# EnricoMiccoli/nodal

Measured on AMD Instinct MI355X. Metric: circuits_per_sec, higher is better.
Workload: dtype f64; 1 GPU; cfg3: grid(1000) 1e6 nodes, sparse CSR path; n=999999, nnz=4995995, parallelism=one GPU

## Files before the change

include/nodal_hip.h:

```cpp
#ifndef NODAL_HIP_H
#define NODAL_HIP_H

#include <stddef.h>
#include <stdint.h>

#ifdef __cplusplus
extern "C" {
#endif

typedef struct nodal_ctx *nodal_handle;

typedef enum {
    NODAL_OK = 0,
    NODAL_E_INVALID = 1,
    NODAL_E_HIP = 2,
    NODAL_E_ZERO_RESISTANCE = 3,
    NODAL_E_STAMP_COLLISION = 4,
    NODAL_E_SINGULAR = 5,
    NODAL_E_NOMEM = 6,
    NODAL_E_UNSUPPORTED = 7
} nodal_status;

enum { NODAL_T_R = 0, NODAL_T_A = 1, NODAL_T_E = 2, NODAL_T_VCVS = 3,
       NODAL_T_CCVS = 4, NODAL_T_CCCS = 5,
       NODAL_T_GM = 6 };

enum { NODAL_SPARSE_AUTO = 0,
       NODAL_SPARSE_PCG = 1,
       NODAL_SPARSE_DENSIFY = 2,
       NODAL_SPARSE_LU = 3,
       NODAL_SPARSE_DIRECT = 4 };

int nodal_create(int device_id, nodal_handle *out);
int nodal_destroy(nodal_handle h);
const char *nodal_last_error(nodal_handle h);
const char *nodal_version(void);

int nodal_upload_components(nodal_handle h, int64_t ncomp,
                            const uint8_t *type, const double *value,
                            const int32_t *a, const int32_t *b,
                            const int32_t *c, const int32_t *d,
                            const int32_t *drv, const int32_t *k,
                            int32_t K, int32_t B);
int nodal_host_alloc(size_t bytes, void **out);
int nodal_host_free(void *p);

int nodal_upload_values(nodal_handle h, int32_t batch, const double *values);

int nodal_assemble_symbolic(nodal_handle h);
int nodal_assemble_numeric(nodal_handle h, int32_t member, int64_t *bad_component);

int nodal_get_sizes(nodal_handle h, int64_t *n, int64_t *nnz, int64_t *ncontrib);

int nodal_export_csr(nodal_handle h, int32_t *indptr, int32_t *indices,
                     double *data, double *rhs);
int nodal_export_dense(nodal_handle h, double *G, double *rhs);

int nodal_solve_dense(nodal_handle h, double *x, int32_t *info);
int nodal_solve_sparse(nodal_handle h, int32_t method, double *x, int32_t *info,
                       int32_t *iters, double *resid);
int nodal_download_x(nodal_handle h, double *x);

int nodal_solve_pairs(nodal_handle h, int32_t dense, int32_t npairs, const int32_t *ia,
                      const int32_t *ib, double *resistance, int32_t *info);

int nodal_solve_sources(nodal_handle h, int32_t dense, int32_t count, int32_t nsrc, const int64_t *rows,
                        const double *values, double *x_out, double *resid_out, int32_t *info_out);

int nodal_branches(nodal_handle h, double *voltage, double *current, double *power, double *totals2);

int nodal_solve_sources_branches(nodal_handle h, int32_t dense, int32_t count, int32_t nsrc, const int64_t *rows,
                                 const double *values, double *x_out, double *resid_out, int32_t *info_out,
                                 double *current_absmax, int32_t *current_member, double *potential_min,
                                 int32_t *potential_min_member, double *potential_max, int32_t *potential_max_member,
                                 double *power_out);

int nodal_sensitivities(nodal_handle h, int32_t dense, int32_t count, const int32_t *kind, const int32_t *p,
                        const int32_t *q2, double *sens_out, double *value_out, double *adjoint_out,
                        double *resid_out, int32_t *info_out);

int nodal_gradient(nodal_handle h, int32_t dense, int32_t count, const double *x, const double *cotangent, int32_t nsrc,
                   const int64_t *rows, double *grad_out, double *grad_sources_out, double *adjoint_out,
                   double *resid_out, int32_t *info_out);

int nodal_transient(nodal_handle h, int32_t dense, int32_t steps, int32_t method, int64_t ncap, const int64_t *cap_rows,
                    int32_t nsrc, const int64_t *src_rows, const double *src_values, const double *x0, int32_t nprobe,
                    const int32_t *probe_a, const int32_t *probe_b, double *wave_out, int32_t keep_every, double *x_out,
                    double *pot_min, int32_t *pot_min_step, double *pot_max, int32_t *pot_max_step, double *resid_out,
                    int32_t *info_out, int32_t *iters_out);

int nodal_transient_rlc(nodal_handle h, int32_t dense, int32_t steps, int32_t method, int64_t ncap, const int64_t *cap_rows,
                        int32_t nsrc, const int64_t *src_rows, const double *src_values, const double *x0, int32_t nprobe,
                        const int32_t *probe_a, const int32_t *probe_b, double *wave_out, int32_t keep_every, double *x_out,
                        double *pot_min, int32_t *pot_min_step, double *pot_max, int32_t *pot_max_step, double *resid_out,
                        int32_t *info_out, int32_t *iters_out, int64_t nind, const int64_t *ind_rows, const double *i0,
                        int32_t ncur, const int32_t *cur_index, double *cur_out, double *i_final_out);

int nodal_transient_gradient(nodal_handle h, int32_t dense, int32_t nprobe, const int32_t *probe_a, const int32_t *probe_b,
                             const double *wave_cot ,
                             double *grad_out ,
                             double *grad_sources_out ,
                             double *grad_x0_out ,
                             double *adjoint_out ,
                             double *resid_out , int32_t *info_out );

int nodal_ac_sweep(nodal_handle h, int32_t dense, int32_t nfreq, const double *omega ,
                   int64_t nreact, const uint8_t *kind , const double *value ,
                   const int32_t *lead_a, const int32_t *lead_b ,
                   int32_t nsrc, const int64_t *src_rows, const double *src_re, const double *src_im,
                   int32_t nprobe, const int32_t *probe_a, const int32_t *probe_b, double *wave_out ,
                   int32_t ncur, const int32_t *cur_index , double *cur_out ,
                   int32_t keep_every, double *x_out ,
                   double *peak_out , int32_t *peak_freq_out ,
                   double *resid_out , int32_t *info_out );

int nodal_ac_noise(nodal_handle h, int32_t dense, int32_t nfreq, const double *omega ,
                   int64_t nreact, const uint8_t *kind , const double *value ,
                   const int32_t *lead_a, const int32_t *lead_b ,
                   double temperature ,
                   int32_t nout, const int32_t *out_a, const int32_t *out_b ,
                   int64_t input_row , const double *weight ,
                   double *density_out , double *gain_out ,
                   double *contrib_out , double *resid_out ,
                   int32_t *info_out );

int nodal_ac_ports(nodal_handle h, int32_t dense, int32_t nfreq, const double *omega ,
                   int64_t nreact, const uint8_t *kind , const double *value ,
                   const int32_t *lead_a, const int32_t *lead_b ,
                   int32_t nports, const int32_t *ia, const int32_t *ib ,
                   double *z_out ,
                   double *node_peak_out , int32_t *node_peak_port_out ,
                   int32_t *node_peak_freq_out ,
                   double *resid_out , int32_t *info_out ,
                   int64_t *work_out );

int nodal_port_matrix(nodal_handle h, int32_t dense, int32_t nports, const int32_t *ia, const int32_t *ib,
                      double *z_out , double *voc_out ,
                      double *resid_out , int32_t *info_out );

int nodal_residual(nodal_handle h, double *scaled_residual);

int nodal_run(nodal_handle h, int32_t dense, int32_t member, int32_t reuse_symbolic,
              int32_t *info);

int nodal_run_batch(nodal_handle h, int32_t first, int32_t count, int32_t reuse_symbolic,
                    double *x_out, int32_t *info_out);
int nodal_batch_x_device(nodal_handle h, void *device_dst, int64_t capacity_bytes);
int nodal_x_device(nodal_handle h, void *device_dst, int64_t capacity_bytes);

int nodal_last_timings(nodal_handle h, double *ms3);
int nodal_last_kernel_stats(nodal_handle h, double *ms_total, int64_t *launches,
                            double *alg_bytes_or_flops);

int nodal_last_solve_info(nodal_handle h, int32_t *iterations, int32_t *amg_levels,
                          double *relative_residual);

int nodal_synchronize(nodal_handle h);

enum {
    NODAL_OPT_FORCE_PIVOTING = 1, NODAL_OPT_GEPP_PANEL = 2, NODAL_OPT_EXTRA_STREAMS = 3, NODAL_OPT_BORROW_TABLE = 4,
    NODAL_OPT_TRANSIENT_TAPE = 5
};
int nodal_set_option(nodal_handle h, int32_t option, int32_t value);

int nodal_debug_gemm(nodal_handle h, int32_t M, int32_t N, int32_t K, const double *A,
                     const double *B, double *C);
int nodal_debug_sources_rhs(nodal_handle h, int32_t count, int32_t nsrc, const int64_t *rows,
                            const double *values, double *rhs_out);
int nodal_debug_residual(nodal_handle h, int32_t transposed, int32_t cols, int32_t layout, const double *x,
                         const double *b, double *scaled_out, double *norms_out);
int nodal_debug_direct_apply(nodal_handle h, int32_t transposed, int32_t cols, const double *r, double *z,
                             int64_t *perturbed_out, int32_t *info_out);
enum {
    NODAL_HA_ACOL = 0, NODAL_HA_AVAL = 1, NODAL_HA_AVALF = 2, NODAL_HA_ALEN = 3, NODAL_HA_DINV = 4, NODAL_HA_ADCOL = 5,
    NODAL_HA_AGG = 6, NODAL_HA_PCOL = 7, NODAL_HA_PVAL = 8, NODAL_HA_PVALF = 9, NODAL_HA_RCOL = 10, NODAL_HA_RVAL = 11,
    NODAL_HA_RVALF = 12, NODAL_HA_RLEN = 13, NODAL_HA_WCOL = 14, NODAL_HA_WVAL = 15, NODAL_HA_WLEN = 16
};
int nodal_debug_hierarchy_info(nodal_handle h, int32_t *nlev, int64_t *ints , double *reals );
int nodal_debug_hierarchy_array(nodal_handle h, int32_t level, int32_t which, void *dst, int64_t capacity_bytes,
                                int64_t *bytes_out);

#ifdef __cplusplus
}
#endif
#endif
```

nodal_amd/_ffi.py:

```python

import atexit
import ctypes as C
import os
import weakref

import numpy as np

_HERE = os.path.dirname(os.path.abspath(__file__))
LIB_PATH = os.path.join(_HERE, "libnodal_hip.so")

OK, E_INVALID, E_HIP, E_ZERO_RESISTANCE, E_STAMP_COLLISION, E_SINGULAR, E_NOMEM, \
    E_UNSUPPORTED = range(8)
SPARSE_AUTO, SPARSE_PCG, SPARSE_DENSIFY, SPARSE_LU, SPARSE_DIRECT = range(5)
OPT_FORCE_PIVOTING = 1
OPT_GEPP_PANEL = 2
OPT_EXTRA_STREAMS = 3
OPT_BORROW_TABLE = 4
OPT_TRANSIENT_TAPE = 5

_p = C.POINTER
_i32p, _i64p, _f64p, _u8p = _p(C.c_int32), _p(C.c_int64), _p(C.c_double), _p(C.c_uint8)

SIGNATURES = {
    "nodal_version": (C.c_char_p, []),
    "nodal_create": (C.c_int, [C.c_int, _p(C.c_void_p)]),
    "nodal_destroy": (C.c_int, [C.c_void_p]),
    "nodal_last_error": (C.c_char_p, [C.c_void_p]),
    "nodal_upload_components": (C.c_int, [C.c_void_p, C.c_int64, _u8p, _f64p, _i32p, _i32p,
                                          _i32p, _i32p, _i32p, _i32p, C.c_int32, C.c_int32]),
    "nodal_host_alloc": (C.c_int, [C.c_size_t, _p(C.c_void_p)]),
    "nodal_host_free": (C.c_int, [C.c_void_p]),
    "nodal_upload_values": (C.c_int, [C.c_void_p, C.c_int32, _f64p]),
    "nodal_assemble_symbolic": (C.c_int, [C.c_void_p]),
    "nodal_assemble_numeric": (C.c_int, [C.c_void_p, C.c_int32, _i64p]),
    "nodal_get_sizes": (C.c_int, [C.c_void_p, _i64p, _i64p, _i64p]),
    "nodal_export_csr": (C.c_int, [C.c_void_p, _i32p, _i32p, _f64p, _f64p]),
    "nodal_export_dense": (C.c_int, [C.c_void_p, _f64p, _f64p]),
    "nodal_solve_dense": (C.c_int, [C.c_void_p, _f64p, _i32p]),
    "nodal_solve_sparse": (C.c_int, [C.c_void_p, C.c_int32, _f64p, _i32p, _i32p, _f64p]),
    "nodal_download_x": (C.c_int, [C.c_void_p, _f64p]),
    "nodal_solve_pairs": (C.c_int, [C.c_void_p, C.c_int32, C.c_int32, _i32p, _i32p, _f64p, _i32p]),
    "nodal_solve_sources": (C.c_int, [C.c_void_p, C.c_int32, C.c_int32, C.c_int32, _i64p, _f64p, _f64p, _f64p,
                                      _i32p]),
    "nodal_branches": (C.c_int, [C.c_void_p, _f64p, _f64p, _f64p, _f64p]),
    "nodal_solve_sources_branches": (C.c_int, [C.c_void_p, C.c_int32, C.c_int32, C.c_int32, _i64p, _f64p, _f64p, _f64p,
                                               _i32p, _f64p, _i32p, _f64p, _i32p, _f64p, _i32p, _f64p]),
    "nodal_sensitivities": (C.c_int, [C.c_void_p, C.c_int32, C.c_int32, _i32p, _i32p, _i32p, _f64p, _f64p, _f64p, _f64p,
                                      _i32p]),
    "nodal_gradient": (C.c_int, [C.c_void_p, C.c_int32, C.c_int32, _f64p, _f64p, C.c_int32, _i64p, _f64p, _f64p, _f64p,
                                 _f64p, _i32p]),
    "nodal_transient": (C.c_int, [C.c_void_p, C.c_int32, C.c_int32, C.c_int32, C.c_int64, _i64p, C.c_int32, _i64p, _f64p,
                                  _f64p, C.c_int32, _i32p, _i32p, _f64p, C.c_int32, _f64p, _f64p, _i32p, _f64p, _i32p,
                                  _f64p, _i32p, _i32p]),
    "nodal_transient_rlc": (C.c_int, [C.c_void_p, C.c_int32, C.c_int32, C.c_int32, C.c_int64, _i64p, C.c_int32, _i64p, _f64p,
                                      _f64p, C.c_int32, _i32p, _i32p, _f64p, C.c_int32, _f64p, _f64p, _i32p, _f64p, _i32p,
                                      _f64p, _i32p, _i32p, C.c_int64, _i64p, _f64p, C.c_int32, _i32p, _f64p, _f64p]),
    "nodal_transient_gradient": (C.c_int, [C.c_void_p, C.c_int32, C.c_int32, _i32p, _i32p, _f64p, _f64p, _f64p, _f64p, _f64p,
                                           _f64p, _i32p]),
    "nodal_ac_sweep": (C.c_int, [C.c_void_p, C.c_int32, C.c_int32, _f64p, C.c_int64, _u8p, _f64p, _i32p, _i32p, C.c_int32,
                                 _i64p, _f64p, _f64p, C.c_int32, _i32p, _i32p, _f64p, C.c_int32, _i32p, _f64p, C.c_int32,
                                 _f64p, _f64p, _i32p, _f64p, _i32p]),
    "nodal_ac_noise": (C.c_int, [C.c_void_p, C.c_int32, C.c_int32, _f64p, C.c_int64, _u8p, _f64p, _i32p, _i32p, C.c_double,
                                 C.c_int32, _i32p, _i32p, C.c_int64, _f64p, _f64p, _f64p, _f64p, _f64p, _i32p]),
    "nodal_ac_ports": (C.c_int, [C.c_void_p, C.c_int32, C.c_int32, _f64p, C.c_int64, _u8p, _f64p, _i32p, _i32p, C.c_int32,
                                 _i32p, _i32p, _f64p, _f64p, _i32p, _i32p, _f64p, _i32p, _i64p]),
    "nodal_port_matrix": (C.c_int, [C.c_void_p, C.c_int32, C.c_int32, _i32p, _i32p, _f64p, _f64p, _f64p, _i32p]),
    "nodal_residual": (C.c_int, [C.c_void_p, _f64p]),
    "nodal_run": (C.c_int, [C.c_void_p, C.c_int32, C.c_int32, C.c_int32, _i32p]),
    "nodal_run_batch": (C.c_int, [C.c_void_p, C.c_int32, C.c_int32, C.c_int32, _f64p, _i32p]),
    "nodal_batch_x_device": (C.c_int, [C.c_void_p, C.c_void_p, C.c_int64]),
    "nodal_x_device": (C.c_int, [C.c_void_p, C.c_void_p, C.c_int64]),
    "nodal_last_timings": (C.c_int, [C.c_void_p, _f64p]),
    "nodal_last_kernel_stats": (C.c_int, [C.c_void_p, _f64p, _i64p, _f64p]),
    "nodal_last_solve_info": (C.c_int, [C.c_void_p, _i32p, _i32p, _f64p]),
    "nodal_synchronize": (C.c_int, [C.c_void_p]),
    "nodal_set_option": (C.c_int, [C.c_void_p, C.c_int32, C.c_int32]),
    "nodal_debug_gemm": (C.c_int, [C.c_void_p, C.c_int32, C.c_int32, C.c_int32, _f64p, _f64p, _f64p]),
    "nodal_debug_sources_rhs": (C.c_int, [C.c_void_p, C.c_int32, C.c_int32, _i64p, _f64p, _f64p]),
    "nodal_debug_residual": (C.c_int, [C.c_void_p, C.c_int32, C.c_int32, C.c_int32, _f64p, _f64p, _f64p, _f64p]),
    "nodal_debug_direct_apply": (C.c_int, [C.c_void_p, C.c_int32, C.c_int32, _f64p, _f64p, _i64p, _i32p]),
    "nodal_debug_hierarchy_info": (C.c_int, [C.c_void_p, _i32p, _i64p, _f64p]),
    "nodal_debug_hierarchy_array": (C.c_int, [C.c_void_p, C.c_int32, C.c_int32, C.c_void_p, C.c_int64, _i64p]),
}

HIERARCHY_ARRAYS = (("acol", np.int32), ("aval", np.float64), ("avalf", np.float32), ("alen", np.int32),
                    ("dinv", np.float64), ("adcol", np.int16), ("agg", np.int32), ("pcol", np.int32),
                    ("pval", np.float64), ("pvalf", np.float32), ("rcol", np.int32), ("rval", np.float64),
                    ("rvalf", np.float32), ("rlen", np.int32), ("wcol", np.int32), ("wval", np.float32),
                    ("wlen", np.int32))
HIERARCHY_INFO = ("n", "ld", "nc", "width", "maxlen", "wfix", "nnz", "rld", "rcap", "wslots", "fold_want", "fold", "d16",
                  "in_tail", "refreshed", "dense_coarsest")

_lib = None
_live = weakref.WeakSet()


@atexit.register
def _close_all():
    _closing[0] = True
    for h in list(_live):
        h.close()


class NodalHipError(RuntimeError):
    def __init__(self, status, message):
        super().__init__(f"libnodal_hip status {status}: {message}")
        self.status = status


def load():
    global _lib
    if _lib is None:
        if not os.path.exists(LIB_PATH):
            raise OSError(
                f"{LIB_PATH} not found: build it with `make` (or "
                "`python -c 'import __graft_entry__ as g; g.build()'`) -- "
                "nodal_amd has no CPU fallback")
        lib = C.CDLL(LIB_PATH)
        for name, (res, args) in SIGNATURES.items():
            fn = getattr(lib, name)
            fn.restype, fn.argtypes = res, args
        _lib = lib
    return _lib


def _ptr(arr, ctype):
    return arr.ctypes.data_as(_p(ctype))


PINNED_MIN_BYTES = 1 << 20
_PINNED_POOL = {}
_PINNED_POOL_BYTES = [0]
_PINNED_POOL_MAX = 1 << 30
_pinned_ok = [None]
_closing = [False]


def _pinned_release(addr, nbytes):
    if _lib is None or _closing[0]:
        return
    if _PINNED_POOL_BYTES[0] + nbytes <= _PINNED_POOL_MAX:
        _PINNED_POOL.setdefault(nbytes, []).append(addr)
        _PINNED_POOL_BYTES[0] += nbytes
    else:
        _lib.nodal_host_free(C.c_void_p(addr))


def host_empty(count, dtype):
    dtype = np.dtype(dtype)
    nbytes = int(count) * dtype.itemsize
    if nbytes < PINNED_MIN_BYTES or _pinned_ok[0] is False:
        return np.empty(count, dtype=dtype)
    try:
        lib = load()
    except OSError:
        _pinned_ok[0] = False
        return np.empty(count, dtype=dtype)
    size = (nbytes + 4095) & ~4095
    free = _PINNED_POOL.get(size)
    if free:
        addr = free.pop()
        _PINNED_POOL_BYTES[0] -= size
    else:
        out = C.c_void_p()
        if lib.nodal_host_alloc(size, C.byref(out)) != OK or not out.value:
            _pinned_ok[0] = False
            return np.empty(count, dtype=dtype)
        _pinned_ok[0] = True
        addr = out.value
    buf = (C.c_char * size).from_address(addr)
    weakref.finalize(buf, _pinned_release, addr, size)
    return np.frombuffer(buf, dtype=dtype, count=count)


class Handle:

    def __init__(self, device=0):
        self.lib = load()
        self._h = C.c_void_p()
        status = self.lib.nodal_create(device, C.byref(self._h))
        if status != OK:
            raise NodalHipError(
                status, f"nodal_create(device={device}) failed: no usable MI355X "
                "(HIP device) is visible; nodal_amd has no CPU fallback")
        self.n = self.nnz = self.ncontrib = 0
        self._ncomp = self._K = 0
        self.lib.nodal_set_option(self._h, OPT_BORROW_TABLE, 1)
        _live.add(self)

    def close(self):
        if getattr(self, "_h", None):
            self.lib.nodal_destroy(self._h)
            self._h = None

    __del__ = close

    @property
    def closed(self):
        return not getattr(self, "_h", None)

    def _check(self, status, allow=()):
        if status != OK and status not in allow:
            raise NodalHipError(status, self.lib.nodal_last_error(self._h).decode())
        return status

    def upload(self, table):
        names = ("type", "value", "a", "b") if table.B == 0 else ("type", "value", "a", "b", "c", "d", "drv", "k")
        cols = [np.ascontiguousarray(getattr(table, n)) for n in names]
        self._keep = cols
        t, v, a, b = cols[:4]
        rest = [_ptr(x, C.c_int32) for x in cols[4:]] or [None] * 4
        self.n_members = table.K + table.B
        self._ncomp, self._K = int(table.ncomp), int(table.K)
        self._check(self.lib.nodal_upload_components(
            self._h, table.ncomp, _ptr(t, C.c_uint8), _ptr(v, C.c_double),
            _ptr(a, C.c_int32), _ptr(b, C.c_int32), *rest, table.K, table.B))

    def upload_values(self, values):
        values = np.ascontiguousarray(values, dtype=np.float64)
        assert values.ndim == 2
        self._check(self.lib.nodal_upload_values(self._h, values.shape[0], _ptr(values, C.c_double)))

    def assemble_symbolic(self):
        self._check(self.lib.nodal_assemble_symbolic(self._h))
        self._refresh_sizes()

    def _refresh_sizes(self):
        n, nnz, nc = C.c_int64(), C.c_int64(), C.c_int64()
        self._check(self.lib.nodal_get_sizes(self._h, C.byref(n), C.byref(nnz), C.byref(nc)))
        self.n, self.nnz, self.ncontrib = n.value, nnz.value, nc.value

    def assemble_numeric(self, member=0):
        bad = C.c_int64(-1)
        status = self._check(self.lib.nodal_assemble_numeric(self._h, member, C.byref(bad)),
                             allow=(E_ZERO_RESISTANCE, E_STAMP_COLLISION))
        return status, bad.value

    def export_csr(self, values=True):
        indptr = np.empty(self.n + 1, dtype=np.int32)
        indices = np.empty(self.nnz, dtype=np.int32)
        data = np.empty(self.nnz, dtype=np.float64) if values else None
        rhs = np.empty(self.n, dtype=np.float64) if values else None
        self._check(self.lib.nodal_export_csr(
            self._h, _ptr(indptr, C.c_int32), _ptr(indices, C.c_int32),
            _ptr(data, C.c_double) if values else None,
            _ptr(rhs, C.c_double) if values else None))
        return indptr, indices, data, rhs

    def export_dense(self):
        G = np.empty((self.n, self.n), dtype=np.float64)
        rhs = np.empty(self.n, dtype=np.float64)
        self._check(self.lib.nodal_export_dense(self._h, _ptr(G, C.c_double), _ptr(rhs, C.c_double)))
        return G, rhs

    def solve_dense(self, download=True):
        x = host_empty(self.n, np.float64) if download else None
        info = C.c_int32(0)
        self._check(self.lib.nodal_solve_dense(
            self._h, _ptr(x, C.c_double) if download else None, C.byref(info)),
            allow=(E_SINGULAR,))
        return x, info.value

    def solve_sparse(self, method=SPARSE_AUTO, download=True):
        x = host_empty(self.n, np.float64) if download else None
        info, iters, resid = C.c_int32(0), C.c_int32(0), C.c_double(0)
        self._check(self.lib.nodal_solve_sparse(
            self._h, method, _ptr(x, C.c_double) if download else None,
            C.byref(info), C.byref(iters), C.byref(resid)))
        return x, info.value, iters.value, resid.value

    def solve_pairs(self, ia, ib, dense):
        ia = np.ascontiguousarray(ia, dtype=np.int32)
        ib = np.ascontiguousarray(ib, dtype=np.int32)
        out = np.empty(len(ia), dtype=np.float64)
        info = C.c_int32(0)
        self._check(self.lib.nodal_solve_pairs(self._h, int(dense), len(ia), _ptr(ia, C.c_int32),
                                               _ptr(ib, C.c_int32), _ptr(out, C.c_double),
                                               C.byref(info)), allow=(E_SINGULAR,))
        return out, info.value

    def solve_sources(self, rows, values, dense):
        rows = np.ascontiguousarray(rows, dtype=np.int64)
        values = np.ascontiguousarray(values, dtype=np.float64)
        assert values.ndim == 2 and values.shape[1] == len(rows)
        count = values.shape[0]
        x = np.empty((count, self.n), dtype=np.float64)
        info = np.zeros(count, dtype=np.int32)
        resid = np.zeros(count, dtype=np.float64)
        self._check(self.lib.nodal_solve_sources(self._h, int(dense), count, len(rows), _ptr(rows, C.c_int64),
                                                 _ptr(values, C.c_double), _ptr(x, C.c_double),
                                                 _ptr(resid, C.c_double), _ptr(info, C.c_int32)))
        return x, info, resid

    def solve_sources_branches(self, rows, values, dense, keep_solutions=True):
        rows = np.ascontiguousarray(rows, dtype=np.int64)
        values = np.ascontiguousarray(values, dtype=np.float64)
        assert values.ndim == 2 and values.shape[1] == len(rows)
        count = values.shape[0]
        ncomp, K = self._ncomp, self._K
        x = np.empty((count, self.n), dtype=np.float64) if keep_solutions else None
        info = np.zeros(count, dtype=np.int32)
        resid = np.zeros(count, dtype=np.float64)
        env = {"current_absmax": np.empty(ncomp), "current_member": np.empty(ncomp, dtype=np.int32),
               "potential_min": np.empty(K), "potential_min_member": np.empty(K, dtype=np.int32),
               "potential_max": np.empty(K), "potential_max_member": np.empty(K, dtype=np.int32),
               "power": np.empty((count, 2))}
        self._check(self.lib.nodal_solve_sources_branches(
            self._h, int(dense), count, len(rows), _ptr(rows, C.c_int64), _ptr(values, C.c_double),
            _ptr(x, C.c_double) if keep_solutions else None, _ptr(resid, C.c_double), _ptr(info, C.c_int32),
            *(_ptr(env[key], C.c_int32 if key.endswith("member") else C.c_double) for key in env)))
        return x, info, resid, env

    def branches(self, voltage=True, current=True, power=True):
        out = [host_empty(self._ncomp, np.float64) if want else None for want in (voltage, current, power)]
        totals = np.zeros(2)
        self._check(self.lib.nodal_branches(self._h, *(_ptr(a, C.c_double) if a is not None else None for a in out),
                                            _ptr(totals, C.c_double)))
        return out[0], out[1], out[2], float(totals[0]), float(totals[1])

    def sensitivities(self, kind, p, q2, dense, adjoints=False, out=None):
        kind, p, q2 = (np.ascontiguousarray(v, dtype=np.int32) for v in (kind, p, q2))
        count = len(kind)
        assert len(p) == count and len(q2) == count
        if out is not None:
            assert out.shape == (count, self._ncomp) and out.dtype == np.float64 and out.flags.c_contiguous
            sens = out
        else:
            sens = host_empty(count * self._ncomp, np.float64).reshape(count, self._ncomp)
        lam = host_empty(count * self.n, np.float64).reshape(count, self.n) if adjoints else None
        y = np.zeros(count, dtype=np.float64)
        resid = np.zeros(count, dtype=np.float64)
        info = np.zeros(count, dtype=np.int32)
        self._check(self.lib.nodal_sensitivities(
            self._h, int(dense), count, _ptr(kind, C.c_int32), _ptr(p, C.c_int32), _ptr(q2, C.c_int32),
            _ptr(sens, C.c_double), _ptr(y, C.c_double), _ptr(lam, C.c_double) if adjoints else None,
            _ptr(resid, C.c_double), _ptr(info, C.c_int32)))
        return sens, y, lam, resid, info

    def gradient(self, cotangents, dense, rows=None, solutions=None, adjoints=False):
        cot = np.ascontiguousarray(cotangents, dtype=np.float64)
        assert cot.ndim == 2 and cot.shape[1] == self.n
        count = cot.shape[0]
        rows = np.ascontiguousarray(rows if rows is not None else [], dtype=np.int64)
        x = None
        if solutions is not None:
            x = np.ascontiguousarray(solutions, dtype=np.float64)
            assert x.shape == cot.shape
        grad = np.zeros(self._ncomp, dtype=np.float64)
        gsrc = np.zeros((count, len(rows)), dtype=np.float64)
        lam = host_empty(count * self.n, np.float64).reshape(count, self.n) if adjoints else None
        resid = np.zeros(count, dtype=np.float64)
        info = np.zeros(count, dtype=np.int32)
        self._check(self.lib.nodal_gradient(
            self._h, int(dense), count, _ptr(x, C.c_double) if x is not None else None, _ptr(cot, C.c_double),
            len(rows), _ptr(rows, C.c_int64) if len(rows) else None, _ptr(grad, C.c_double), _ptr(gsrc, C.c_double),
            _ptr(lam, C.c_double) if adjoints else None, _ptr(resid, C.c_double), _ptr(info, C.c_int32)))
        return grad, gsrc, lam, resid, info

    def port_matrix(self, ia, ib, dense, voc=True):
        ia, ib = (np.ascontiguousarray(v, dtype=np.int32) for v in (ia, ib))
        count = len(ia)
        assert ia.ndim == 1 and ib.shape == ia.shape
        z = np.zeros((count, count), dtype=np.float64)
        v_oc = np.zeros(count, dtype=np.float64) if voc else None
        resid = np.zeros(count, dtype=np.float64)
        info = np.zeros(count, dtype=np.int32)
        self._check(self.lib.nodal_port_matrix(
            self._h, int(dense), count, _ptr(ia, C.c_int32), _ptr(ib, C.c_int32), _ptr(z, C.c_double),
            _ptr(v_oc, C.c_double) if voc else None, _ptr(resid, C.c_double), _ptr(info, C.c_int32)))
        return z, v_oc, info, resid

    def transient(self, cap_rows, rows, values, x0, ia, ib, dense, method=0, keep_every=0, envelope=False):
        return self._transient(cap_rows, rows, values, x0, ia, ib, dense, method, keep_every, envelope)[:6]

    def transient_rlc(self, cap_rows, ind_rows, rows, values, x0, i0, ia, ib, cur_index, dense, method=0, keep_every=0,
                      envelope=False):
        return self._transient(cap_rows, rows, values, x0, ia, ib, dense, method, keep_every, envelope,
                               inductors=(ind_rows, i0, cur_index))

    def _transient(self, cap_rows, rows, values, x0, ia, ib, dense, method, keep_every, envelope, inductors=None):
        cap_rows = np.ascontiguousarray(cap_rows, dtype=np.int64)
        rows = np.ascontiguousarray(rows, dtype=np.int64)
        values = np.ascontiguousarray(values, dtype=np.float64)
        assert values.ndim == 2 and values.shape[1] == len(rows)
        steps = values.shape[0]
        x0 = np.ascontiguousarray(x0, dtype=np.float64)
        assert x0.shape == (self.n,)
        ia, ib = (np.ascontiguousarray(v, dtype=np.int32) for v in (ia, ib))
        assert ia.ndim == 1 and ib.shape == ia.shape
        wave = np.zeros((steps + 1, len(ia)), dtype=np.float64)
        kept = steps // keep_every if keep_every > 0 else 0
        x = host_empty(kept * self.n, np.float64).reshape(kept, self.n) if keep_every > 0 else None
# ... 260 lines not shown
```

nodal_amd/csrc/knobs.h:

```cpp
#pragma once
#include <stdint.h>
#include <stdlib.h>

#include <optional>

namespace knob {

struct Present {
    const char *name;
    bool now() const { return getenv(name) != nullptr; }
};
struct OnUnless0 {
    const char *name;
    bool now() const { const char *e = getenv(name); return !(e && atoi(e) == 0); }
};
struct OffUnlessNon0 {
    const char *name;
    bool now() const { const char *e = getenv(name); return e && atoi(e) != 0; }
};
struct OnIfSet0 {
    const char *name;
    bool now() const { const char *e = getenv(name); return e != nullptr && atoi(e) == 0; }
};
struct Level {
    const char *name;
    int now() const {
        const char *e = getenv(name);
        if (!e) return 0;
        const int v = atoi(e);
        return v > 1 ? v : 1;
    }
};
struct Int {
    const char *name;
    int dflt;
    int now() const { const char *e = getenv(name); return e ? atoi(e) : dflt; }
};
struct Int64 {
    const char *name;
    int64_t dflt;
    int64_t now() const { const char *e = getenv(name); return e ? atoll(e) : dflt; }
};
struct Double {
    const char *name;
    double dflt;
    double now() const { const char *e = getenv(name); return e ? atof(e) : dflt; }
};
struct IntIfSet {
    const char *name;
    std::optional<int> now() const { const char *e = getenv(name); return e ? std::optional<int>(atoi(e)) : std::nullopt; }
};
struct Int64IfSet {
    const char *name;
    std::optional<int64_t> now() const { const char *e = getenv(name); return e ? std::optional<int64_t>(atoll(e)) : std::nullopt; }
};
struct DoubleIfSet {
    const char *name;
    std::optional<double> now() const { const char *e = getenv(name); return e ? std::optional<double>(atof(e)) : std::nullopt; }
};
struct Text {
    const char *name;
    const char *now() const { return getenv(name); }
};

inline constexpr Present TRACE{"NODAL_TRACE"};
inline constexpr Level POISON{"NODAL_POISON"};
inline constexpr Present NOFILL{"NODAL_NOFILL"};
inline constexpr Present NANCHECK{"NODAL_NANCHECK"};
inline constexpr Double WAIT_TIMEOUT_S{"NODAL_WAIT_TIMEOUT_S", 60.0};
inline constexpr Text STREAM_PRIORITY{"NODAL_STREAM_PRIORITY"};
inline constexpr IntIfSet EXTRA_STREAMS{"NODAL_EXTRA_STREAMS"};
inline constexpr IntIfSet HOST_THREADS{"NODAL_HOST_THREADS"};
inline constexpr IntIfSet CSV_CHUNKS{"NODAL_CSV_CHUNKS"};
inline constexpr OnUnless0 FOLD_STREAM{"NODAL_FOLD_STREAM"};
inline constexpr OffUnlessNon0 COUNT_LDS{"NODAL_COUNT_LDS"};
inline constexpr IntIfSet DENSE_BLOCKINV{"NODAL_DENSE_BLOCKINV"};
inline constexpr IntIfSet GJ_SCALAR{"NODAL_GJ_SCALAR"};
inline constexpr OnUnless0 GJ_DPP{"NODAL_GJ_DPP"};
inline constexpr OnUnless0 BI_SYM{"NODAL_BI_SYM"};
inline constexpr OnIfSet0 BI_MASKED{"NODAL_BI_MASKED"};
inline constexpr Int PANEL_CUS{"NODAL_PANEL_CUS", 32};
inline constexpr Int64 BI_UNMASK_ROWS{"NODAL_BI_UNMASK_ROWS", 0};
inline constexpr OnUnless0 BI_EARLY_COPY{"NODAL_BI_EARLY_COPY"};
inline constexpr Int BI_FIRST_BLOCKS{"NODAL_BI_FIRST_BLOCKS", 2};
inline constexpr Text BI_SWITCH{"NODAL_BI_SWITCH"};
inline constexpr Text BI_SWITCH2{"NODAL_BI_SWITCH2"};
inline constexpr Text BI_WIDTH{"NODAL_BI_WIDTH"};
inline constexpr IntIfSet GEPP_PANEL{"NODAL_GEPP_PANEL"};
inline constexpr Int GEPP_MAX{"NODAL_GEPP_MAX", 1280};
inline constexpr Present GEPP_PROBE{"NODAL_GEPP_PROBE"};
inline constexpr Int64IfSet FCG_MAXIT{"NODAL_FCG_MAXIT"};
inline constexpr OnUnless0 FCG_HOST_SUM{"NODAL_FCG_HOST_SUM"};
inline constexpr Double FCG_LOOK{"NODAL_FCG_LOOK", 0.75};
inline constexpr OnUnless0 LOWDEG{"NODAL_LOWDEG"};
inline constexpr IntIfSet LOWDEG_SHARE{"NODAL_LOWDEG_SHARE"};
inline constexpr Int64 LOWDEG_MIN{"NODAL_LOWDEG_MIN", 32};
inline constexpr Present SPARSE_FORCE_DIRECT{"NODAL_SPARSE_FORCE_DIRECT"};
inline constexpr Present SPARSE_CHILD_DIRECT{"NODAL_SPARSE_CHILD_DIRECT"};
inline constexpr OnUnless0 SAGG{"NODAL_SAGG"};
inline constexpr OnUnless0 SA_REUSE{"NODAL_SA_REUSE"};
inline constexpr OnUnless0 SA_FORK{"NODAL_SA_FORK"};
inline constexpr Double SA_SPREAD{"NODAL_SA_SPREAD", 16.0};
inline constexpr Double SA_SHARE{"NODAL_SA_SHARE", 0.9};
inline constexpr IntIfSet SA_MIS{"NODAL_SA_MIS"};
inline constexpr Text SA_OMEGA_P{"NODAL_SA_OMEGA_P"};
inline constexpr Double SA_PADSLACK{"NODAL_SA_PADSLACK", 1.3};
inline constexpr OnUnless0 SA_D16{"NODAL_SA_D16"};
inline constexpr Int SA_GG{"NODAL_SA_GG", 40};
inline constexpr Int64 SA_GCAP{"NODAL_SA_GCAP", 16384};
inline constexpr Int SA_GSEG{"NODAL_SA_GSEG", 4};
inline constexpr Text SA_NU{"NODAL_SA_NU"};
inline constexpr Int SA_KCYCLE{"NODAL_SA_KCYCLE", 1};
inline constexpr Int SA_KLEVELS{"NODAL_SA_KLEVELS", 1};
inline constexpr OnUnless0 SA_KFREEZE{"NODAL_SA_KFREEZE"};
inline constexpr OnUnless0 SA_FUSE_DIR{"NODAL_SA_FUSE_DIR"};
inline constexpr OffUnlessNon0 SA_GRAPH{"NODAL_SA_GRAPH"};
inline constexpr Text SA_FOLD_POST{"NODAL_SA_FOLD_POST"};
inline constexpr OffUnlessNon0 SA_FOLD_CHECK{"NODAL_SA_FOLD_CHECK"};
inline constexpr OnUnless0 SA_TAIL_DENSE{"NODAL_SA_TAIL_DENSE"};
inline constexpr OffUnlessNon0 SA_TAIL_CHECK{"NODAL_SA_TAIL_CHECK"};
inline constexpr Int SA_TAIL_NU{"NODAL_SA_TAIL_NU", 3};
inline constexpr Present TAIL_PROBE{"NODAL_TAIL_PROBE"};
inline constexpr IntIfSet AMG_PASSES0{"NODAL_AMG_PASSES0"};
inline constexpr IntIfSet AMG_PASSES1{"NODAL_AMG_PASSES1"};
inline constexpr IntIfSet AMG_SWEEPS0{"NODAL_AMG_SWEEPS0"};
inline constexpr IntIfSet AMG_BLOCK{"NODAL_AMG_BLOCK"};
inline constexpr DoubleIfSet AMG_THETA{"NODAL_AMG_THETA"};
inline constexpr Present AMG_KEEP_DENSE{"NODAL_AMG_KEEP_DENSE"};
inline constexpr Present AMG_NOTAIL{"NODAL_AMG_NOTAIL"};
inline constexpr IntIfSet AMG_KMAX{"NODAL_AMG_KMAX"};
inline constexpr OnUnless0 PAIRS_BLOCK{"NODAL_PAIRS_BLOCK"};
inline constexpr OnUnless0 PAIRS_FUNCTIONAL{"NODAL_PAIRS_FUNCTIONAL"};
inline constexpr Int PAIRS_DIRECT{"NODAL_PAIRS_DIRECT", -1};
inline constexpr Int64 PAIRS_DIRECT_MIN{"NODAL_PAIRS_DIRECT_MIN", 256};
inline constexpr Double MULTI_BAR{"NODAL_MULTI_BAR", 1e-14};
inline constexpr IntIfSet PRESOLVE{"NODAL_PRESOLVE"};
inline constexpr OnUnless0 PRESOLVE_KEEP{"NODAL_PRESOLVE_KEEP"};
inline constexpr IntIfSet FGMRES_WINDOW{"NODAL_FGMRES_WINDOW"};
inline constexpr Text DIRECT_NB{"NODAL_DIRECT_NB"};
inline constexpr Int DIRECT_LANES{"NODAL_DIRECT_LANES", 4};
inline constexpr DoubleIfSet DIRECT_MAX_GB{"NODAL_DIRECT_MAX_GB"};
inline constexpr IntIfSet DIRECT_BIG_DIM{"NODAL_DIRECT_BIG_DIM"};
inline constexpr OnUnless0 DIRECT_FRONT_LDS{"NODAL_DIRECT_FRONT_LDS"};
inline constexpr Int DIRECT_LDS_BS{"NODAL_DIRECT_LDS_BS", 64};
inline constexpr OnUnless0 DIRECT_PANEL_REGS{"NODAL_DIRECT_PANEL_REGS"};
inline constexpr OnUnless0 DIRECT_BATCHED{"NODAL_DIRECT_BATCHED"};
inline constexpr OnUnless0 DIRECT_WAVE{"NODAL_DIRECT_WAVE"};
inline constexpr Present DIRECT_LEVELS{"NODAL_DIRECT_LEVELS"};
inline constexpr OnUnless0 DIRECT_SUPER{"NODAL_DIRECT_SUPER"};
inline constexpr OnUnless0 DIRECT_APPLY_STEPPED{"NODAL_DIRECT_APPLY_STEPPED"};
inline constexpr OnUnless0 DIRECT_PEEL{"NODAL_DIRECT_PEEL"};
inline constexpr Int ND_DEPTH{"NODAL_ND_DEPTH", 4};
inline constexpr Int64 ND_PAR{"NODAL_ND_PAR", 20000};
inline constexpr Present SLU_DEBUG{"SLU_DEBUG"};

}
```

nodal_amd/csrc/sagg.hip:

```cpp
#include <hip/hip_ext.h>

#include <atomic>
#include <type_traits>

#include "group.h"

int grounded_flags(nodal_ctx *h, uint8_t *flags_dev);

namespace {

using grp::TB;
constexpr int PW = 4;
constexpr int ACAP = 64;
constexpr int RCAP = 96;
constexpr int RCAP_SMALL = 512;
constexpr int RCAP_SMALL_ROWS = 16384;
inline int rcap_for(int64_t nc) { return nc <= RCAP_SMALL_ROWS ? RCAP_SMALL : RCAP; }
constexpr int W0_MAX = 32;
constexpr int COARSEST = 64;
constexpr int MAX_LEVELS = 12;
constexpr int MIS_ROUNDS = 6;
constexpr int TAIL_MAX_N = 1024;
constexpr int TAIL_LEVELS = 6;
constexpr int TAIL_LDS_BUDGET = 150 * 1024;
constexpr int APAD = 32;
constexpr int DOT_BLOCKS = 1024;
#ifndef NODAL_SA_OMEGA
#define NODAL_SA_OMEGA 0.85
#endif
constexpr double OMEGA = NODAL_SA_OMEGA;
constexpr double OMEGA_P = 0.70;
constexpr double OMEGA_P_COARSE = 0.85;
using cyc_t = nodal_cyc_t;

inline unsigned grid_for(int64_t n, unsigned cap = 8192) {
    int64_t g = (n + TB - 1) / TB;
    if (g < 1) g = 1;
    if (g >= 64) g = (g + 7) & ~(int64_t)7;
    return (unsigned)(g > cap ? cap : g);
}
inline int64_t pad64(int64_t n) { return (n + 63) & ~(int64_t)63; }
inline size_t align256(size_t x) { return (x + 255) & ~(size_t)255; }

__device__ __forceinline__ unsigned xcd_block() {
    const unsigned g = gridDim.x, b = blockIdx.x;
    return (g & 7u) ? b : (b & 7u) * (g >> 3) + (b >> 3);
}


struct Ell {
    int64_t n = 0, ld = 0;
    int32_t width = 0;
    const int32_t *col = nullptr;
    const int16_t *dcol = nullptr;
    const double *val = nullptr;
    const float *valf = nullptr;
    const int32_t *len = nullptr;
};

enum { ST_MAXLEN = 0, ST_GRADED = 1, ST_BADDIAG = 2, ST_OVERFLOW = 3, ST_NNZ = 4, ST_UNASSIGNED = 5,
       ST_MAXR = 6, ST_NC = 7 ,
       ST_FARCOL = 8 ,
       ST_FOLDMISS = 9 ,
       ST_COUNT = 10 };

struct SLevel {
    int64_t n = 0, ld = 0, nc = 0;
    int32_t width = 0;
    int32_t maxlen = 0;
    int32_t wfix = 0;
    int64_t nnz = 0;
    DevBuf acol, aval, alen, dinv;
    DevBuf adcol;
    bool d16 = false;
    DevBuf agg, pcol, pval;
    DevBuf rcol, rval, rlen;
    int64_t rld = 0;
    DevBuf vec, part, gflag;
    DevBuf avalf, pvalf, rvalf;
    DevBuf wcol, wval, wlen;
    int32_t wslots = 0;
    bool fold_want = false, fold = false;
    Ell A() const {
        Ell e;
        e.n = n; e.ld = ld; e.width = width;
        e.col = acol.as<int32_t>(); e.val = aval.as<double>(); e.len = alen.as<int32_t>();
        e.valf = avalf.as<float>();
        e.dcol = d16 ? adcol.as<int16_t>() : nullptr;
        return e;
    }
    template <typename T = double> T *v(int which) const { return reinterpret_cast<T *>(vec.as<double>() + (int64_t)which * ld); }
};
enum { V_X = 0, V_R = 1, V_XP = 2, V_RC = 3, V_C1 = 4, V_C2 = 5, V_V1 = 6, V_V2 = 7, V_R2 = 8, V_X1 = 9, V_T = 10,
       V_COUNT = 11 };

struct TailLevelDesc {
    int n, nc, ld, rld, width, nq, lpr;
    const int32_t *acol, *pcol, *rcol, *rlen, *alen;
    const double *aval, *dinv, *pval, *rval;
    int o_aval, o_acol, o_dinv, o_pval, o_pcol, o_rval, o_rcol, o_B, o_X, o_Y, o_R;
};
struct TailDesc {
    int nlev;
    TailLevelDesc lv[TAIL_LEVELS];
    const double *inv;
    int nu;
    int image_bytes;
    int lds_bytes;
    int skip;
    int slots;
    long long *stamps;
};

struct SHierarchy {
    std::vector<SLevel *> pool;
    int nlev = 0;
    int tail = -1;
    bool ready = false;
    bool kcycle = true;
    bool kfrozen = false;
    int kslot = -1, kcount = 0, ksamples = 0;
    int klevels = 1;
    int nu[3] = {2, 1, 2};
    bool dense_coarsest = true;
    DevBuf tail_stamps, tail_image, apcol, apval, aplen, bstat;
    DevBuf tail_op;
    bool tail_dense = false;
    DevBuf mvec;
    hipEvent_t ev_copy = nullptr;
    hipStream_t aux = nullptr;
    hipEvent_t ev_fork = nullptr, ev_join = nullptr, ev_flags = nullptr;
    bool aux_pending = false;
    bool aux_tried = false;
    bool want_flags = false;
    int flags_levels = 0;
    DevBuf stats, coarse_inv, mis_t, mis_m, mis_flag, mis_id, agg1, keys, rstart, cursor, lists;
    TailDesc td;
    uint64_t *host_stats = nullptr;
    bool sym_valid = false;
    uint64_t sym_epoch = 0;
    int64_t sym_n = 0, sym_nnz = 0;
    bool sym_general = false, sym_check = false;
    int32_t sym_floating = 0;
    hipGraph_t it_graph = nullptr;
    hipGraphExec_t it_exec = nullptr;
    uint64_t it_key = 0;
    bool refreshed = false;
    int last_iters = 0;
    int hint_iters = 0;
    int64_t hint_n = 0, hint_nnz = 0;
    int mblock_iters = 0;
    int64_t mblock_n = 0;
    unsigned long long sym_stats[MAX_LEVELS * ST_COUNT] = {0};
    SLevel *level(int l) {
        while ((int)pool.size() <= l) pool.push_back(new SLevel());
        return pool[l];
    }
    void drop_graph() {
        if (it_exec) (void)hipGraphExecDestroy(it_exec);
        if (it_graph) (void)hipGraphDestroy(it_graph);
        it_exec = nullptr;
        it_graph = nullptr;
        it_key = 0;
    }
    ~SHierarchy() {
        drop_graph();
        if (ev_copy) (void)hipEventDestroy(ev_copy);
        if (ev_fork) (void)hipEventDestroy(ev_fork);
        if (ev_join) (void)hipEventDestroy(ev_join);
        if (ev_flags) (void)hipEventDestroy(ev_flags);
        if (aux) (void)hipStreamDestroy(aux);
        for (SLevel *l : pool) {
            DevBuf *b[] = {&l->acol, &l->aval, &l->alen, &l->dinv, &l->agg, &l->pcol, &l->pval, &l->rcol,
                           &l->rval, &l->rlen, &l->vec, &l->part, &l->gflag, &l->avalf, &l->pvalf, &l->rvalf, &l->adcol,
                           &l->wcol, &l->wval, &l->wlen};
            for (DevBuf *x : b) x->release();
            delete l;
        }
        tail_image.release();
        tail_op.release();
        mvec.release();
        tail_stamps.release();
        bstat.release();
        apcol.release();
        apval.release();
        aplen.release();
        DevBuf *b[] = {&stats, &coarse_inv, &mis_t, &mis_m, &mis_flag, &mis_id, &agg1, &keys, &rstart, &cursor, &lists};
        for (DevBuf *x : b) x->release();
        if (host_stats) (void)hipHostFree(host_stats);
    }
};


constexpr int BSTAT_MAX = 65536;
__global__ __launch_bounds__(1024) void reduce_bstat(int nblocks, const uint32_t *__restrict__ bstat,
                                                     unsigned long long *__restrict__ stats, int slot_max,
                                                     int slot_sum) {
    __shared__ unsigned int s_max;
    __shared__ unsigned long long s_sum;
    if (threadIdx.x == 0) { s_max = 0; s_sum = 0; }
    __syncthreads();
    unsigned int m = 0;
    unsigned long long t = 0;
    for (int i = threadIdx.x; i < nblocks; i += 1024) {
        m = max(m, bstat[i]);
        t += bstat[BSTAT_MAX + i];
    }
    atomicMax(&s_max, m);
    atomicAdd(&s_sum, t);
    __syncthreads();
    if (threadIdx.x == 0) {
        if (slot_max >= 0) stats[slot_max] = s_max;
        if (slot_sum >= 0) stats[slot_sum] = s_sum;
    }
}

__global__ __launch_bounds__(TB) void row_stats(int64_t n, const int32_t *__restrict__ indptr,
                                                const int32_t *__restrict__ indices,
                                                const double *__restrict__ data, double share, double spread,
                                                bool general, unsigned long long *__restrict__ stats,
                                                uint32_t *__restrict__ bstat) {
    int32_t mlen = 0;
    uint32_t graded = 0, bad = 0, far = 0;
    for (int64_t i = (int64_t)xcd_block() * TB + threadIdx.x; i < n; i += (int64_t)gridDim.x * TB) {
        const int32_t e0 = indptr[i], e1 = indptr[i + 1];
        mlen = max(mlen, e1 - e0);
        double d = 0.0, mx = 0.0, mn = 1e300;
        for (int32_t e = e0; e < e1; ++e) {
            const double v = data[e];
            const int64_t dc = (int64_t)indices[e] - i;
            if (dc > 32767 || dc < -32767) far = 1;
            if (indices[e] == (int32_t)i) d = v;
            else if (v != 0.0) {
                mx = fmax(mx, fabs(v));
                mn = fmin(mn, fabs(v));
                if (v > 0.0 && !general) bad = 1;
            }
        }
        if (!(d > 0.0)) bad = 1;
        graded += (d > 0.0 && (mx > share * d || mx > spread * mn)) ? 1u : 0u;
    }
    __shared__ unsigned int s_len, s_graded, s_bad;
    if (threadIdx.x == 0) s_len = s_graded = s_bad = 0;
    __syncthreads();
    atomicMax(&s_len, (unsigned)mlen);
    if (graded) atomicAdd(&s_graded, graded);
    if (bad) atomicOr(&s_bad, 1u);
    if (far) atomicOr(&s_bad, 2u);
    __syncthreads();
    if (threadIdx.x == 0) {
        bstat[blockIdx.x] = s_len;
        bstat[BSTAT_MAX + blockIdx.x] = s_graded;
        if (s_bad & 1u) atomicOr(&stats[ST_BADDIAG], 1ull);
        if (s_bad & 2u) stats[ST_FARCOL] = 1ull;
    }
}

__global__ __launch_bounds__(TB) void csr_to_ell(int64_t n, int64_t ld, const int32_t *__restrict__ indptr,
                                                 const int32_t *__restrict__ indices,
                                                 const double *__restrict__ data, int32_t *__restrict__ col,
                                                 double *__restrict__ val, float *__restrict__ valf,
                                                 int32_t *__restrict__ len, double *__restrict__ dinv, int32_t wpad,
                                                 int16_t *__restrict__ dcol) {
    for (int64_t i = (int64_t)xcd_block() * TB + threadIdx.x; i < n; i += (int64_t)gridDim.x * TB) {
        const int32_t e0 = indptr[i], e1 = indptr[i + 1];
        double d = 1.0;
        for (int32_t e = e0; e < e1; ++e) {
            const int32_t c = indices[e];
            const double v = data[e];
            col[(int64_t)(e - e0) * ld + i] = c;
            if (dcol) dcol[(int64_t)(e - e0) * ld + i] = (int16_t)(c - (int32_t)i);
            val[(int64_t)(e - e0) * ld + i] = v;
            valf[(int64_t)(e - e0) * ld + i] = (float)v;
            if (c == (int32_t)i) d = v;
        }
        for (int32_t s = e1 - e0; s < wpad; ++s) {
            col[(int64_t)s * ld + i] = (int32_t)i;
            if (dcol) dcol[(int64_t)s * ld + i] = 0;
            val[(int64_t)s * ld + i] = 0.0;
            valf[(int64_t)s * ld + i] = 0.0f;
        }
        len[i] = e1 - e0;
        dinv[i] = 1.0 / d;
    }
}


__device__ __forceinline__ uint32_t hash30(uint32_t x) {
    x ^= x >> 16;
    x *= 0x7feb352du;
    x ^= x >> 15;
    x *= 0x846ca68bu;
    x ^= x >> 16;
    return x & 0x3fffffffu;
}

__global__ __launch_bounds__(TB) void mis_init(int64_t n, uint32_t *__restrict__ T) {
    for (int64_t i = (int64_t)xcd_block() * TB + threadIdx.x; i < n; i += (int64_t)gridDim.x * TB)
        T[i] = (1u << 30) | hash30((uint32_t)i);
}

template <int NB>
__device__ __forceinline__ uint32_t nbr_max_batch(const Ell &A, const uint32_t *__restrict__ v, int64_t i, int32_t l, int32_t s0,
                                                  uint32_t best) {
    int32_t c[NB];
#pragma unroll
    for (int u = 0; u < NB; ++u) c[u] = A.col[(int64_t)(s0 + u < l ? s0 + u : 0) * A.ld + i];
    uint32_t t[NB];
#pragma unroll
    for (int u = 0; u < NB; ++u) t[u] = v[c[u]];
#pragma unroll
    for (int u = 0; u < NB; ++u) best = t[u] > best ? t[u] : best;
    return best;
}
__device__ __forceinline__ uint32_t nbr_max(const Ell &A, const uint32_t *__restrict__ v, int64_t i, int32_t l, uint32_t best) {
    if (l <= 5) return nbr_max_batch<5>(A, v, i, l, 0, best);
    for (int32_t s0 = 0; s0 < l; s0 += 8) best = nbr_max_batch<8>(A, v, i, l, s0, best);
    return best;
}

__global__ __launch_bounds__(TB) void mis_max(Ell A, const uint32_t *__restrict__ v, uint32_t *__restrict__ m) {
    for (int64_t i = (int64_t)xcd_block() * TB + threadIdx.x; i < A.n; i += (int64_t)gridDim.x * TB)
        m[i] = nbr_max(A, v, i, A.len[i], v[i]);
}

__global__ __launch_bounds__(TB) void mis_update(Ell A, uint32_t *__restrict__ T, const uint32_t *__restrict__ m1) {
    for (int64_t i = (int64_t)xcd_block() * TB + threadIdx.x; i < A.n; i += (int64_t)gridDim.x * TB) {
        const uint32_t own = T[i];
        if ((own >> 30) != 1) continue;
        const uint32_t best = nbr_max(A, m1, i, A.len[i], m1[i]);
        if (best == own) T[i] = own | (2u << 30);
        else if ((best >> 30) == 3) T[i] = 0;
    }
}

__global__ __launch_bounds__(TB) void mis_count(int64_t n, const uint32_t *__restrict__ T,
                                                unsigned long long *__restrict__ out) {
    uint32_t left = 0;
    for (int64_t i = (int64_t)xcd_block() * TB + threadIdx.x; i < n; i += (int64_t)gridDim.x * TB)
        left += (T[i] >> 30) == 1 ? 1u : 0u;
#pragma unroll
    for (int off = 32; off > 0; off >>= 1) left += __shfl_down(left, off, 64);
    if ((threadIdx.x & 63) == 0 && left) atomicAdd(out, (unsigned long long)left);
}

__global__ __launch_bounds__(TB) void mis_flag_roots(Ell A, const uint32_t *__restrict__ T,
                                                     uint32_t *__restrict__ flag) {
    for (int64_t i = (int64_t)xcd_block() * TB + threadIdx.x; i <= A.n; i += (int64_t)gridDim.x * TB) {
        uint32_t f = 0;
        if (i < A.n) {
            const uint32_t own = T[i];
            if ((own >> 30) == 3) f = 1;
            else if ((own >> 30) == 1) {
                bool near = false;
                const int32_t l = A.len[i];
                for (int32_t s = 0; s < l; ++s) near = near || (T[A.col[(int64_t)s * A.ld + i]] >> 30) == 3;
                f = near ? 0u : 1u;
            }
        }
        flag[i] = f;
    }
}

constexpr int64_t MIS_SMALL_MAX = 1024;
__global__ __launch_bounds__(1024) void mis_small(Ell A, uint32_t *__restrict__ T, uint32_t *__restrict__ M,
                                                  uint32_t *__restrict__ flag, int rounds) {
    const int64_t n = A.n;
    for (int64_t i = threadIdx.x; i < n; i += 1024) T[i] = (1u << 30) | hash30((uint32_t)i);
    __syncthreads();
    for (int r = 0; r < rounds; ++r) {
        for (int64_t i = threadIdx.x; i < n; i += 1024) {
            uint32_t best = T[i];
            const int32_t l = A.len[i];
            for (int32_t s = 0; s < l; ++s) {
                const uint32_t t = T[A.col[(int64_t)s * A.ld + i]];
                best = t > best ? t : best;
            }
            M[i] = best;
        }
        __syncthreads();
        for (int64_t i = threadIdx.x; i < n; i += 1024) {
            const uint32_t own = T[i];
            if ((own >> 30) != 1) continue;
            uint32_t best = M[i];
            const int32_t l = A.len[i];
            for (int32_t s = 0; s < l; ++s) {
                const uint32_t t = M[A.col[(int64_t)s * A.ld + i]];
                best = t > best ? t : best;
            }
            if (best == own) T[i] = own | (2u << 30);
            else if ((best >> 30) == 3) T[i] = 0;
        }
        __syncthreads();
    }
    for (int64_t i = threadIdx.x; i <= n; i += 1024) {
        uint32_t f = 0;
        if (i < n) {
            const uint32_t own = T[i];
            if ((own >> 30) == 3) f = 1;
            else if ((own >> 30) == 1) {
                bool near = false;
                const int32_t l = A.len[i];
                for (int32_t s = 0; s < l; ++s) near = near || (T[A.col[(int64_t)s * A.ld + i]] >> 30) == 3;
                f = near ? 0u : 1u;
            }
        }
        flag[i] = f;
    }
}

__global__ __launch_bounds__(TB) void assign_near(Ell A, const uint32_t *__restrict__ T,
                                                  const uint32_t *__restrict__ flag,
                                                  const uint32_t *__restrict__ id, int32_t *__restrict__ agg1) {
    for (int64_t i = (int64_t)xcd_block() * TB + threadIdx.x; i < A.n; i += (int64_t)gridDim.x * TB) {
        int32_t a = -1;
        if (flag[i]) a = (int32_t)id[i];
        else {
            uint32_t best = 0;
            const int32_t l = A.len[i];
            auto batch = [&](auto NBc, int32_t s0) {
                constexpr int NB = decltype(NBc)::value;
                int32_t c[NB];
#pragma unroll
                for (int u = 0; u < NB; ++u) c[u] = A.col[(int64_t)(s0 + u < l ? s0 + u : 0) * A.ld + i];
                uint32_t fl[NB], tt[NB], idd[NB];
#pragma unroll
                for (int u = 0; u < NB; ++u) {
                    fl[u] = flag[c[u]];
                    tt[u] = T[c[u]];
                    idd[u] = id[c[u]];
                }
#pragma unroll
                for (int u = 0; u < NB; ++u) {
                    if (s0 + u >= l || c[u] == (int32_t)i || !fl[u]) continue;
                    const uint32_t t = tt[u] | (3u << 30);
                    if (t > best) { best = t; a = (int32_t)idd[u]; }
                }
            };
            if (l <= 5) batch(std::integral_constant<int, 5>{}, 0);
            else for (int32_t s0 = 0; s0 < l; s0 += 8) batch(std::integral_constant<int, 8>{}, s0);
        }
        agg1[i] = a;
    }
}

__global__ __launch_bounds__(TB) void assign_far(Ell A, const int32_t *__restrict__ agg1, int32_t *__restrict__ agg,
                                                 unsigned long long *__restrict__ stats) {
    for (int64_t i = (int64_t)xcd_block() * TB + threadIdx.x; i < A.n; i += (int64_t)gridDim.x * TB) {
        int32_t a = agg1[i];
        if (a < 0) {
            double bw = -1.0;
            const int32_t l = A.len[i];
            auto batch = [&](auto NBc, int32_t s0) {
                constexpr int NB = decltype(NBc)::value;
                int32_t c[NB];
                double w[NB];
#pragma unroll
                for (int u = 0; u < NB; ++u) {
                    const int64_t at = (int64_t)(s0 + u < l ? s0 + u : 0) * A.ld + i;
                    c[u] = A.col[at];
                    w[u] = fabs(A.val[at]);
                }
                int32_t aj[NB];
#pragma unroll
                for (int u = 0; u < NB; ++u) aj[u] = agg1[c[u]];
#pragma unroll
                for (int u = 0; u < NB; ++u) {
                    if (s0 + u >= l || c[u] == (int32_t)i || aj[u] < 0) continue;
                    if (w[u] > bw) { bw = w[u]; a = aj[u]; }
                }
            };
            if (l <= 5) batch(std::integral_constant<int, 5>{}, 0);
            else for (int32_t s0 = 0; s0 < l; s0 += 8) batch(std::integral_constant<int, 8>{}, s0);
            if (a < 0) stats[ST_UNASSIGNED] = 1;
        }
        agg[i] = a;
    }
}
// ... 448 lines not shown
#pragma unroll
        for (int q = 0; q < 4; ++q) {
            mine[q] = set[lane * 4 + q];
            cnt += mine[q] >= 0 ? 1 : 0;
        }
        int off = wave_excl_scan(cnt, &total);
        __syncthreads();
#pragma unroll
        for (int q = 0; q < 4; ++q)
            if (mine[q] >= 0) set[off++] = mine[q];
        __syncthreads();
        if (total > ACAP) {
            my_flags |= 1u;
            total = ACAP;
        }
        myJ = lane < total ? set[lane] : 0x7fffffff;
        __syncthreads();
#pragma unroll
        for (int k = 2; k <= 64; k <<= 1) {
#pragma unroll
            for (int j = k >> 1; j > 0; j >>= 1) {
                const int32_t other = __shfl_xor(myJ, j, 64);
                const bool up = (lane & k) == 0, lower = (lane & j) == 0;
                const int32_t lo = myJ < other ? myJ : other, hi = myJ < other ? other : myJ;
                myJ = (lower == up) ? lo : hi;
            }
        }
        }
        const int nseg = min(maxseg, total <= 16 ? 4 : (total <= 32 ? 2 : 1)), segw = 64 / nseg;
        const int seg = lane / segw;
        const int32_t segJ = __shfl(myJ, lane % segw, 64);
        double acc = 0.0;
        for (int g = 0; g < ngroups; ++g) {
            if (ngroups > 1 || NUMERIC)
                np = galerkin_products(ld, apcol, apval, aplen, rld, rcol, rval, I, g * G, min(G, rl - g * G), lJ, lV);
            int chunk = (((np + nseg - 1) / nseg) + 7) & ~7;
            if (nseg > 1 && ((chunk >> 3) & 1) == 0) chunk += 8;
            for (int p = seg * chunk; p < (seg + 1) * chunk; p += 8) {
                int32_t j8[8];
                double v8[8];
#pragma unroll
                for (int u = 0; u < 8; ++u) {
                    j8[u] = lJ[p + u];
                    v8[u] = lV[p + u];
                }
#pragma unroll
                for (int u = 0; u < 8; ++u) acc += j8[u] == segJ ? v8[u] : 0.0;
            }
            __syncthreads();
        }
        if (nseg == 4) {
            const double a1 = __shfl(acc, lane + 16, 64), a2 = __shfl(acc, lane + 32, 64), a3 = __shfl(acc, lane + 48, 64);
            acc = (acc + a1) + (a2 + a3);
        } else if (nseg == 2) {
            acc += __shfl(acc, lane + 32, 64);
        }
        if (lane >= total && lane < APAD) {
            ccol[(int64_t)lane * cld + I] = (int32_t)I;
            cval[(int64_t)lane * cld + I] = 0.0;
            cvalf[(int64_t)lane * cld + I] = 0.0f;
        }
        if (lane < total) {
            ccol[(int64_t)lane * cld + I] = myJ;
            cval[(int64_t)lane * cld + I] = acc;
            cvalf[(int64_t)lane * cld + I] = (float)acc;
            if (myJ == (int32_t)I) {
                if (!(acc > 0.0)) my_flags |= 4u;
                cdinv[I] = acc > 0.0 ? 1.0 / acc : 1.0;
            }
        }
        if (lane == 0) {
            clen[I] = total;
            my_max = (uint32_t)total > my_max ? (uint32_t)total : my_max;
            my_nnz += (uint32_t)total;
        }
        __syncthreads();
    }
    if (lane == 0) {
        bstat[blockIdx.x] = my_max;
        bstat[BSTAT_MAX + blockIdx.x] = my_nnz;
    }
    if (my_flags & 1u) atomicOr(&stats[ST_OVERFLOW], 1ull);
    if (my_flags & 4u) atomicOr(&stats[ST_BADDIAG], 1ull);
}

__global__ __launch_bounds__(256) void coarsest_inverse(Ell A, double *__restrict__ inv,
                                                        unsigned long long *__restrict__ stats) {
    __shared__ double M[COARSEST][2 * COARSEST + 1];
    const int n = (int)A.n;
    for (int t = threadIdx.x; t < n * 2 * n; t += 256) {
        const int r = t / (2 * n), c = t % (2 * n);
        M[r][c] = (c >= n && c - n == r) ? 1.0 : 0.0;
    }
    __syncthreads();
    for (int r = threadIdx.x; r < n; r += 256)
        for (int s = 0; s < A.len[r]; ++s) M[r][A.col[(int64_t)s * A.ld + r]] = A.val[(int64_t)s * A.ld + r];
    __syncthreads();
    for (int k = 0; k < n; ++k) {
        const double pv = M[k][k];
        if (!(pv > 0.0)) {
            if (threadIdx.x == 0) atomicOr(&stats[ST_BADDIAG], 2ull);
            return;
        }
        const double rp = 1.0 / pv;
        __syncthreads();
        for (int c = threadIdx.x; c < 2 * n; c += 256) M[k][c] *= rp;
        __syncthreads();
        for (int t = threadIdx.x; t < n * 2 * n; t += 256) {
            const int r = t / (2 * n), c = t % (2 * n);
            if (r != k && c != k) M[r][c] = fma(-M[r][k], M[k][c], M[r][c]);
        }
        __syncthreads();
        for (int r = threadIdx.x; r < n; r += 256)
            if (r != k) M[r][k] = 0.0;
        __syncthreads();
    }
    for (int t = threadIdx.x; t < n * n; t += 256) inv[t] = M[t / n][n + t % n];
}

__global__ __launch_bounds__(TB) void flags_up(int64_t n, const int32_t *__restrict__ agg,
                                               const uint8_t *__restrict__ fine, uint8_t *__restrict__ coarse) {
    for (int64_t i = (int64_t)xcd_block() * TB + threadIdx.x; i < n; i += (int64_t)gridDim.x * TB)
        if (fine[i]) coarse[agg[i]] = 1;
}
__global__ __launch_bounds__(64) void last_level_floating(Ell A, const uint8_t *__restrict__ grounded,
                                                          uint32_t *__restrict__ floating) {
    __shared__ int label[COARSEST];
    __shared__ int changed;
    const int n = (int)A.n, i = threadIdx.x;
    if (i < n) label[i] = i;
    __syncthreads();
    for (int it = 0; it < COARSEST; ++it) {
        if (i == 0) changed = 0;
        __syncthreads();
        int best = i < n ? label[i] : 0;
        if (i < n)
            for (int s = 0; s < A.len[i]; ++s) {
                const int l = label[A.col[(int64_t)s * A.ld + i]];
                best = l < best ? l : best;
            }
        __syncthreads();
        if (i < n && best < label[i]) {
            label[i] = best;
            changed = 1;
        }
        __syncthreads();
        if (!changed) break;
        __syncthreads();
    }
    __shared__ int ok[COARSEST];
    if (i < n) ok[i] = 0;
    __syncthreads();
    if (i < n && grounded[i]) ok[label[i]] = 1;
    __syncthreads();
    if (i < n && label[i] == i && !ok[i]) *floating = 1;
}

__global__ __launch_bounds__(TB) void any_unflagged(int64_t n, const uint8_t *__restrict__ grounded,
                                                    uint32_t *__restrict__ floating) {
    for (int64_t i = (int64_t)xcd_block() * TB + threadIdx.x; i < n; i += (int64_t)gridDim.x * TB)
        if (!grounded[i]) *floating = 1;
}

}

#include "sagg_cycle.h"

namespace {

constexpr int SAGG_DECLINED = -3;

int width_class(int maxlen) {
    static const int classes[] = {4, 5, 6, 8, 12, 16, 20, 24, 32};
    for (int c : classes)
        if (maxlen <= c) return c;
    return 0;
}
int choose_wfix(int maxlen, int64_t n, int64_t nnz, int pad_limit) {
    const int c = width_class(maxlen);
    if (c == 0 || c > pad_limit) return 0;
    static const double slack = knob::SA_PADSLACK.now();
    if ((double)c * (double)n <= slack * (double)nnz || n <= 32768) return c;
    return 0;
}

SHierarchy *hierarchy_of(nodal_ctx *h) {
    if (!h->sagg) h->sagg = new SHierarchy();
    return static_cast<SHierarchy *>(h->sagg);
}

struct SolveBufs {
    double *r, *p, *p2, *Ap, *part_rz, *part_zap, *part_rr, *part_pap, *sc;
    cyc_t *z, *x0;
    int g0;
};

template <bool NUMERIC>
int galerkin_product(nodal_ctx *h, SHierarchy *H, int l, hipEvent_t r_ready = nullptr, int phase = 0) {
    hipStream_t st = h->stream;
    SLevel *L = H->level(l), *C = H->level(l + 1);
    const int64_t n = L->n, ld = L->ld, nc = C->n;
    Ell A = L->A();
    A.width = L->maxlen;
    unsigned long long *dstats = H->stats.as<unsigned long long>();
    const int apw = A.width <= 6 ? 16 : 64;
    NODAL_HIP_TRY(h, H->apcol.reserve((size_t)apw * ld * 4 + 64));
    NODAL_HIP_TRY(h, H->apval.reserve((size_t)apw * ld * 8 + 64));
    NODAL_HIP_TRY(h, H->aplen.reserve((size_t)ld * 4 + 64));
    int32_t *apcol = H->apcol.as<int32_t>(), *aplen = H->aplen.as<int32_t>();
    double *apval = H->apval.as<double>();
    unsigned long long *lst = dstats + (size_t)l * ST_COUNT;
    const unsigned g = grid_for(n);
    if (phase != 2) {
        const bool w = L->fold_want && L->wslots == apw;
        int32_t *wcol = w ? L->wcol.as<int32_t>() : nullptr, *wlen = w ? L->wlen.as<int32_t>() : nullptr;
        float *wval = w ? L->wval.as<float>() : nullptr;
        const double *dinv = L->dinv.as<double>();
        const int32_t *pc = L->pcol.as<int32_t>();
        const double *pv = L->pval.as<double>();
        const unsigned gl = (unsigned)((n + 63) / 64 < 4096 ? (n + 63) / 64 : 4096);
        if (apw == 16 && w) ap_rows<16, true><<<g, TB, 0, st>>>(A, pc, pv, apcol, apval, aplen, lst, dinv, wcol, wval, wlen);
        else if (apw == 16) ap_rows<16, false><<<g, TB, 0, st>>>(A, pc, pv, apcol, apval, aplen, lst, dinv, wcol, wval, wlen);
        else if (w) ap_rows_lds<64, true><<<gl, 64, 0, st>>>(A, pc, pv, apcol, apval, aplen, lst, dinv, wcol, wval, wlen);
        else ap_rows_lds<64, false><<<gl, 64, 0, st>>>(A, pc, pv, apcol, apval, aplen, lst, dinv, wcol, wval, wlen);
        NODAL_HIP_TRY(h, hipGetLastError());
    }
    if (phase == 1) return NODAL_OK;
    int G = 1024 / apw;
    G = (G < 8 ? 8 : (G > 64 ? 64 : G));
    static const int g_env = knob::SA_GG.now();
    if (g_env >= 8 && g_env <= 64 && apw == 16) G = g_env & ~7;
    const int pcap = G * apw + 72;
    const size_t lds = 1024 + (size_t)pcap * 12;
    static const int64_t gcap = knob::SA_GCAP.now();
    static const int maxseg = knob::SA_GSEG.now();
    const unsigned gg = (unsigned)(nc < gcap ? nc : (gcap < BSTAT_MAX ? gcap : BSTAT_MAX));
    if (r_ready) NODAL_HIP_TRY(h, hipStreamWaitEvent(st, r_ready, 0));
    galerkin<NUMERIC><<<gg, 64, lds, st>>>(
        ld, apcol, apval, aplen, nc, L->rld, L->rcol.as<int32_t>(), L->rval.as<double>(), L->rlen.as<int32_t>(),
        C->ld, C->acol.as<int32_t>(), C->aval.as<double>(), C->avalf.as<float>(), C->alen.as<int32_t>(),
        C->dinv.as<double>(), dstats + (size_t)(l + 1) * ST_COUNT, H->bstat.as<uint32_t>(), G, pcap, maxseg);
    if (!NUMERIC)
        reduce_bstat<<<1, 1024, 0, st>>>((int)gg, H->bstat.as<uint32_t>(), dstats + (size_t)(l + 1) * ST_COUNT,
                                         ST_MAXLEN, ST_NNZ);
    NODAL_HIP_TRY(h, hipGetLastError());
    return NODAL_OK;
}

double omega_p(int level) {
    static double w[2] = {-1.0, -1.0};
    if (w[0] < 0.0) {
        double a = OMEGA_P, b = OMEGA_P_COARSE;
        if (const char *e = knob::SA_OMEGA_P.now()) {
            a = atof(e);
            const char *c = strchr(e, ',');
            b = c ? atof(c + 1) : a;
        }
        w[1] = b > 0.0 && b < 1.2 ? b : OMEGA_P_COARSE;
        w[0] = a > 0.0 && a < 1.0 ? a : OMEGA_P;
    }
    return w[level > 0 ? 1 : 0];
}

constexpr int64_t FOLD_MAX_ROWS = 1 << 19;
struct FoldSetting { int mode = 0; unsigned mask = 0; };
const FoldSetting &fold_setting() {
    static const FoldSetting s = [] {
        FoldSetting f;
        const char *e = knob::SA_FOLD_POST.now();
        if (!e || !*e) return f;
        if (strchr(e, 'l')) {
            f.mode = 3;
            for (const char *q = e; (q = strchr(q, 'l')) != nullptr; ++q) {
                const int k = atoi(q + 1);
                if (q[1] >= '0' && q[1] <= '9' && k < MAX_LEVELS) f.mask |= 1u << k;
            }
        } else {
            f.mode = atoi(e) == 0 ? 1 : 2;
        }
        return f;
    }();
    return s;
}
bool fold_wanted(int level, int64_t n) {
    if (level > 0 && n <= TAIL_MAX_N) return false;
    const FoldSetting &f = fold_setting();
    switch (f.mode) {
    case 1: return false;
    case 2: return true;
    case 3: return (f.mask >> level & 1u) != 0;
    default: return n <= FOLD_MAX_ROWS;
    }
}
void decide_folds(SHierarchy *H, const unsigned long long *hs, bool trace) {
    for (int k = 0; k < H->nlev; ++k) {
        SLevel *L = H->pool[k];
        const bool runs_cycle = k + 1 < H->nlev && (H->tail < 0 || k < H->tail);
        const bool miss = hs[(size_t)k * ST_COUNT + ST_FOLDMISS] != 0;
        L->fold = L->fold_want && runs_cycle && !miss;
        if (trace && L->fold_want && runs_cycle)
            fprintf(stderr, "[sagg] level %d (%lld rows): first post-smoothing sweep %s\n", k, (long long)L->n,
                    miss ? "NOT folded: a row of A P lacks a column of its P row (no stored diagonal)"
                         : "folded into the prolongation");
    }
}

int build_level(nodal_ctx *h, SHierarchy *H, int l, unsigned long long *hs, bool *declined, bool *stop) {
    hipStream_t st = h->stream;
    SLevel *L = H->level(l);
    const int64_t n = L->n, ld = L->ld;
    Ell A = L->A();
    A.width = L->maxlen;
    unsigned long long *dstats = H->stats.as<unsigned long long>();

    NODAL_HIP_TRY(h, H->mis_t.reserve((size_t)n * 8 + 64));
    NODAL_HIP_TRY(h, H->mis_m.reserve((size_t)n * 8 + 64));
    NODAL_HIP_TRY(h, H->mis_flag.reserve((size_t)(n + 1) * 4 + 64));
    NODAL_HIP_TRY(h, H->mis_id.reserve((size_t)(n + 1) * 4 + 64 + scan_tmp_bytes(n + 1)));
    NODAL_HIP_TRY(h, H->agg1.reserve((size_t)n * 4 + 64));
    NODAL_HIP_TRY(h, L->agg.reserve((size_t)n * 4 + 64));
    NODAL_HIP_TRY(h, H->cursor.reserve((MIS_ROUNDS + 2) * 8 + 64));
    uint32_t *T = H->mis_t.as<uint32_t>(), *M = H->mis_m.as<uint32_t>();
    uint32_t *flag = H->mis_flag.as<uint32_t>(), *id = H->mis_id.as<uint32_t>();
    unsigned long long *cnt = H->cursor.as<unsigned long long>();
    void *scan_tmp = H->mis_id.as<char>() + (((size_t)(n + 1) * 4 + 63) & ~(size_t)63);

    const unsigned g = grid_for(n);
    static const bool trace_mis = knob::TRACE.now();
    if (trace_mis) NODAL_HIP_TRY(h, hipMemsetAsync(cnt, 0, (MIS_ROUNDS + 2) * 8, st));
    static const int mis_rounds = std::min(MIS_ROUNDS, std::max(1, knob::SA_MIS.now().value_or(MIS_ROUNDS)));
    if (n <= MIS_SMALL_MAX && !trace_mis) {
        mis_small<<<1, 1024, 0, st>>>(A, T, M, flag, mis_rounds);
    } else {
        mis_init<<<g, TB, 0, st>>>(n, T);
        for (int r = 0; r < mis_rounds; ++r) {
            mis_max<<<g, TB, 0, st>>>(A, T, M);
            mis_update<<<g, TB, 0, st>>>(A, T, M);
            if (trace_mis) mis_count<<<g, TB, 0, st>>>(n, T, cnt + r + 1);
        }
        mis_flag_roots<<<grid_for(n + 1), TB, 0, st>>>(A, T, flag);
    }
    NODAL_HIP_TRY(h, hipGetLastError());
    NODAL_TRY(scan_exclusive_u32(h, flag, id, n + 1, reinterpret_cast<uint32_t *>(dstats + (size_t)l * ST_COUNT + ST_NC),
                                 scan_tmp));
    NODAL_HIP_TRY(h, hipMemcpyAsync(hs, dstats, (size_t)MAX_LEVELS * ST_COUNT * 8, hipMemcpyDeviceToHost, st));
    unsigned long long hcnt[MIS_ROUNDS + 1] = {0};
    if (trace_mis) NODAL_HIP_TRY(h, hipMemcpyAsync(hcnt, cnt, sizeof hcnt, hipMemcpyDeviceToHost, st));
    if (!H->ev_copy) NODAL_HIP_TRY(h, hipEventCreateWithFlags(&H->ev_copy, hipEventDisableTiming));
    NODAL_HIP_TRY(h, hipEventRecord(H->ev_copy, st));
    NODAL_HIP_TRY(h, L->pcol.reserve((size_t)PW * ld * 4 + 64));
    NODAL_HIP_TRY(h, L->pval.reserve((size_t)PW * ld * 8 + 64));
    NODAL_HIP_TRY(h, L->pvalf.reserve((size_t)PW * ld * 4 + 64));
    assign_near<<<g, TB, 0, st>>>(A, T, flag, id, H->agg1.as<int32_t>());
    assign_far<<<g, TB, 0, st>>>(A, H->agg1.as<int32_t>(), L->agg.as<int32_t>(), dstats + (size_t)l * ST_COUNT);
    build_P<<<g, TB, 0, st>>>(A, L->dinv.as<double>(), L->agg.as<int32_t>(), L->pcol.as<int32_t>(),
                             L->pval.as<double>(), L->pvalf.as<float>(), omega_p(l));
    NODAL_HIP_TRY(h, hipGetLastError());
    NODAL_WAIT_EVENT(h, H->ev_copy, st);
    if (trace_mis) {
        fprintf(stderr, "[sagg] level %d: undecided after each MIS round:", l);
        for (int r = 1; r <= MIS_ROUNDS; ++r) fprintf(stderr, " %llu", hcnt[r]);
        fprintf(stderr, "\n");
    }
    const int64_t nc = (int64_t)(hs[(size_t)l * ST_COUNT + ST_NC] & 0xffffffffull);
    if (l > 0) {
        const unsigned long long *s = hs + (size_t)l * ST_COUNT;
        L->maxlen = (int32_t)s[ST_MAXLEN];
        L->nnz = (int64_t)s[ST_NNZ];
        A.width = L->maxlen;
        if (s[ST_OVERFLOW] || s[ST_BADDIAG] || hs[(size_t)(l - 1) * ST_COUNT + ST_OVERFLOW] ||
            hs[(size_t)(l - 1) * ST_COUNT + ST_UNASSIGNED]) {
            *declined = true;
            return NODAL_OK;
        }
    }
    if (nc >= n || L->maxlen <= 1) {
        *stop = true;
        return NODAL_OK;
    }
    if ((nc * 2 > n && n > 4096) || nc < 1) {
        *declined = true;
        return NODAL_OK;
    }
    L->nc = nc;

    static const bool fork_allowed = knob::SA_FORK.now();
    if (H->aux && !nodal_extra_streams_ok(h) && nodal_calls_in_flight() <= 1) {
        NODAL_WAIT_STREAM(h, H->aux);
        (void)hipStreamDestroy(H->aux);
        H->aux = nullptr;
        H->aux_tried = false;
    }
    if (fork_allowed && !H->aux_tried && nodal_extra_streams_ok(h)) {
        H->aux_tried = true;
        if (hipStreamCreateWithFlags(&H->aux, hipStreamNonBlocking) != hipSuccess) H->aux = nullptr;
        if (H->aux && ((!H->ev_fork && hipEventCreateWithFlags(&H->ev_fork, hipEventDisableTiming) != hipSuccess) ||
                       (!H->ev_join && hipEventCreateWithFlags(&H->ev_join, hipEventDisableTiming) != hipSuccess) ||
                       (!H->ev_flags && hipEventCreateWithFlags(&H->ev_flags, hipEventDisableTiming) != hipSuccess))) {
            (void)hipStreamDestroy(H->aux);
            H->aux = nullptr;
        }
        (void)hipGetLastError();
    }
    const bool forked = fork_allowed && H->aux != nullptr && nodal_extra_streams_ok(h);
    const size_t a4 = (((size_t)(nc + 1) * 4) + 255) & ~(size_t)255;
    const size_t scan2 = (scan_tmp_bytes(nc + 1) + 255) & ~(size_t)255;
    NODAL_HIP_TRY(h, H->rstart.reserve(a4 + 256 + scan2 + (size_t)PW * ld * 4 + 64));
    NODAL_HIP_TRY(h, H->keys.reserve((size_t)PW * n * 8 + 64));
    SLevel *C = H->level(l + 1);
    C->n = nc;
    C->ld = pad64(nc);
    C->width = ACAP;
    C->nc = 0;
    L->rld = C->ld;
    const int rcap = rcap_for(nc);
    NODAL_HIP_TRY(h, L->rcol.reserve((size_t)rcap * C->ld * 4 + 64));
    NODAL_HIP_TRY(h, L->rval.reserve((size_t)rcap * C->ld * 8 + 64));
    NODAL_HIP_TRY(h, L->rvalf.reserve((size_t)rcap * C->ld * 4 + 64));
    NODAL_HIP_TRY(h, L->rlen.reserve((size_t)C->ld * 4 + 64));
    NODAL_HIP_TRY(h, C->acol.reserve((size_t)ACAP * C->ld * 4 + 64));
    NODAL_HIP_TRY(h, C->aval.reserve((size_t)ACAP * C->ld * 8 + 64));
    NODAL_HIP_TRY(h, C->avalf.reserve((size_t)ACAP * C->ld * 4 + 64));
    NODAL_HIP_TRY(h, C->alen.reserve((size_t)C->ld * 4 + 64));
    NODAL_HIP_TRY(h, C->dinv.reserve((size_t)C->ld * 8 + 64));
    if (forked && H->want_flags) {
        if (l == 0) NODAL_HIP_TRY(h, L->gflag.reserve((size_t)n + 64));
        NODAL_HIP_TRY(h, C->gflag.reserve((size_t)C->n + 64));
    }
    {
        const int apw = L->maxlen <= 6 ? 16 : 64;
        NODAL_HIP_TRY(h, H->apcol.reserve((size_t)apw * ld * 4 + 64));
        NODAL_HIP_TRY(h, H->apval.reserve((size_t)apw * ld * 8 + 64));
        NODAL_HIP_TRY(h, H->aplen.reserve((size_t)ld * 4 + 64));
        L->fold = false;
        L->fold_want = fold_wanted(l, n);
        L->wslots = apw;
        if (L->fold_want) {
            NODAL_HIP_TRY(h, L->wcol.reserve((size_t)apw * ld * 4 + 64));
            NODAL_HIP_TRY(h, L->wval.reserve((size_t)apw * ld * 4 + 64));
            NODAL_HIP_TRY(h, L->wlen.reserve((size_t)ld * 4 + 64));
        }
    }
    hipStream_t main_st = h->stream;
    struct StreamGuard {
        nodal_ctx *h;
        hipStream_t keep;
        ~StreamGuard() { h->stream = keep; }
    } guard{h, main_st};
    if (forked) {
        NODAL_HIP_TRY(h, hipEventRecord(H->ev_fork, main_st));
        NODAL_HIP_TRY(h, hipStreamWaitEvent(H->aux, H->ev_fork, 0));
        H->aux_pending = true;
        NODAL_TRY(galerkin_product<false>(h, H, l, nullptr, 1));
        h->stream = H->aux;
        st = H->aux;
    }
    char *rs = H->rstart.as<char>();
    uint32_t *rstart = reinterpret_cast<uint32_t *>(rs);
    void *scan_tmp2 = rs + a4 + 256;
    uint32_t *place = reinterpret_cast<uint32_t *>(rs + a4 + 256 + scan2);
    NODAL_HIP_TRY(h, hipMemsetAsync(rs, 0, a4 + 256, st));
    r_count<<<g, TB, 0, st>>>(n, ld, L->pcol.as<int32_t>(), rstart, place);
    NODAL_HIP_TRY(h, hipGetLastError());
    NODAL_TRY(scan_exclusive_u32(h, rstart, rstart, nc + 1, nullptr, scan_tmp2));
    uint64_t *keys = H->keys.as<uint64_t>();
    r_fill<<<g, TB, 0, st>>>(n, ld, L->pcol.as<int32_t>(), rstart, place, keys);
    r_sort_short<<<grid_for(nc), TB, 0, st>>>(rstart, keys, nc);
    r_sort_medium<<<(unsigned)(nc < 8192 ? nc : 8192), 64, 0, st>>>(rstart, keys, nc);
    NODAL_HIP_TRY(h, hipGetLastError());

    {
        const unsigned gr = grid_for(nc * 8);
        r_to_ell<<<gr, TB, 0, st>>>(nc, L->rld, rstart, keys, ld, L->pval.as<double>(), L->rcol.as<int32_t>(),
                                   L->rval.as<double>(), L->rvalf.as<float>(), L->rlen.as<int32_t>(),
                                   dstats + (size_t)l * ST_COUNT, H->bstat.as<uint32_t>(), (uint32_t)rcap);
        reduce_bstat<<<1, 1024, 0, st>>>((int)gr, H->bstat.as<uint32_t>(), dstats + (size_t)l * ST_COUNT, ST_MAXR, -1);
    }
    if (forked) {
        NODAL_HIP_TRY(h, hipGetLastError());
        NODAL_HIP_TRY(h, hipEventRecord(H->ev_join, H->aux));
        if (H->want_flags && H->flags_levels == l) {
            if (l == 0) NODAL_TRY(grounded_flags(h, L->gflag.as<uint8_t>()));
            NODAL_HIP_TRY(h, hipMemsetAsync(C->gflag.p, 0, ((size_t)C->n + 63) & ~(size_t)63, st));
            flags_up<<<grid_for(n), TB, 0, st>>>(n, L->agg.as<int32_t>(), L->gflag.as<uint8_t>(), C->gflag.as<uint8_t>());
            NODAL_HIP_TRY(h, hipGetLastError());
            NODAL_HIP_TRY(h, hipEventRecord(H->ev_flags, H->aux));
            H->flags_levels = l + 1;
        }
        h->stream = main_st;
        st = main_st;
    }
    NODAL_TRY(galerkin_product<false>(h, H, l, forked ? H->ev_join : nullptr, forked ? 2 : 0));
    if (forked && H->flags_levels != l + 1) H->aux_pending = false;
    return NODAL_OK;
}

const void *tail_kernel(int slots) {
    return slots <= 8 ? reinterpret_cast<const void *>(k_tail<8>)
                      : slots <= 16 ? reinterpret_cast<const void *>(k_tail<16>)
                                    : reinterpret_cast<const void *>(k_tail<32>);
}

const void *tail_op_kernel(int slots) {
    return slots <= 8 ? reinterpret_cast<const void *>(k_tail_pack_op<8>)
                      : slots <= 16 ? reinterpret_cast<const void *>(k_tail_pack_op<16>)
                                    : reinterpret_cast<const void *>(k_tail_pack_op<32>);
}

int tail_walk(nodal_ctx *h, SHierarchy *H, const double *b, double *out, int nv) {
    const TailDesc &d = H->td;
    const char *img = H->tail_image.as<char>();
    if (d.slots <= 8) k_tail<8><<<nv, 1024, (size_t)d.lds_bytes, h->stream>>>(d, img, b, out, nv);
    else if (d.slots <= 16) k_tail<16><<<nv, 1024, (size_t)d.lds_bytes, h->stream>>>(d, img, b, out, nv);
    else k_tail<32><<<nv, 1024, (size_t)d.lds_bytes, h->stream>>>(d, img, b, out, nv);
    NODAL_HIP_TRY(h, hipGetLastError());
    return NODAL_OK;
}

template <int NV>
int tail_apply(nodal_ctx *h, SHierarchy *H, const double *b, double *out) {
    const int n = H->td.lv[0].n;
    const double *T = H->tail_op.as<double>();
    const unsigned gr = (unsigned)((n + 3) / 4);
    if (n <= 256) k_tail_apply<4, NV><<<gr, 256, 0, h->stream>>>(n, T, b, out);
    else if (n <= 512) k_tail_apply<8, NV><<<gr, 256, 0, h->stream>>>(n, T, b, out);
    else k_tail_apply<16, NV><<<gr, 256, 0, h->stream>>>(n, T, b, out);
    NODAL_HIP_TRY(h, hipGetLastError());
    return NODAL_OK;
}

int tail_self_check(nodal_ctx *h, SHierarchy *H) {
    const int n = H->td.lv[0].n;
    std::vector<double> b((size_t)n), yc((size_t)n), yd((size_t)n), T((size_t)n * n);
    uint64_t seed = 0x9e3779b97f4a7c15ull;
    for (int i = 0; i < n; ++i) {
        uint64_t z = (seed += 0x9e3779b97f4a7c15ull);
        z = (z ^ (z >> 30)) * 0xbf58476d1ce4e5b9ull;
        z = (z ^ (z >> 27)) * 0x94d049bb133111ebull;
        z ^= z >> 31;
        b[i] = (double)(z >> 11) * (1.0 / 4503599627370496.0) - 1.0;
    }
    DevBuf v;
    hipError_t e = v.reserve((size_t)3 * n * 8);
    double *db = v.as<double>(), *dc = db + n, *dd = dc + n;
    int rc = NODAL_OK;
    if (e == hipSuccess) e = hipMemcpyAsync(db, b.data(), (size_t)n * 8, hipMemcpyHostToDevice, h->stream);
    if (e == hipSuccess) rc = tail_walk(h, H, db, dc, 1);
    if (e == hipSuccess && rc == NODAL_OK) rc = tail_apply<1>(h, H, db, dd);
    if (e == hipSuccess && rc == NODAL_OK) e = hipStreamSynchronize(h->stream);
    if (e == hipSuccess) e = hipMemcpy(yc.data(), dc, (size_t)n * 8, hipMemcpyDeviceToHost);
    if (e == hipSuccess) e = hipMemcpy(yd.data(), dd, (size_t)n * 8, hipMemcpyDeviceToHost);
    if (e == hipSuccess) e = hipMemcpy(T.data(), H->tail_op.p, (size_t)n * n * 8, hipMemcpyDeviceToHost);
    v.release();
    if (rc != NODAL_OK) return rc;
    NODAL_HIP_TRY(h, e);
    double d = 0.0, dp = 0.0;
    for (int i = 0; i < n; ++i) {
        long double y = 0.0L, a = 0.0L;
        for (int j = 0; j < n; ++j) {
            y += (long double)T[(size_t)i * n + j] * b[j];
            a += fabsl((long double)T[(size_t)i * n + j] * b[j]);
        }
        const double den = (double)a;
        const double q = fabs(yd[i] - yc[i]) / den, qp = (double)(fabsl((long double)yd[i] - y) / a);
        d = !(q <= d) ? q : d;
        dp = !(qp <= dp) ? qp : dp;
    }
    fprintf(stderr, "[sagg] tail check: n_t %d, dense operator against the cycle d = %.3e (product alone %.3e)\n", n, d, dp);
    return NODAL_OK;
}

int form_tail_op(nodal_ctx *h, SHierarchy *H) {
    static const bool on = knob::SA_TAIL_DENSE.now();
    H->tail_dense = false;
    if (!on || H->tail < 0) return NODAL_OK;
    const TailDesc &d = H->td;
    const int n = d.lv[0].n;
    static std::atomic<int> cus[64];
    const int dev = h->device >= 0 && h->device < 64 ? h->device : 0;
    int ncu = cus[dev].load(std::memory_order_acquire);
    if (ncu == 0) {
        NODAL_HIP_TRY(h, hipDeviceGetAttribute(&ncu, hipDeviceAttributeMultiprocessorCount, h->device >= 0 ? h->device : 0));
        if (ncu < 1) ncu = 1;
        cus[dev].store(ncu, std::memory_order_release);
    }
    NODAL_HIP_TRY(h, H->tail_op.reserve((size_t)n * n * 8 + 64));
    const unsigned gr = (unsigned)(n < ncu ? n : ncu);
    double *T = H->tail_op.as<double>();
    const char *img = H->tail_image.as<char>();
    if (d.slots <= 8) k_tail_pack_op<8><<<gr, 1024, (size_t)d.lds_bytes, h->stream>>>(d, img, T);
    else if (d.slots <= 16) k_tail_pack_op<16><<<gr, 1024, (size_t)d.lds_bytes, h->stream>>>(d, img, T);
    else k_tail_pack_op<32><<<gr, 1024, (size_t)d.lds_bytes, h->stream>>>(d, img, T);
    NODAL_HIP_TRY(h, hipGetLastError());
    H->tail_dense = true;
    static const bool check = knob::TRACE.now() && knob::SA_TAIL_CHECK.now();
    if (check) NODAL_TRY(tail_self_check(h, H));
    return NODAL_OK;
}

template <typename TC>
int fold_check_level(nodal_ctx *h, SHierarchy *H, int l, bool two) {
    hipStream_t st = h->stream;
    const SLevel *L = H->pool[l];
    const int64_t n = L->n, nc = H->pool[l + 1]->n;
    const Ell A = L->A();
    uint64_t seed = 0x9e3779b97f4a7c15ull + (uint64_t)l;
    auto unit = [&]() {
        uint64_t z = (seed += 0x9e3779b97f4a7c15ull);
        z = (z ^ (z >> 30)) * 0xbf58476d1ce4e5b9ull;
        z = (z ^ (z >> 27)) * 0x94d049bb133111ebull;
        z ^= z >> 31;
        return (double)(z >> 11) * (1.0 / 4503599627370496.0) - 1.0;
    };
    std::vector<cyc_t> hx((size_t)n), hb((size_t)n);
    std::vector<TC> he((size_t)2 * nc);
    for (auto &v : hx) v = (cyc_t)unit();
    for (auto &v : hb) v = (cyc_t)unit();
    for (auto &v : he) v = (TC)unit();
    const double hcoef[2] = {0.9, 0.4};
    const size_t vb = align256((size_t)n * sizeof(cyc_t)), eb = align256((size_t)nc * sizeof(TC)), db = align256((size_t)n * 8);
    DevBuf buf;
    hipError_t e = buf.reserve(6 * vb + 2 * eb + 2 * db + 256);
    char *p = buf.as<char>();
    cyc_t *x = reinterpret_cast<cyc_t *>(p), *b = reinterpret_cast<cyc_t *>(p + vb), *r = reinterpret_cast<cyc_t *>(p + 2 * vb),
          *xp = reinterpret_cast<cyc_t *>(p + 3 * vb), *mt = reinterpret_cast<cyc_t *>(p + 4 * vb),
          *mf = reinterpret_cast<cyc_t *>(p + 5 * vb);
    TC *c1 = reinterpret_cast<TC *>(p + 6 * vb), *c2 = reinterpret_cast<TC *>(p + 6 * vb + eb);
    double *d = reinterpret_cast<double *>(p + 6 * vb + 2 * eb), *q = reinterpret_cast<double *>(p + 6 * vb + 2 * eb + db);
    double *coef = reinterpret_cast<double *>(p + 6 * vb + 2 * eb + 2 * db);
    std::vector<double> hd((size_t)n), hq((size_t)n);
    if (e == hipSuccess) e = hipMemcpyAsync(x, hx.data(), (size_t)n * sizeof(cyc_t), hipMemcpyHostToDevice, st);
    if (e == hipSuccess) e = hipMemcpyAsync(b, hb.data(), (size_t)n * sizeof(cyc_t), hipMemcpyHostToDevice, st);
    if (e == hipSuccess) e = hipMemcpyAsync(c1, he.data(), (size_t)nc * sizeof(TC), hipMemcpyHostToDevice, st);
    if (e == hipSuccess) e = hipMemcpyAsync(c2, he.data() + nc, (size_t)nc * sizeof(TC), hipMemcpyHostToDevice, st);
    if (e == hipSuccess) e = hipMemcpyAsync(coef, hcoef, sizeof hcoef, hipMemcpyHostToDevice, st);
    if (e == hipSuccess) {
        const unsigned g = grid_for(n), tb = L->wfix ? TB : TB * LPR_RAGGED;
        const double *dinv = L->dinv.as<double>(), *cf = two ? coef : nullptr;
        const int32_t *wcol = L->wcol.as<int32_t>(), *wlen = L->wlen.as<int32_t>();
        const float *wval = L->wval.as<float>();
        SAGG_DISPATCH_W(L->wfix, (k_smooth_residual<W, cyc_t><<<g, tb, 0, st>>>(A, b, x, r)));
        k_prolong<TC><<<g, TB, 0, st>>>(n, L->ld, L->pcol.as<int32_t>(), L->pvalf.as<float>(), x, c1, two ? c2 : nullptr, cf, xp);
        SAGG_DISPATCH_W(L->wfix, (k_post<W, false, cyc_t, cyc_t><<<g, tb, 0, st>>>(A, dinv, b, xp, mt, nullptr, nullptr, nullptr)));
        k_prolong_post<TC, cyc_t><<<g, TB, 0, st>>>(n, L->ld, wcol, wval, wlen, x, r, dinv, c1, two ? c2 : nullptr, cf, mf);
        k_fold_check<TC><<<g, TB, 0, st>>>(A, dinv, b, x, xp, wcol, wval, wlen, c1, two ? c2 : nullptr, cf, mt, mf, d, q);
        e = hipGetLastError();
    }
    if (e == hipSuccess) e = hipStreamSynchronize(st);
    if (e == hipSuccess) e = hipMemcpy(hd.data(), d, (size_t)n * 8, hipMemcpyDeviceToHost);
    if (e == hipSuccess) e = hipMemcpy(hq.data(), q, (size_t)n * 8, hipMemcpyDeviceToHost);
    buf.release();
    NODAL_HIP_TRY(h, e);
    double dm = 0.0, qm = 0.0;
    for (int64_t i = 0; i < n; ++i) {
        dm = !(hd[i] <= dm) ? hd[i] : dm;
        qm = !(hq[i] <= qm) ? hq[i] : qm;
    }
    fprintf(stderr, "[sagg] fold check: level %d, rows %lld, slots %d, width %d, fused launch against the two d = %.3e "
                    "(worst row against its own bound: %.3e)\n", l, (long long)n, (int)L->wslots, (int)L->maxlen, dm, qm);
    return NODAL_OK;
}
int fold_self_check(nodal_ctx *h, SHierarchy *H) {
    static const bool check = knob::TRACE.now() && knob::SA_FOLD_CHECK.now();
    if (!check) return NODAL_OK;
    for (int l = 0; l + 1 < H->nlev; ++l) {
        if (!H->pool[l]->fold) continue;
        const bool last = l + 1 == H->tail || l + 1 == H->nlev - 1;
        if (last) NODAL_TRY(fold_check_level<double>(h, H, l, false));
        else NODAL_TRY(fold_check_level<cyc_t>(h, H, l, true));
    }
    return NODAL_OK;
}

int build_tail(nodal_ctx *h, SHierarchy *H, const unsigned long long *hs) {
    H->tail = -1;
    H->tail_dense = false;
    const int last = H->nlev - 1;
    auto up16 = [](int x) { return (x + 15) & ~15; };
    for (int t = 1; t <= last; ++t) {
        if (H->pool[t]->n > TAIL_MAX_N || last - t + 1 > TAIL_LEVELS) continue;
        TailDesc d;
        memset(&d, 0, sizeof d);
        d.nlev = last - t + 1;
        d.nu = knob::SA_TAIL_NU.now();
        if (d.nu < 1) d.nu = 1;
        int off = 0;
        for (int k = 0; k < d.nlev; ++k) {
            const SLevel *L = H->pool[t + k];
            TailLevelDesc &q = d.lv[k];
            q.n = (int)L->n; q.nc = (int)L->nc; q.ld = (int)L->ld; q.rld = (int)L->rld; q.width = L->maxlen;
            q.acol = L->acol.as<int32_t>(); q.aval = L->aval.as<double>();
            q.dinv = L->dinv.as<double>(); q.alen = L->alen.as<int32_t>();
            q.pcol = L->pcol.as<int32_t>(); q.pval = L->pval.as<double>();
            q.rcol = L->rcol.as<int32_t>(); q.rval = L->rval.as<double>(); q.rlen = L->rlen.as<int32_t>();
            if (k == d.nlev - 1) {
                q.o_aval = off; off = up16(off + (H->dense_coarsest ? q.n * q.n : q.n) * 8);
                continue;
            }
            const int maxr = (int)hs[(size_t)(t + k) * ST_COUNT + ST_MAXR];
            q.nq = (maxr + 7) / 8;
            q.lpr = 1;
            while (q.lpr < 8 && q.n * q.lpr * 2 <= 1024) q.lpr *= 2;
            q.o_aval = off; off = up16(off + q.n * q.width * 8);
            q.o_acol = off; off = up16(off + q.n * q.width * 2);
            q.o_dinv = off; off = up16(off + q.n * 8);
            q.o_pval = off; off = up16(off + q.n * PW * 8);
            q.o_pcol = off; off = up16(off + q.n * PW * 2);
            q.o_rval = off; off = up16(off + q.nq * q.nc * 8 * 8);
            q.o_rcol = off; off = up16(off + q.nq * q.nc * 8 * 2);
        }
        d.image_bytes = off;
        for (int k = 0; k < d.nlev; ++k) {
            TailLevelDesc &q = d.lv[k];
            q.o_B = off; off = up16(off + q.n * 8);
            q.o_X = off; off = up16(off + q.n * 8);
            if (k == d.nlev - 1) continue;
            q.o_Y = off; off = up16(off + q.n * 8);
            q.o_R = off; off = up16(off + q.n * 8);
        }
        d.inv = H->dense_coarsest ? H->coarse_inv.as<double>() : nullptr;
        d.skip = d.nlev > 1 ? d.lv[0].o_dinv : 0;
        d.lds_bytes = off - d.skip;
        if (knob::TAIL_PROBE.now()) {
            NODAL_HIP_TRY(h, H->tail_stamps.reserve(64 * sizeof(long long)));
            d.stamps = H->tail_stamps.as<long long>();
        }
        if (d.lds_bytes > TAIL_LDS_BUDGET) continue;
        d.slots = d.nlev > 1 ? (d.lv[0].width + d.lv[0].lpr - 1) / d.lv[0].lpr : 1;
        if (d.slots > 32) continue;
        {
            static std::atomic<bool> lds_allowed[64][3];
            const int dev = h->device >= 0 && h->device < 64 ? h->device : 0;
            const int which = d.slots <= 8 ? 0 : (d.slots <= 16 ? 1 : 2);
            if (!lds_allowed[dev][which].load(std::memory_order_acquire)) {
                NODAL_HIP_TRY(h, hipFuncSetAttribute(tail_kernel(d.slots), hipFuncAttributeMaxDynamicSharedMemorySize,
                                                     TAIL_LDS_BUDGET));
                NODAL_HIP_TRY(h, hipFuncSetAttribute(tail_op_kernel(d.slots), hipFuncAttributeMaxDynamicSharedMemorySize,
                                                     TAIL_LDS_BUDGET));
                lds_allowed[dev][which].store(true, std::memory_order_release);
            }
        }
        NODAL_HIP_TRY(h, H->tail_image.reserve((size_t)d.image_bytes + 256));
        k_tail_pack<<<1, 1024, 0, h->stream>>>(d, H->tail_image.as<char>());
        NODAL_HIP_TRY(h, hipGetLastError());
        H->td = d;
        H->tail = t;
        NODAL_TRY(form_tail_op(h, H));
        break;
    }
    return NODAL_OK;
}

int sagg_refresh(nodal_ctx *h, SHierarchy *H, const int32_t *indptr0, const int32_t *indices0, const double *data0,
                 bool general, bool *ok) {
    *ok = false;
    hipStream_t st = h->stream;
    unsigned long long *dstats = H->stats.as<unsigned long long>();
    unsigned long long *hs = reinterpret_cast<unsigned long long *>(H->host_stats);
    NODAL_HIP_TRY(h, hipMemsetAsync(dstats, 0, (size_t)MAX_LEVELS * ST_COUNT * 8, st));
    SLevel *L0 = H->pool[0];
    const int64_t n0 = L0->n;
    {
        const unsigned gr = grid_for(n0);
        static const double spread = knob::SA_SPREAD.now();
        static const double share = knob::SA_SHARE.now();
        row_stats<<<gr, TB, 0, st>>>(n0, indptr0, indices0, data0, share, spread, general, dstats, H->bstat.as<uint32_t>());
        reduce_bstat<<<1, 1024, 0, st>>>((int)gr, H->bstat.as<uint32_t>(), dstats, ST_MAXLEN, ST_GRADED);
    }
    csr_to_ell<<<grid_for(n0), TB, 0, st>>>(n0, L0->ld, indptr0, indices0, data0, L0->acol.as<int32_t>(),
                                           L0->aval.as<double>(), L0->avalf.as<float>(),
                                           L0->alen.as<int32_t>(), L0->dinv.as<double>(), L0->wfix,
                                           L0->d16 ? L0->adcol.as<int16_t>() : nullptr);
    NODAL_HIP_TRY(h, hipGetLastError());
    for (int l = 0; l + 1 < H->nlev; ++l) {
        SLevel *L = H->pool[l], *C = H->pool[l + 1];
        Ell A = L->A();
        A.width = L->maxlen;
        build_P<<<grid_for(L->n), TB, 0, st>>>(A, L->dinv.as<double>(), L->agg.as<int32_t>(), L->pcol.as<int32_t>(),
                                              L->pval.as<double>(), L->pvalf.as<float>(), omega_p(l));
        const bool forked = H->aux != nullptr && nodal_extra_streams_ok(h) &&
                            knob::SA_FORK.now();
        hipStream_t rst = st;
        if (forked) {
            NODAL_HIP_TRY(h, hipEventRecord(H->ev_fork, st));
            NODAL_HIP_TRY(h, hipStreamWaitEvent(H->aux, H->ev_fork, 0));
            H->aux_pending = true;
            NODAL_TRY(galerkin_product<true>(h, H, l, nullptr, 1));
            rst = H->aux;
        }
        r_refresh<<<grid_for(C->n * 8), TB, 0, rst>>>(C->n, L->rld, L->rlen.as<int32_t>(), L->rcol.as<int32_t>(), L->ld,
                                                     L->pcol.as<int32_t>(), L->pval.as<double>(), L->rval.as<double>(),
                                                     L->rvalf.as<float>());
        NODAL_HIP_TRY(h, hipGetLastError());
        if (forked) NODAL_HIP_TRY(h, hipEventRecord(H->ev_join, H->aux));
        NODAL_TRY(galerkin_product<true>(h, H, l, forked ? H->ev_join : nullptr, forked ? 2 : 0));
        if (forked) H->aux_pending = false;
    }
    const int last = H->nlev - 1;
    if (H->dense_coarsest)
        coarsest_inverse<<<1, 256, 0, st>>>(H->pool[last]->A(), H->coarse_inv.as<double>(), dstats + (size_t)last * ST_COUNT);
    if (H->tail >= 0) k_tail_pack<<<1, 1024, 0, st>>>(H->td, H->tail_image.as<char>());
    NODAL_HIP_TRY(h, hipGetLastError());
    NODAL_TRY(form_tail_op(h, H));
    NODAL_HIP_TRY(h, hipMemcpyAsync(hs, dstats, (size_t)MAX_LEVELS * ST_COUNT * 8, hipMemcpyDeviceToHost, st));
    NODAL_WAIT_STREAM(h, st);
    const int64_t bar = n0 / 100 < 32 ? (n0 / 100 > 0 ? n0 / 100 : 1) : 32;
    if (hs[ST_BADDIAG] || (int64_t)hs[ST_GRADED] >= bar) return NODAL_OK;
    for (int k = 1; k < H->nlev; ++k)
        if (hs[(size_t)k * ST_COUNT + ST_BADDIAG] || hs[(size_t)k * ST_COUNT + ST_OVERFLOW]) return NODAL_OK;
    decide_folds(H, hs, false);
    NODAL_TRY(fold_self_check(h, H));
    *ok = true;
    return NODAL_OK;
}

}

void sagg_destroy(nodal_ctx *h) {
    delete static_cast<SHierarchy *>(h->sagg);
    h->sagg = nullptr;
}

static int sagg_setup_csr_body(nodal_ctx *h, int64_t n0, int64_t nnz0, const int32_t *indptr0, const int32_t *indices0,
                               const double *data0, bool general, bool check_floating, bool *accepted, int32_t *floating);

int sagg_setup_csr(nodal_ctx *h, int64_t n0, int64_t nnz0, const int32_t *indptr0, const int32_t *indices0,
                   const double *data0, bool general, bool check_floating, bool *accepted, int32_t *floating) {
    const int s = sagg_setup_csr_body(h, n0, nnz0, indptr0, indices0, data0, general, check_floating, accepted, floating);
    SHierarchy *H = static_cast<SHierarchy *>(h->sagg);
    if (H && H->aux && H->aux_pending && H->ev_flags) {
        if (hipEventRecord(H->ev_flags, H->aux) == hipSuccess) (void)hipStreamWaitEvent(h->stream, H->ev_flags, 0);
        H->aux_pending = false;
        (void)hipGetLastError();
    }
    return s;
}

static int sagg_setup_csr_body(nodal_ctx *h, int64_t n0, int64_t nnz0, const int32_t *indptr0, const int32_t *indices0,
                               const double *data0, bool general, bool check_floating, bool *accepted, int32_t *floating) {
    *accepted = false;
    *floating = 0;
    static const bool enabled = knob::SAGG.now();
    static const bool trace = knob::TRACE.now();
    if (!enabled) return NODAL_OK;
    SHierarchy *H = hierarchy_of(h);
    H->ready = false;
    hipStream_t st = h->stream;
    if (n0 >= (1ll << 30)) return NODAL_OK;
    static const bool reuse = knob::SA_REUSE.now();
    if (reuse && H->sym_valid && H->sym_epoch == h->struct_epoch && H->sym_n == n0 && H->sym_nnz == nnz0 &&
        H->sym_general == general && H->sym_check == check_floating) {
        bool ok = false;
        NODAL_TRY(sagg_refresh(h, H, indptr0, indices0, data0, general, &ok));
        if (ok) {
            *floating = H->sym_floating;
            H->refreshed = true;
            H->ready = true;
            *accepted = true;
            if (trace) fprintf(stderr, "[sagg] symbolic setup kept (struct epoch %llu): values refreshed\n",
                               (unsigned long long)h->struct_epoch);
            return NODAL_OK;
        }
        if (trace) fprintf(stderr, "[sagg] the kept hierarchy does not take the new values: full setup\n");
    }
    H->sym_valid = false;
    H->refreshed = false;
    H->want_flags = check_floating;
    H->flags_levels = 0;
    H->last_iters = 0;
    H->drop_graph();
    NODAL_HIP_TRY(h, H->stats.reserve((size_t)MAX_LEVELS * ST_COUNT * 8 + 64));
    if (!H->host_stats)
        NODAL_HIP_TRY(h, hipHostMalloc(reinterpret_cast<void **>(&H->host_stats), (size_t)MAX_LEVELS * ST_COUNT * 8 + 64));
    unsigned long long *dstats = H->stats.as<unsigned long long>();
    unsigned long long *hs = reinterpret_cast<unsigned long long *>(H->host_stats);
    NODAL_HIP_TRY(h, hipMemsetAsync(dstats, 0, (size_t)MAX_LEVELS * ST_COUNT * 8, st));
    NODAL_HIP_TRY(h, H->bstat.reserve((size_t)2 * BSTAT_MAX * 4 + 64));
    {
        const unsigned gr = grid_for(n0);
        static const double spread = knob::SA_SPREAD.now();
        static const double share = knob::SA_SHARE.now();
        row_stats<<<gr, TB, 0, st>>>(n0, indptr0, indices0, data0, share, spread, general, dstats, H->bstat.as<uint32_t>());
        reduce_bstat<<<1, 1024, 0, st>>>((int)gr, H->bstat.as<uint32_t>(), dstats, ST_MAXLEN, ST_GRADED);
    }
    NODAL_HIP_TRY(h, hipGetLastError());
    NODAL_HIP_TRY(h, hipMemcpyAsync(hs, dstats, ST_COUNT * 8, hipMemcpyDeviceToHost, st));
    NODAL_WAIT_STREAM(h, st);
    const int64_t bar = n0 / 100 < 32 ? (n0 / 100 > 0 ? n0 / 100 : 1) : 32;
    if (hs[ST_MAXLEN] > (unsigned long long)W0_MAX || hs[ST_MAXLEN] == 0 || hs[ST_BADDIAG] ||
        (int64_t)hs[ST_GRADED] >= bar) {
        if (trace)
            fprintf(stderr, "[sagg] declined: longest row %llu, graded nodes %llu (bar %lld), M-matrix %s\n",
                    hs[ST_MAXLEN], hs[ST_GRADED], (long long)bar, hs[ST_BADDIAG] ? "no" : "yes");
        return NODAL_OK;
    }
    SLevel *L0 = H->level(0);
    L0->n = n0;
    L0->ld = pad64(n0);
    L0->maxlen = (int32_t)hs[ST_MAXLEN];
    L0->nnz = nnz0;
    L0->wfix = choose_wfix(L0->maxlen, n0, nnz0, 8);
    L0->width = L0->wfix ? L0->wfix : L0->maxlen;
    NODAL_HIP_TRY(h, L0->acol.reserve((size_t)L0->width * L0->ld * 4 + 64));
    NODAL_HIP_TRY(h, L0->aval.reserve((size_t)L0->width * L0->ld * 8 + 64));
    NODAL_HIP_TRY(h, L0->avalf.reserve((size_t)L0->width * L0->ld * 4 + 64));
    NODAL_HIP_TRY(h, L0->alen.reserve((size_t)L0->ld * 4 + 64));
    NODAL_HIP_TRY(h, L0->dinv.reserve((size_t)L0->ld * 8 + 64));
    static const bool d16_env = knob::SA_D16.now();
    L0->d16 = d16_env && hs[ST_FARCOL] == 0;
    if (L0->d16) NODAL_HIP_TRY(h, L0->adcol.reserve((size_t)L0->width * L0->ld * 2 + 64));
    csr_to_ell<<<grid_for(n0), TB, 0, st>>>(n0, L0->ld, indptr0, indices0, data0, L0->acol.as<int32_t>(),
                                           L0->aval.as<double>(), L0->avalf.as<float>(),
                                           L0->alen.as<int32_t>(), L0->dinv.as<double>(), L0->wfix,
                                           L0->d16 ? L0->adcol.as<int16_t>() : nullptr);
    NODAL_HIP_TRY(h, hipGetLastError());

    int l = 0;
    bool diag_last = false;
    for (;; ++l) {
        SLevel *L = H->level(l);
        if (L->n <= COARSEST && l > 0) break;
        if (l + 1 >= MAX_LEVELS) {
            if (trace) fprintf(stderr, "[sagg] declined: more than %d levels\n", MAX_LEVELS);
            return NODAL_OK;
        }
        bool declined = false, stop = false;
        NODAL_TRY(build_level(h, H, l, hs, &declined, &stop));
        if (declined) {
            if (trace)
                fprintf(stderr, "[sagg] declined at level %d (%lld rows): does not coarsen / over a cap / not positive "
                                "(this level: overflow %llx baddiag %llx; level above: overflow %llx unassigned %llu maxr %llu)\n",
                        l, (long long)L->n, hs[(size_t)l * ST_COUNT + ST_OVERFLOW], hs[(size_t)l * ST_COUNT + ST_BADDIAG],
                        l > 0 ? hs[(size_t)(l - 1) * ST_COUNT + ST_OVERFLOW] : 0ull,
                        l > 0 ? hs[(size_t)(l - 1) * ST_COUNT + ST_UNASSIGNED] : 0ull,
                        l > 0 ? hs[(size_t)(l - 1) * ST_COUNT + ST_MAXR] : 0ull);
            return NODAL_OK;
        }
        if (stop) {
            diag_last = true;
            break;
        }
    }
    H->nlev = l + 1;
    SLevel *last = H->level(l);
    last->fold_want = last->fold = false;
    if (H->nlev < 2) return NODAL_OK;
    NODAL_HIP_TRY(h, hipMemcpyAsync(hs, dstats, (size_t)MAX_LEVELS * ST_COUNT * 8, hipMemcpyDeviceToHost, st));
    if (!H->ev_copy) NODAL_HIP_TRY(h, hipEventCreateWithFlags(&H->ev_copy, hipEventDisableTiming));
    NODAL_HIP_TRY(h, hipEventRecord(H->ev_copy, st));
    if (check_floating) {
        if (H->flags_levels == 0) {
            NODAL_HIP_TRY(h, H->level(0)->gflag.reserve((size_t)n0 + 64));
            NODAL_TRY(grounded_flags(h, H->level(0)->gflag.as<uint8_t>()));
        } else {
            NODAL_HIP_TRY(h, hipStreamWaitEvent(st, H->ev_flags, 0));
            H->aux_pending = false;
        }
        for (int k = H->flags_levels; k + 1 < H->nlev; ++k) {
            SLevel *L = H->pool[k], *C = H->pool[k + 1];
            NODAL_HIP_TRY(h, C->gflag.reserve((size_t)C->n + 64));
            NODAL_HIP_TRY(h, hipMemsetAsync(C->gflag.p, 0, ((size_t)C->n + 63) & ~(size_t)63, st));
            flags_up<<<grid_for(L->n), TB, 0, st>>>(L->n, L->agg.as<int32_t>(), L->gflag.as<uint8_t>(),
                                                   C->gflag.as<uint8_t>());
        }
        NODAL_HIP_TRY(h, hipGetLastError());
    }
    NODAL_WAIT_EVENT(h, H->ev_copy, st);
    for (int k = 0; k < H->nlev; ++k) {
        const unsigned long long *s = hs + (size_t)k * ST_COUNT;
        if (k > 0) {
            H->pool[k]->maxlen = (int32_t)s[ST_MAXLEN];
            H->pool[k]->nnz = (int64_t)s[ST_NNZ];
            H->pool[k]->wfix = choose_wfix(H->pool[k]->maxlen, H->pool[k]->n, H->pool[k]->nnz, APAD);
        }
        if (s[ST_OVERFLOW] || (k > 0 && s[ST_BADDIAG]) || s[ST_UNASSIGNED]) {
            if (trace) fprintf(stderr, "[sagg] declined: level %d over a cap / not positive\n", k);
            return NODAL_OK;
        }
    }
    diag_last = last->maxlen <= 1;
    H->dense_coarsest = !diag_last;
    if (H->dense_coarsest) {
        if (last->n > COARSEST) return NODAL_OK;
        NODAL_HIP_TRY(h, H->coarse_inv.reserve((size_t)last->n * last->n * 8 + 64));
        coarsest_inverse<<<1, 256, 0, st>>>(last->A(), H->coarse_inv.as<double>(),
                                            dstats + (size_t)l * ST_COUNT);
        NODAL_HIP_TRY(h, hipGetLastError());
    }
    for (int k = 0; k < H->nlev; ++k) {
        SLevel *L = H->pool[k];
        NODAL_HIP_TRY(h, L->vec.reserve((size_t)V_COUNT * L->ld * 8 + 256));
        NODAL_HIP_TRY(h, L->part.reserve(5 * DOT_BLOCKS * 8 + 512));
    }
    NODAL_TRY(build_tail(h, H, hs));

    if (!check_floating) {
        NODAL_HIP_TRY(h, hipMemcpyAsync(hs, dstats, (size_t)MAX_LEVELS * ST_COUNT * 8, hipMemcpyDeviceToHost, st));
        NODAL_WAIT_STREAM(h, st);
        if (hs[(size_t)l * ST_COUNT + ST_BADDIAG] & 2ull) return NODAL_OK;
    } else {
        uint32_t *fl = reinterpret_cast<uint32_t *>(dstats + (size_t)(MAX_LEVELS - 1) * ST_COUNT + ST_COUNT - 1);
        if (H->dense_coarsest) last_level_floating<<<1, 64, 0, st>>>(last->A(), last->gflag.as<uint8_t>(), fl);
        else any_unflagged<<<grid_for(last->n), TB, 0, st>>>(last->n, last->gflag.as<uint8_t>(), fl);
        NODAL_HIP_TRY(h, hipGetLastError());
        NODAL_HIP_TRY(h, hipMemcpyAsync(hs, dstats, (size_t)MAX_LEVELS * ST_COUNT * 8, hipMemcpyDeviceToHost, st));
        NODAL_WAIT_STREAM(h, st);
        if (hs[(size_t)l * ST_COUNT + ST_BADDIAG] & 2ull) {
            if (trace) fprintf(stderr, "[sagg] declined: coarsest matrix not positive definite\n");
            return NODAL_OK;
        }
        *floating = hs[(size_t)(MAX_LEVELS - 1) * ST_COUNT + ST_COUNT - 1] != 0 ? 1 : 0;
    }
    if (trace) {
        fprintf(stderr, "[sagg] levels (rows/entries/longest row/padded width):");
        for (int k = 0; k < H->nlev; ++k)
            fprintf(stderr, " %lld/%lld/%d/%d", (long long)H->pool[k]->n, (long long)H->pool[k]->nnz,
                    H->pool[k]->maxlen, H->pool[k]->wfix);
        fprintf(stderr, "  tail %d (%d register slots)  coarsest %s\n", H->tail, H->tail >= 0 ? H->td.slots : 0,
                H->dense_coarsest ? "dense" : "diagonal");
    }
    decide_folds(H, hs, trace);
    NODAL_TRY(fold_self_check(h, H));
    H->ready = true;
    *accepted = true;
    H->sym_valid = true;
    H->sym_epoch = h->struct_epoch;
    H->sym_n = n0;
    H->sym_nnz = nnz0;
    H->sym_general = general;
    H->sym_check = check_floating;
    H->sym_floating = *floating;
    memcpy(H->sym_stats, hs, sizeof H->sym_stats);
    return NODAL_OK;
}

int sagg_setup(nodal_ctx *h, bool *accepted, int32_t *floating) {
    return sagg_setup_csr(h, h->n, h->nnz, h->indptr.as<int32_t>(), h->indices.as<int32_t>(), h->data.as<double>(),
                          false, true, accepted, floating);
}

namespace {

int last_level(nodal_ctx *h, SHierarchy *H, int l, const double *b, double *out) {
    hipStream_t st = h->stream;
    SLevel *L = H->pool[l];
    const int64_t n = L->n;
    if (l == H->tail) return H->tail_dense ? tail_apply<1>(h, H, b, out) : tail_walk(h, H, b, out, 1);
    k_coarsest<<<grid_for(n), TB, 0, st>>>(n, H->dense_coarsest ? H->coarse_inv.as<double>() : nullptr,
                                           L->dinv.as<double>(), b, out);
    NODAL_HIP_TRY(h, hipGetLastError());
    return NODAL_OK;
}

void kcycle_schedule(SHierarchy *H, int it) {
    static const bool on = knob::SA_KFREEZE.now();
    H->kfrozen = false;
    H->kslot = -1;
    if (!on || it < 0) return;
    if (it == 0) H->ksamples = 0;
    const bool adaptive = it < 4 || (it & 3) == 0;
    if (!adaptive && H->ksamples > 0) {
        H->kfrozen = true;
    } else if (it >= 2) {
        H->kslot = H->ksamples % 3;
        ++H->ksamples;
        H->kcount = H->ksamples < 3 ? H->ksamples : 3;
    }
}

template <typename TBV, typename TOUT>
int cycle(nodal_ctx *h, SHierarchy *H, int l, const TBV *b, const cyc_t *x0, TOUT *out, const SolveBufs *sb) {
    hipStream_t st = h->stream;
    SLevel *L = H->pool[l];
    const int64_t n = L->n;
    SLevel *C = H->pool[l + 1];
    const int64_t nc = C->n;
    const Ell A = L->A();
    const double *dinv = L->dinv.as<double>();
    const cyc_t *x = x0;
    cyc_t *r = L->v<cyc_t>(V_R), *xp = L->v<cyc_t>(V_XP);
    const unsigned g = sb ? (unsigned)sb->g0 : grid_for(n);
    const unsigned tb = L->wfix ? TB : TB * LPR_RAGGED;
    const int nu = H->nu[l < 2 ? l : 2];
    const bool fold = L->fold && !(sb && nu == 1);
    auto hand_up = [&](const auto *c1, const auto *c2, const double *cf) {
        using TC = std::remove_cv_t<std::remove_pointer_t<decltype(c1)>>;
        if (!fold)
            k_prolong<TC><<<grid_for(n), TB, 0, st>>>(n, L->ld, L->pcol.as<int32_t>(), L->pvalf.as<float>(), x, c1, c2, cf, xp);
        else if (nu == 1)
            k_prolong_post<TC, TOUT><<<grid_for(n), TB, 0, st>>>(n, L->ld, L->wcol.as<int32_t>(), L->wval.as<float>(),
                                                               L->wlen.as<int32_t>(), x, r, dinv, c1, c2, cf, out);
        else
            k_prolong_post<TC, cyc_t><<<grid_for(n), TB, 0, st>>>(n, L->ld, L->wcol.as<int32_t>(), L->wval.as<float>(),
                                                                L->wlen.as<int32_t>(), x, r, dinv, c1, c2, cf, xp);
    };
    if (nu >= 2) {
        cyc_t *x1 = L->v<cyc_t>(V_X1);
        SAGG_DISPATCH_W(L->wfix, (k_post<W, false, TBV, cyc_t><<<g, tb, 0, st>>>(A, dinv, b, x0, x1, nullptr, nullptr, nullptr)));
        x = x1;
    }
    if (nu >= 3) {
        cyc_t *x2 = L->v<cyc_t>(V_T);
        SAGG_DISPATCH_W(L->wfix, (k_post<W, false, TBV, cyc_t><<<g, tb, 0, st>>>(A, dinv, b, x, x2, nullptr, nullptr, nullptr)));
        x = x2;
    }
    SAGG_DISPATCH_W(L->wfix, (k_smooth_residual<W, TBV><<<g, tb, 0, st>>>(A, b, x, r)));
    const bool last = l + 1 == H->tail || l + 1 == H->nlev - 1;
    const double *coef = nullptr;
    if (last) {
        double *rc = C->v<double>(V_RC), *c1 = C->v<double>(V_C1);
        k_restrict<double><<<grid_for(nc * RL), TB, 0, st>>>(nc, L->rld, L->rcol.as<int32_t>(), L->rvalf.as<float>(),
                                                            L->rlen.as<int32_t>(), r, rc, C->dinv.as<double>(), nullptr);
        NODAL_HIP_TRY(h, hipGetLastError());
        NODAL_TRY(last_level(h, H, l + 1, rc, c1));
        hand_up((const double *)c1, (const double *)nullptr, nullptr);
    } else {
        cyc_t *rc = C->v<cyc_t>(V_RC), *c1 = C->v<cyc_t>(V_C1), *c2 = C->v<cyc_t>(V_C2), *x0c = C->v<cyc_t>(V_X);
        k_restrict<cyc_t><<<grid_for(nc * RL), TB, 0, st>>>(nc, L->rld, L->rcol.as<int32_t>(), L->rvalf.as<float>(),
                                                           L->rlen.as<int32_t>(), r, rc, C->dinv.as<double>(), x0c);
        NODAL_HIP_TRY(h, hipGetLastError());
        int nparts = 0;
        const bool kcycle = l < H->klevels && H->kcycle;
        if (kcycle) {
            cyc_t *v1 = C->v<cyc_t>(V_V1), *v2 = C->v<cyc_t>(V_V2), *r2 = C->v<cyc_t>(V_R2);
            double *part = C->part.as<double>();
            const Ell Ac = C->A();
            const unsigned gd = grid_for(nc, DOT_BLOCKS);
            const unsigned tbc = C->wfix ? TB : TB * LPR_RAGGED;
            nparts = (int)gd;
            double *cf = part + 5 * DOT_BLOCKS;
            if (H->kfrozen && l == 0) {
                NODAL_TRY((cycle<cyc_t, cyc_t>(h, H, l + 1, rc, x0c, c1, nullptr)));
                SAGG_DISPATCH_W(C->wfix, (k_spmv_resid<W><<<gd, tbc, 0, st>>>(Ac, c1, rc, cf + 3, r2, C->dinv.as<double>(), x0c)));
                NODAL_HIP_TRY(h, hipGetLastError());
                NODAL_TRY((cycle<cyc_t, cyc_t>(h, H, l + 1, r2, x0c, c2, nullptr)));
                coef = cf + 3;
                nparts = 0;
            } else {
                NODAL_TRY((cycle<cyc_t, cyc_t>(h, H, l + 1, rc, x0c, c1, nullptr)));
                SAGG_DISPATCH_W(C->wfix, (k_spmv_dots<W><<<gd, tbc, 0, st>>>(Ac, c1, v1, rc, nullptr, part + 0 * DOT_BLOCKS,
                                                                            part + 1 * DOT_BLOCKS, nullptr)));
                k_second_residual<<<grid_for(nc), TB, 0, st>>>(nc, rc, v1, part, nparts, r2, C->dinv.as<double>(), x0c);
                NODAL_HIP_TRY(h, hipGetLastError());
                NODAL_TRY((cycle<cyc_t, cyc_t>(h, H, l + 1, r2, x0c, c2, nullptr)));
                SAGG_DISPATCH_W(C->wfix, (k_spmv_dots<W><<<gd, tbc, 0, st>>>(Ac, c2, v2, v1, r2, part + 3 * DOT_BLOCKS,
                                                                            part + 2 * DOT_BLOCKS, part + 4 * DOT_BLOCKS)));
                NODAL_HIP_TRY(h, hipGetLastError());
            }
        } else {
            NODAL_TRY((cycle<cyc_t, cyc_t>(h, H, l + 1, rc, x0c, c1, nullptr)));
        }
        if (nparts) {
            double *cf = C->part.as<double>() + 5 * DOT_BLOCKS;
            const bool sample = l == 0 && H->kslot >= 0;
            k_kcoef<<<1, 320, 0, st>>>(C->part.as<double>(), nparts, cf, sample ? H->kslot : -1, sample ? H->kcount : 0);
            coef = cf;
        }
        hand_up((const cyc_t *)c1, (const cyc_t *)c2, coef);
    }
    const cyc_t *cur = xp;
    const int left = fold ? nu - 1 : nu;
    if (left == 0) {
        NODAL_HIP_TRY(h, hipGetLastError());
        return NODAL_OK;
    }
    if (left >= 2) {
        cyc_t *mid = L->v<cyc_t>(V_T);
        SAGG_DISPATCH_W(L->wfix, (k_post<W, false, TBV, cyc_t><<<g, tb, 0, st>>>(A, dinv, b, cur, mid, nullptr, nullptr, nullptr)));
        cur = mid;
    }
    if (left >= 3) {
        cyc_t *mid2 = L->v<cyc_t>(V_X1);
        SAGG_DISPATCH_W(L->wfix, (k_post<W, false, TBV, cyc_t><<<g, tb, 0, st>>>(A, dinv, b, cur, mid2, nullptr, nullptr, nullptr)));
        cur = mid2;
    }
    if (sb) {
        SAGG_DISPATCH_W(L->wfix, (k_post<W, true, TBV, TOUT><<<g, tb, 0, st>>>(A, dinv, b, cur, out, sb->Ap, sb->part_rz,
                                                                              sb->part_zap)));
    } else {
        SAGG_DISPATCH_W(L->wfix, (k_post<W, false, TBV, TOUT><<<g, tb, 0, st>>>(A, dinv, b, cur, out, nullptr, nullptr, nullptr)));
    }
    NODAL_HIP_TRY(h, hipGetLastError());
    return NODAL_OK;
}

__global__ void f_set_scalars(double *__restrict__ sc, double tol2) {
    for (int k = 0; k < F_COUNT; ++k) sc[k] = 0.0;
    sc[F_TOL2] = tol2;
}

size_t align_up(size_t x) { return (x + 255) & ~(size_t)255; }

}

__global__ __launch_bounds__(TB) void k_x0(int64_t n, const double *__restrict__ dinv, const double *__restrict__ r,
                                           cyc_t *__restrict__ x0) {
    for (int64_t i = (int64_t)xcd_block() * TB + threadIdx.x; i < n; i += (int64_t)gridDim.x * TB)
        x0[i] = (cyc_t)(OMEGA * dinv[i] * r[i]);
}
bool sagg_ready(nodal_ctx *h, int64_t n) {
    SHierarchy *H = static_cast<SHierarchy *>(h->sagg);
    return H && H->ready && H->pool[0]->n == n;
}
void sagg_invalidate(nodal_ctx *h) {
    if (h->sagg) static_cast<SHierarchy *>(h->sagg)->ready = false;
}
int sagg_levels(nodal_ctx *h) { return h->sagg ? static_cast<SHierarchy *>(h->sagg)->nlev : 0; }

static SHierarchy *debug_hierarchy(nodal_ctx *h, nodal_ctx **owner) {
    for (nodal_ctx *c : {h, h->reduced}) {
        SHierarchy *H = c ? static_cast<SHierarchy *>(c->sagg) : nullptr;
        if (H && H->ready && H->nlev >= 1 && H->nlev <= MAX_LEVELS && (int)H->pool.size() >= H->nlev) {
            *owner = c;
            return H;
        }
    }
    return nullptr;
}

int sagg_debug_info(nodal_ctx *h, int32_t *nlev, int64_t *ints, double *reals) {
    nodal_ctx *c = nullptr;
    SHierarchy *H = debug_hierarchy(h, &c);
    if (!H) return nodal_fail(h, NODAL_E_INVALID, "debug hierarchy: the handle holds no ready hierarchy");
    *nlev = H->nlev;
    memset(ints, 0, sizeof(int64_t) * MAX_LEVELS * 16);
    memset(reals, 0, sizeof(double) * MAX_LEVELS * 2);
    for (int l = 0; l < H->nlev; ++l) {
        const SLevel *L = H->pool[l];
        const bool next = l + 1 < H->nlev;
        int64_t *w = ints + (size_t)l * 16;
        w[0] = L->n; w[1] = L->ld; w[2] = next ? L->nc : 0; w[3] = L->width; w[4] = L->maxlen; w[5] = L->wfix;
        w[6] = L->nnz; w[7] = next ? L->rld : 0; w[8] = next ? rcap_for(L->nc) : 0; w[9] = next ? L->wslots : 0;
        w[10] = next && L->fold_want; w[11] = next && L->fold; w[12] = L->d16; w[13] = H->tail >= 0 && l >= H->tail;
        w[14] = H->refreshed; w[15] = H->dense_coarsest;
        reals[(size_t)l * 2] = omega_p(l);
        reals[(size_t)l * 2 + 1] = OMEGA;
    }
    return NODAL_OK;
}

int sagg_debug_array(nodal_ctx *h, int32_t level, int32_t which, void *dst, int64_t capacity_bytes, int64_t *bytes_out) {
    nodal_ctx *c = nullptr;
    SHierarchy *H = debug_hierarchy(h, &c);
    if (!H) return nodal_fail(h, NODAL_E_INVALID, "debug hierarchy: the handle holds no ready hierarchy");
    const DevBuf *buf = nullptr;
    int64_t bytes = 0;
    if (level == -1) {
        const int64_t nl = H->pool[H->nlev - 1]->n;
        buf = &H->coarse_inv;
        bytes = H->dense_coarsest ? nl * nl * 8 : 0;
    } else {
        if (level < 0 || level >= H->nlev) return nodal_fail(h, NODAL_E_INVALID, "debug hierarchy: no such level");
        const SLevel *L = H->pool[level];
        const bool next = level + 1 < H->nlev;
        const int64_t slots = (int64_t)L->width * L->ld, pslots = next ? (int64_t)PW * L->ld : 0;
        const int64_t rslots = next ? (int64_t)rcap_for(L->nc) * L->rld : 0;
        const int64_t wslots = next && L->fold_want ? (int64_t)L->wslots * L->ld : 0;
        switch (which) {
        case NODAL_HA_ACOL: buf = &L->acol; bytes = slots * 4; break;
        case NODAL_HA_AVAL: buf = &L->aval; bytes = slots * 8; break;
        case NODAL_HA_AVALF: buf = &L->avalf; bytes = slots * 4; break;
        case NODAL_HA_ALEN: buf = &L->alen; bytes = L->n * 4; break;
        case NODAL_HA_DINV: buf = &L->dinv; bytes = L->n * 8; break;
        case NODAL_HA_ADCOL: buf = &L->adcol; bytes = L->d16 ? slots * 2 : 0; break;
        case NODAL_HA_AGG: buf = &L->agg; bytes = next ? L->n * 4 : 0; break;
        case NODAL_HA_PCOL: buf = &L->pcol; bytes = pslots * 4; break;
        case NODAL_HA_PVAL: buf = &L->pval; bytes = pslots * 8; break;
        case NODAL_HA_PVALF: buf = &L->pvalf; bytes = pslots * 4; break;
        case NODAL_HA_RCOL: buf = &L->rcol; bytes = rslots * 4; break;
        case NODAL_HA_RVAL: buf = &L->rval; bytes = rslots * 8; break;
        case NODAL_HA_RVALF: buf = &L->rvalf; bytes = rslots * 4; break;
        case NODAL_HA_RLEN: buf = &L->rlen; bytes = next ? L->nc * 4 : 0; break;
        case NODAL_HA_WCOL: buf = &L->wcol; bytes = wslots * 4; break;
        case NODAL_HA_WVAL: buf = &L->wval; bytes = wslots * 4; break;
        case NODAL_HA_WLEN: buf = &L->wlen; bytes = wslots ? L->n * 4 : 0; break;
        default: return nodal_fail(h, NODAL_E_INVALID, "debug hierarchy: no such array");
        }
    }
    if (bytes < 0 || (bytes > 0 && (!buf->p || (size_t)bytes > buf->cap)))
        return nodal_fail(h, NODAL_E_INVALID, "debug hierarchy: the level's buffer is smaller than its extent");
    *bytes_out = bytes;
    if (!dst || bytes == 0) return NODAL_OK;
    if (capacity_bytes < bytes) return nodal_fail(h, NODAL_E_INVALID, "debug hierarchy: destination too small");
    NODAL_WAIT_STREAM(h, c->stream);
    if (H->aux) NODAL_WAIT_STREAM(h, H->aux);
    NODAL_HIP_TRY(h, hipMemcpyAsync(dst, buf->p, (size_t)bytes, hipMemcpyDeviceToHost, c->stream));
    NODAL_WAIT_STREAM(h, c->stream);
    return NODAL_OK;
}

bool sagg_x0_slot(nodal_ctx *h, const double **dinv, nodal_cyc_t **x0, int64_t *n0, double *omega) {
    SHierarchy *H = static_cast<SHierarchy *>(h->sagg);
    if (!H || !H->ready) return false;
    SLevel *L0 = H->pool[0];
    *dinv = L0->dinv.as<double>();
    *x0 = L0->v<cyc_t>(V_X);
    *n0 = L0->n;
    *omega = OMEGA;
    return true;
}
int sagg_apply(nodal_ctx *h, const double *r, double *z, bool x0_ready, int it) {
    SHierarchy *H = static_cast<SHierarchy *>(h->sagg);
    if (!H || !H->ready) return nodal_fail(h, NODAL_E_INVALID, "sagg_setup_csr not called");
    SLevel *L0 = H->pool[0];
    cyc_t *x0 = L0->v<cyc_t>(V_X);
    if (!x0_ready) k_x0<<<grid_for(L0->n), TB, 0, h->stream>>>(L0->n, L0->dinv.as<double>(), r, x0);
    NODAL_HIP_TRY(h, hipGetLastError());
    kcycle_schedule(H, it);
    const int rc = cycle<double, double>(h, H, 0, r, x0, z, nullptr);
    H->kfrozen = false;
    H->kslot = -1;
    return rc;
}

int sagg_spmv(nodal_ctx *h, const double *x, double *y, hipEvent_t start, hipEvent_t stop) {
    SHierarchy *H = static_cast<SHierarchy *>(h->sagg);
    if (!H || !H->ready) return nodal_fail(h, NODAL_E_INVALID, "sagg_setup_csr not called");
    const SLevel *L0 = H->pool[0];
    const Ell A0 = L0->A();
    const unsigned tb0 = L0->wfix ? TB : TB * LPR_RAGGED;
    if (start && stop) {
        SAGG_DISPATCH_W(L0->wfix, (hipExtLaunchKernelGGL((k_ell_spmv<W>), dim3(grid_for(L0->n)), dim3(tb0), 0, h->stream,
                                                         start, stop, 0, A0, x, y)));
    } else {
        SAGG_DISPATCH_W(L0->wfix, (k_ell_spmv<W><<<grid_for(L0->n), tb0, 0, h->stream>>>(A0, x, y)));
    }
    NODAL_HIP_TRY(h, hipGetLastError());
    return NODAL_OK;
}

int sagg_fcg_solve(nodal_ctx *h, const double *b, bool do_setup, int32_t *info, int32_t *iters, double *resid) {
    static const bool trace = knob::TRACE.now();
    const int64_t n = h->n;
    hipStream_t st = h->stream;
    SHierarchy *H = hierarchy_of(h);
    if (do_setup) {
        bool accepted = false;
        int32_t floating = 0;
        NODAL_TRY(sagg_setup(h, &accepted, &floating));
        if (!accepted) return SAGG_DECLINED;
        if (floating) {
            *info = 1;
            *iters = 0;
            *resid = 0.0;
            return -2;
        }
    }
    if (!H->ready || H->pool[0]->n != n) return SAGG_DECLINED;
    h->amg_levels = H->nlev;
    static const int kc = knob::SA_KCYCLE.now();
    H->kcycle = kc != 0;
    H->klevels = knob::SA_KLEVELS.now();
    if (const char *e = knob::SA_NU.now()) {
        for (int k = 0; k < 3 && e[k] >= '1' && e[k] <= '3'; ++k) H->nu[k] = e[k] - '0';
    }

    const size_t vec = align_up((size_t)n * 8);
    NODAL_HIP_TRY(h, h->solver.reserve(6 * vec + 4 * MAX_PARTIALS * 8 + F_COUNT * 8 + 256));
    char *base = h->solver.as<char>();
    SolveBufs sb;
    sb.r = reinterpret_cast<double *>(base);
    sb.z = reinterpret_cast<cyc_t *>(base + vec);
    sb.p = reinterpret_cast<double *>(base + 2 * vec);
    sb.Ap = reinterpret_cast<double *>(base + 3 * vec);
    sb.x0 = reinterpret_cast<cyc_t *>(base + 4 * vec);
    sb.p2 = reinterpret_cast<double *>(base + 5 * vec);
    sb.part_rz = reinterpret_cast<double *>(base + 6 * vec);
    sb.part_zap = sb.part_rz + MAX_PARTIALS;
    sb.part_rr = sb.part_zap + MAX_PARTIALS;
    sb.part_pap = sb.part_rr + MAX_PARTIALS;
    sb.sc = sb.part_pap + MAX_PARTIALS;
    sb.g0 = (int)grid_for(n, MAX_PARTIALS);
    double *x = h->x.as<double>();
    const Ell A0 = H->pool[0]->A();

    const double tol = 1e-13;
    f_set_scalars<<<1, 1, 0, st>>>(sb.sc, tol * tol);
    const double *dinv0 = H->pool[0]->dinv.as<double>();
    f_init<<<sb.g0, TB, 0, st>>>(b, x, sb.r, sb.Ap, dinv0, sb.x0, sb.part_rr, n);
    NODAL_HIP_TRY(h, hipGetLastError());

    const int64_t maxit = knob::FCG_MAXIT.now().value_or(2000);
    hipEvent_t e0 = h->ev[2], e1 = h->ev[3];
    h->kern_ms = 0;
    h->kern_launches = 0;
    double hs[F_COUNT];
    int64_t enqueued = 0;
    int batch = 6;
    if (H->last_iters > 6 && (H->refreshed || !do_setup)) batch = H->last_iters + 1 > 32 ? 32 : H->last_iters + 1;
    else if (H->hint_iters > 8 && H->hint_n == n && H->hint_nnz == H->pool[0]->nnz) {
        batch = (3 * H->hint_iters) / 4;
        if (batch > 32) batch = 32;
    }
    int status = 0;
    const bool poll_partials = knob::FCG_HOST_SUM.now();
    double rr_prev = -1.0;
    int64_t it_prev = 0;
    int polls = 0;
    static const bool fuse_dir_env = knob::SA_FUSE_DIR.now();
    const bool fuse_dir = fuse_dir_env && LPR_RAGGED == 1;
    static const bool graphs_env = knob::SA_GRAPH.now();
    auto iteration = [&](int it, bool timed) -> int {
        kcycle_schedule(H, graphs_env ? -1 : it);
        struct KReset {
            SHierarchy *H;
            ~KReset() { H->kfrozen = false; H->kslot = -1; }
        } kreset{H};
        NODAL_TRY((cycle<double, cyc_t>(h, H, 0, sb.r, sb.x0, sb.z, &sb)));
        if (fuse_dir) {
            double *p_new = (it & 1) ? sb.p2 : sb.p;
            const double *p_old = (it & 1) ? sb.p : sb.p2;
            const unsigned tbf = TB;
            if (timed) {
                SAGG_DISPATCH_W(H->pool[0]->wfix, (hipExtLaunchKernelGGL((f_dir_spmv<W>), dim3(sb.g0), dim3(tbf), 0, st, e0, e1, 0,
                                                                         A0, (const cyc_t *)sb.z, p_old, p_new, sb.Ap,
                                                                         (const double *)sb.part_rz, (const double *)sb.part_zap,
                                                                         (const double *)sb.part_rr, sb.g0, sb.part_pap, sb.sc,
                                                                         it & 1)));
            } else {
                SAGG_DISPATCH_W(H->pool[0]->wfix, (f_dir_spmv<W><<<sb.g0, tbf, 0, st>>>(A0, sb.z, p_old, p_new, sb.Ap, sb.part_rz,
                                                                                       sb.part_zap, sb.part_rr, sb.g0,
                                                                                       sb.part_pap, sb.sc, it & 1)));
            }
            f_update<<<sb.g0, TB, 0, st>>>(x, sb.r, p_new, sb.Ap, sb.part_pap, sb.g0, dinv0, sb.x0, sb.part_rr, sb.sc, it & 1, n);
            NODAL_HIP_TRY(h, hipGetLastError());
            return NODAL_OK;
        }
        f_direction<<<sb.g0, TB, 0, st>>>(sb.z, sb.p, sb.part_rz, sb.part_zap, sb.part_rr, sb.g0, sb.sc, it & 1, n);
        const unsigned tb0 = H->pool[0]->wfix ? TB : TB * LPR_RAGGED;
        if (timed) {
            SAGG_DISPATCH_W(H->pool[0]->wfix, (hipExtLaunchKernelGGL((f_spmv<W>), dim3(sb.g0), dim3(tb0), 0, st, e0, e1, 0,
                                                                     A0, (const double *)sb.p, sb.Ap, sb.part_pap,
                                                                     (const double *)sb.sc, it & 1)));
        } else {
            SAGG_DISPATCH_W(H->pool[0]->wfix, (f_spmv<W><<<sb.g0, tb0, 0, st>>>(A0, sb.p, sb.Ap, sb.part_pap, sb.sc, it & 1)));
        }
        f_update<<<sb.g0, TB, 0, st>>>(x, sb.r, sb.p, sb.Ap, sb.part_pap, sb.g0, dinv0, sb.x0, sb.part_rr, sb.sc, it & 1, n);
        NODAL_HIP_TRY(h, hipGetLastError());
        return NODAL_OK;
    };
    static const bool graphs = knob::SA_GRAPH.now();
    if (graphs && (H->refreshed || !do_setup)) {
        uint64_t key = 1469598103934665603ull;
        auto mix = [&](uint64_t v) { key = (key ^ v) * 1099511628211ull; };
        mix((uint64_t)(uintptr_t)base); mix((uint64_t)(uintptr_t)x); mix((uint64_t)n); mix((uint64_t)sb.g0);
        mix((uint64_t)H->nlev); mix((uint64_t)(H->tail + 1)); mix((uint64_t)H->kcycle); mix((uint64_t)H->klevels);
        mix((uint64_t)(H->nu[0] * 100 + H->nu[1] * 10 + H->nu[2])); mix((uint64_t)H->td.lds_bytes);
        mix((uint64_t)(uintptr_t)H->tail_image.p); mix((uint64_t)(uintptr_t)H->coarse_inv.p);
        mix((uint64_t)(uintptr_t)(H->tail_dense ? H->tail_op.p : nullptr));
        for (int k = 0; k < H->nlev; ++k) {
            const SLevel *L = H->pool[k];
            const void *ps[] = {L->acol.p, L->aval.p, L->avalf.p, L->alen.p, L->dinv.p, L->pcol.p, L->pvalf.p,
                                L->rcol.p, L->rvalf.p, L->rlen.p, L->vec.p, L->part.p};
            for (const void *q : ps) mix((uint64_t)(uintptr_t)q);
            mix((uint64_t)(L->fold ? 1 + L->wslots : 0));
            if (L->fold) { mix((uint64_t)(uintptr_t)L->wcol.p); mix((uint64_t)(uintptr_t)L->wval.p); mix((uint64_t)(uintptr_t)L->wlen.p); }
            mix((uint64_t)L->n); mix((uint64_t)L->ld); mix((uint64_t)L->wfix); mix((uint64_t)L->rld);
        }
        if (H->it_exec && H->it_key != key) H->drop_graph();
        if (!H->it_exec) {
            hipGraph_t g = nullptr;
            hipGraphExec_t ex = nullptr;
            if (hipStreamBeginCapture(st, hipStreamCaptureModeThreadLocal) == hipSuccess) {
                int cs = iteration(0, false);
                if (cs == NODAL_OK) cs = iteration(1, false);
                const hipError_t ce = hipStreamEndCapture(st, &g);
                if (cs == NODAL_OK && ce == hipSuccess && g && hipGraphInstantiate(&ex, g, nullptr, nullptr, 0) == hipSuccess) {
                    H->it_graph = g;
                    H->it_exec = ex;
                    H->it_key = key;
                } else {
                    if (g) (void)hipGraphDestroy(g);
                    (void)hipGetLastError();
                }
            } else {
                (void)hipGetLastError();
            }
        }
    } else if (H->it_exec && do_setup) {
        H->drop_graph();
    }
    while (status == 0) {
        for (int c = 0; c < batch;) {
            if (H->it_exec && c > 0 && c + 1 < batch && (enqueued & 1) == 0) {
                NODAL_HIP_TRY(h, hipGraphLaunch(H->it_exec, st));
                c += 2;
                enqueued += 2;
            } else {
                NODAL_TRY(iteration((int)enqueued, c == 0));
                ++c;
                ++enqueued;
            }
        }
        double rr_now = -1.0;
        {
            const size_t bytes = (size_t)(2 * MAX_PARTIALS + F_COUNT) * 8;
            double *stage = poll_partials ? static_cast<double *>(nodal_pinned_arena(h, bytes)) : nullptr;
            if (stage) {
                NODAL_HIP_TRY(h, hipMemcpyAsync(stage, sb.part_rr, bytes, hipMemcpyDeviceToHost, st));
                NODAL_WAIT_STREAM(h, st);
                memcpy(hs, stage + 2 * MAX_PARTIALS, F_COUNT * 8);
                double acc = 0.0;
                for (int k = 0; k < sb.g0; ++k) acc += stage[k];
                rr_now = acc;
            } else {
                NODAL_TRY(nodal_read_words(h, hs, sb.sc, F_COUNT * 8));
            }
        }
        ++polls;
        bool conv = hs[F_CONV + ((enqueued - 1) & 1)] != 0.0;
        bool host_conv = false;
        if (!conv && rr_now >= 0.0 && hs[F_FLAG] == 0.0 && hs[F_BB] > 0.0 && rr_now <= tol * tol * hs[F_BB]) {
            host_conv = true;
            hs[F_RR] = rr_now;
            hs[F_ITERS] = (double)enqueued;
        } else if (!conv && rr_now >= 0.0) {
            hs[F_RR] = rr_now;
        }
        float ms = 0;
        if (!(conv && !host_conv && hs[F_ITERS] <= (double)(enqueued - batch)) && hipEventElapsedTime(&ms, e0, e1) == hipSuccess) {
            h->kern_ms += ms;
            h->kern_launches += 1;
        }
        if (hs[F_FLAG] != 0.0 || !(hs[F_RR] == hs[F_RR])) status = 2;
        else if (conv || host_conv) status = 1;
        else if (enqueued >= maxit) status = 3;
        else {
            int next = 2;
            const double target = tol * tol * hs[F_BB];
            const double rr_ref = rr_prev > 0.0 ? rr_prev : hs[F_BB];
            const int64_t it_ref = rr_prev > 0.0 ? it_prev : 0;
            if (hs[F_RR] > 0.0 && hs[F_RR] < rr_ref && enqueued > it_ref) {
                const double rate = log(hs[F_RR] / rr_ref) / (double)(enqueued - it_ref);
                static const double look = knob::FCG_LOOK.now();
                next = (int)floor(look * log(target / hs[F_RR]) / rate);
            }
            if (next > enqueued) next = (int)enqueued;
            batch = next < 1 ? 1 : (next > 32 ? 32 : next);
            rr_prev = hs[F_RR];
            it_prev = enqueued;
        }
    }
    const int64_t its = status == 1 ? (int64_t)hs[F_ITERS] : enqueued;
    *iters = (int32_t)its;
    *resid = hs[F_BB] > 0 ? sqrt(hs[F_RR] / hs[F_BB]) : 0.0;
    const SLevel *L0 = H->pool[0];
    h->kern_alg = 12.0 * (double)L0->nnz + 4.0 * (double)n + 16.0 * (double)n;
    if (fuse_dir) h->kern_alg += 12.0 * (double)n;
    if (trace)
        fprintf(stderr, "[sagg] %d iterations (%lld enqueued, %d polls), relative residual %.2e, status %d\n", *iters,
                (long long)enqueued, polls, *resid, status);
    if (trace && H->tail >= 0 && H->td.stamps && !H->tail_dense) {
        long long ts[64];
        if (hipMemcpy(ts, H->td.stamps, sizeof ts, hipMemcpyDeviceToHost) == hipSuccess) {
            fprintf(stderr, "[sagg] tail phases (us):");
            for (int k = 1; k < (int)ts[63] && k < 63; ++k) fprintf(stderr, " %.2f", (double)(ts[k] - ts[k - 1]) * 0.01);
            fprintf(stderr, "  total %.2f, image %d B, lds %d B\n", (double)(ts[ts[63] - 1] - ts[0]) * 0.01,
                    H->td.image_bytes, H->td.lds_bytes);
            for (int k = 0; k < H->td.nlev; ++k)
                fprintf(stderr, "[sagg]   tail level %d: n %d width %d lpr %d nq %d\n", k, H->td.lv[k].n,
                        H->td.lv[k].width, H->td.lv[k].lpr, H->td.lv[k].nq);
        }
    }
    if (status != 1) {
        H->last_iters = 0;
        return -1;
    }
    H->last_iters = (int)its;
    H->hint_iters = (int)its;
    H->hint_n = n;
    H->hint_nnz = H->pool[0]->nnz;
    *info = 0;
    return NODAL_OK;
}

#include "sagg_multi.h"
```

nodal_amd/csrc/sagg_cycle.h:

```cpp
#pragma once

namespace {

constexpr int LPR_RAGGED = 1;
template <int W> struct RowLanes { static constexpr int value = W == 0 ? LPR_RAGGED : 1; };

template <class VT, class XF>
__device__ __forceinline__ double ell_row_lanes(const Ell &A, const VT *__restrict__ val, int64_t i, int sub, XF xf) {
    constexpr int Q = 8;
    const int32_t len = A.len[i];
    double acc = 0.0;
    for (int32_t s0 = sub; s0 < len; s0 += LPR_RAGGED * Q) {
        int32_t c[Q];
        double v[Q];
        if (A.dcol) {
#pragma unroll
            for (int q = 0; q < Q; ++q) {
                const bool ok = s0 + q * LPR_RAGGED < len;
                const int64_t at = (int64_t)(ok ? s0 + q * LPR_RAGGED : s0) * A.ld + i;
                c[q] = (int32_t)i + (int32_t)A.dcol[at];
                const VT loaded = val[at];
                v[q] = ok ? (double)loaded : 0.0;
            }
        } else {
// ... 390 lines not shown
        const cyc_t vs = (cyc_t)sd;
        v[i] = vs;
        const double s = (double)vs, ci = (double)c[i];
        a0 = fma(ci, s, a0);
        a1 = fma(ci, (double)u1[i], a1);
        if (u2) a2 = fma(ci, (double)u2[i], a2);
    }
    a0 = block_sum<NT>(a0);
    a1 = block_sum<NT>(a1);
    a2 = block_sum<NT>(a2);
    if (threadIdx.x == 0) {
        p_cv[blockIdx.x] = a0;
        p_cu1[blockIdx.x] = a1;
        if (p_cu2) p_cu2[blockIdx.x] = a2;
    }
}

__global__ __launch_bounds__(TB) void k_second_residual(int64_t n, const cyc_t *__restrict__ rc,
                                                        const cyc_t *__restrict__ v1,
                                                        const double *__restrict__ part, int nparts,
                                                        cyc_t *__restrict__ r2, const double *__restrict__ dinv,
                                                        cyc_t *__restrict__ x0) {
    double rho1, alpha1, unused;
    reduce_partials3(part + 0 * DOT_BLOCKS, part + 1 * DOT_BLOCKS, nullptr, nparts, rho1, alpha1, unused);
    const double t = rho1 > 0.0 ? alpha1 / rho1 : 0.0;
    for (int64_t i = (int64_t)xcd_block() * TB + threadIdx.x; i < n; i += (int64_t)gridDim.x * TB)
    {
        const double v = fma(-t, (double)v1[i], (double)rc[i]);
        r2[i] = (cyc_t)v;
        x0[i] = (cyc_t)(OMEGA * dinv[i] * v);
    }
}

__global__ __launch_bounds__(TB) void k_coarsest(int64_t n, const double *__restrict__ inv,
                                                 const double *__restrict__ dinv, const double *__restrict__ b,
                                                 double *__restrict__ out) {
    for (int64_t i = (int64_t)xcd_block() * TB + threadIdx.x; i < n; i += (int64_t)gridDim.x * TB) {
        double s = 0.0;
        if (inv)
            for (int64_t j = 0; j < n; ++j) s = fma(inv[i * n + j], b[j], s);
        else
            s = dinv[i] * b[i];
        out[i] = s;
    }
}



__device__ __forceinline__ double lds_row(const double *aval, const uint16_t *acol, int n, int width, int i,
                                          int sub, int lpr, const double *x) {
    double s0 = 0.0, s1 = 0.0;
    int t = sub;
    for (; t + 3 * lpr < width; t += 4 * lpr) {
        const double v0 = aval[t * n + i], v1 = aval[(t + lpr) * n + i], v2 = aval[(t + 2 * lpr) * n + i],
                     v3 = aval[(t + 3 * lpr) * n + i];
        const int c0 = acol[t * n + i], c1 = acol[(t + lpr) * n + i], c2 = acol[(t + 2 * lpr) * n + i],
                  c3 = acol[(t + 3 * lpr) * n + i];
        s0 = fma(v0, x[c0], s0);
        s1 = fma(v1, x[c1], s1);
        s0 = fma(v2, x[c2], s0);
        s1 = fma(v3, x[c3], s1);
    }
    for (; t < width; t += lpr) s0 = fma(aval[t * n + i], x[acol[t * n + i]], s0);
    double s = s0 + s1;
    for (int off = lpr >> 1; off > 0; off >>= 1) s += __shfl_xor(s, off, 64);
    return s;
}

__global__ __launch_bounds__(1024) void k_tail_pack(TailDesc d, char *__restrict__ image) {
    const int tid = threadIdx.x;
    const int last = d.nlev - 1;
    auto f64 = [&](int off) { return reinterpret_cast<double *>(image + off); };
    auto u16 = [&](int off) { return reinterpret_cast<uint16_t *>(image + off); };
    auto copy_f64 = [&](double *dst, const double *src, int rows, int64_t ld, int slots) {
        for (int e = tid; e < rows * slots; e += 1024) {
            const int t = e / rows, i = e - t * rows;
            dst[e] = src[(int64_t)t * ld + i];
        }
    };
    auto copy_u16 = [&](uint16_t *dst, const int32_t *src, int rows, int64_t ld, int slots) {
        for (int e = tid; e < rows * slots; e += 1024) {
            const int t = e / rows, i = e - t * rows;
            const int32_t v = src[(int64_t)t * ld + i];
            dst[e] = (uint16_t)(v < 0 ? 0 : v);
        }
    };
    for (int k = 0; k < last; ++k) {
        const TailLevelDesc &L = d.lv[k];
        for (int e = tid; e < L.n * L.width; e += 1024) {
            const int t = e / L.n, i = e - t * L.n;
            const bool in = t < L.alen[i];
            f64(L.o_aval)[e] = in ? L.aval[(int64_t)t * L.ld + i] : 0.0;
            const int32_t c = in ? L.acol[(int64_t)t * L.ld + i] : 0;
            u16(L.o_acol)[e] = (uint16_t)(c < 0 ? 0 : c);
        }
        copy_f64(f64(L.o_dinv), L.dinv, L.n, L.ld, 1);
        copy_f64(f64(L.o_pval), L.pval, L.n, L.ld, PW);
        copy_u16(u16(L.o_pcol), L.pcol, L.n, L.ld, PW);
        copy_f64(f64(L.o_rval), L.rval, L.nc * RL, (int64_t)L.rld * RL, L.nq);
        copy_u16(u16(L.o_rcol), L.rcol, L.nc * RL, (int64_t)L.rld * RL, L.nq);
    }
    const TailLevelDesc &L = d.lv[last];
    if (d.inv) copy_f64(f64(L.o_aval), d.inv, L.n * L.n, L.n * L.n, 1);
    else copy_f64(f64(L.o_aval), L.dinv, L.n, L.n, 1);
}

template <int SLOTS>
__device__ __forceinline__ double reg_row(const double (&v)[SLOTS], const uint32_t (&c)[SLOTS / 2], int lpr,
                                          const double *x) {
    double s0 = 0.0, s1 = 0.0;
#pragma unroll
    for (int j = 0; j < SLOTS; j += 2) {
        s0 = fma(v[j], x[c[j / 2] & 0xffffu], s0);
        s1 = fma(v[j + 1], x[c[j / 2] >> 16], s1);
    }
    double s = s0 + s1;
    for (int off = lpr >> 1; off > 0; off >>= 1) s += __shfl_xor(s, off, 64);
    return s;
}

template <int SLOTS, bool UNIT>
__device__ __forceinline__ void tail_cycle(const TailDesc &d, char *smem, const char *__restrict__ image,
                                           const double *__restrict__ rc, double *__restrict__ out, int vs, int voff) {
    const int tid = threadIdx.x;
    const int last = d.nlev - 1;
    const int TAIL_NU = d.nu;
    auto f64 = [&](int off) { return reinterpret_cast<double *>(smem + (off - d.skip)); };
    auto u16 = [&](int off) { return reinterpret_cast<uint16_t *>(smem + (off - d.skip)); };
    int stamp_no = 0;
    auto stamp = [&]() {
        if (!UNIT && d.stamps && tid == 0) d.stamps[stamp_no] = wall_clock64();
        ++stamp_no;
    };
    stamp();
    double v0[SLOTS];
    uint32_t c0[SLOTS / 2];
    {
        const TailLevelDesc &L = d.lv[0];
        const double *aval = reinterpret_cast<const double *>(image + L.o_aval);
        const uint16_t *acol = reinterpret_cast<const uint16_t *>(image + L.o_acol);
        const int lpr = L.lpr, sub = tid & (lpr - 1), i = tid / lpr, ii = i < L.n ? i : L.n - 1;
        const bool row = last > 0 && i < L.n;
#pragma unroll
        for (int j = 0; j < SLOTS; j += 2) {
            const int ta = sub + j * lpr, tb = ta + lpr;
            const bool ha = row && ta < L.width, hb = row && tb < L.width;
            const int ea = ha ? ta * L.n + ii : 0, eb = hb ? tb * L.n + ii : 0;
            const double va = aval[ea], vb = aval[eb];
            const uint32_t ca = acol[ea], cb = acol[eb];
            v0[j] = ha ? va : 0.0;
            v0[j + 1] = hb ? vb : 0.0;
            c0[j / 2] = (ha ? ca : 0u) | ((hb ? cb : 0u) << 16);
        }
    }
    {
        constexpr int FLY = (TAIL_LDS_BUDGET / 16 + 1023) / 1024;
        const int4 *src = reinterpret_cast<const int4 *>(image + d.skip);
        int4 *dst = reinterpret_cast<int4 *>(smem);
        const int pieces = (d.image_bytes - d.skip) / 16;
        int4 v[FLY];
#pragma unroll
        for (int u = 0; u < FLY; ++u) v[u] = src[tid + u * 1024 < pieces ? tid + u * 1024 : 0];
#pragma unroll
        for (int u = 0; u < FLY; ++u)
            if (tid + u * 1024 < pieces) dst[tid + u * 1024] = v[u];
    }
    for (;;) {
        for (int i = tid; i < d.lv[0].n; i += 1024)
            f64(d.lv[0].o_B)[i] = UNIT ? (i == voff ? 1.0 : 0.0) : rc[(int64_t)i * vs + voff];
        __syncthreads();
        stamp();
        for (int k = 0; k < last; ++k) {
            const TailLevelDesc &L = d.lv[k];
            const double *aval = f64(L.o_aval), *dinv = f64(L.o_dinv), *B = f64(L.o_B);
            const uint16_t *acol = u16(L.o_acol);
            double *X = f64(L.o_X), *Y = f64(L.o_Y), *R = f64(L.o_R);
            const int lpr = L.lpr, sub = tid & (lpr - 1), rows = 1024 / lpr;
            for (int i = tid; i < L.n; i += 1024) X[i] = OMEGA * dinv[i] * B[i];
            __syncthreads();
            for (int sweep = 1; sweep < TAIL_NU; ++sweep) {
                for (int i0 = 0; i0 < L.n; i0 += rows) {
                    const int i = i0 + tid / lpr, ii = i < L.n ? i : L.n - 1;
                    const double ax = k == 0 ? reg_row<SLOTS>(v0, c0, lpr, X)
                                             : lds_row(aval, acol, L.n, L.width, ii, sub, lpr, X);
                    if (i < L.n && sub == 0) Y[i] = fma(OMEGA * dinv[i], B[i] - ax, X[i]);
                }
                __syncthreads();
                double *t = X; X = Y; Y = t;
            }
            for (int i0 = 0; i0 < L.n; i0 += rows) {
                const int i = i0 + tid / lpr, ii = i < L.n ? i : L.n - 1;
                const double ax = k == 0 ? reg_row<SLOTS>(v0, c0, lpr, X)
                                         : lds_row(aval, acol, L.n, L.width, ii, sub, lpr, X);
                if (i < L.n && sub == 0) R[i] = B[i] - ax;
            }
            __syncthreads();
            stamp();
            const double *rval = f64(L.o_rval);
            const uint16_t *rcol = u16(L.o_rcol);
            double *Bc = f64(d.lv[k + 1].o_B);
            for (int I0 = 0; I0 < L.nc; I0 += 1024 / RL) {
                const int I = I0 + tid / RL, r8 = tid & (RL - 1);
                double s = 0.0;
                if (I < L.nc) {
                    double s1 = 0.0;
                    const int e0 = I * RL + r8, step = L.nc * RL;
                    int q = 0;
                    for (; q + 3 < L.nq; q += 4) {
                        const int ea = e0 + q * step, eb = ea + step, ec = eb + step, ed = ec + step;
                        const double va = rval[ea], vb = rval[eb], vc = rval[ec], vd = rval[ed];
                        const int ca = rcol[ea], cb = rcol[eb], cc = rcol[ec], cd = rcol[ed];
                        s = fma(va, R[ca], s);
                        s1 = fma(vb, R[cb], s1);
                        s = fma(vc, R[cc], s);
                        s1 = fma(vd, R[cd], s1);
                    }
                    for (; q < L.nq; ++q) s = fma(rval[e0 + q * step], R[rcol[e0 + q * step]], s);
                    s += s1;
                }
#pragma unroll
                for (int off = RL >> 1; off > 0; off >>= 1) s += __shfl_xor(s, off, 64);
                if (I < L.nc && r8 == 0) Bc[I] = s;
            }
            __syncthreads();
            stamp();
        }
        {
            const TailLevelDesc &L = d.lv[last];
            const double *inv = f64(L.o_aval), *B = f64(L.o_B);
            double *E = f64(L.o_X);
            for (int i = tid; i < L.n; i += 1024) {
                double s = 0.0;
                if (d.inv) {
                    double s1 = 0.0, s2 = 0.0, s3 = 0.0;
                    const double *row = inv + i * L.n;
                    int j = 0;
                    for (; j + 3 < L.n; j += 4) {
                        s = fma(row[j], B[j], s);
                        s1 = fma(row[j + 1], B[j + 1], s1);
                        s2 = fma(row[j + 2], B[j + 2], s2);
                        s3 = fma(row[j + 3], B[j + 3], s3);
                    }
                    for (; j < L.n; ++j) s = fma(row[j], B[j], s);
                    s = (s + s1) + (s2 + s3);
                } else {
                    s = inv[i] * B[i];
                }
                E[i] = s;
            }
            __syncthreads();
            stamp();
        }
        const double *Ec = f64(d.lv[last].o_X);
        for (int k = last - 1; k >= 0; --k) {
            const TailLevelDesc &L = d.lv[k];
            const double *aval = f64(L.o_aval), *dinv = f64(L.o_dinv), *B = f64(L.o_B), *pval = f64(L.o_pval);
            const uint16_t *acol = u16(L.o_acol), *pcol = u16(L.o_pcol);
            double *X = f64((TAIL_NU & 1) ? L.o_X : L.o_Y), *Y = f64((TAIL_NU & 1) ? L.o_Y : L.o_X);
            for (int i = tid; i < L.n; i += 1024) {
                double s = X[i];
#pragma unroll
                for (int q = 0; q < PW; ++q) s = fma(pval[q * L.n + i], Ec[pcol[q * L.n + i]], s);
                Y[i] = s;
            }
            __syncthreads();
            stamp();
            const int lpr = L.lpr, sub = tid & (lpr - 1), rows = 1024 / lpr;
            for (int sweep = 0; sweep < TAIL_NU; ++sweep) {
                for (int i0 = 0; i0 < L.n; i0 += rows) {
                    const int i = i0 + tid / lpr, ii = i < L.n ? i : L.n - 1;
                    const double ax = k == 0 ? reg_row<SLOTS>(v0, c0, lpr, Y)
                                             : lds_row(aval, acol, L.n, L.width, ii, sub, lpr, Y);
                    if (i < L.n && sub == 0) X[i] = fma(OMEGA * dinv[i], B[i] - ax, Y[i]);
                }
                __syncthreads();
                double *t = X; X = Y; Y = t;
            }
            Ec = Y;
            stamp();
        }
        for (int i = tid; i < d.lv[0].n; i += 1024) out[(int64_t)i * vs + voff] = Ec[i];
        stamp();
        voff += (int)gridDim.x;
        if (!UNIT || voff >= d.lv[0].n) break;
        __syncthreads();
    }
    if (!UNIT && d.stamps && tid == 0) d.stamps[63] = stamp_no;
}

template <int SLOTS>
__global__ __launch_bounds__(1024) void k_tail(TailDesc d, const char *__restrict__ image,
                                               const double *__restrict__ rc, double *__restrict__ out, int vs) {
    extern __shared__ __attribute__((aligned(16))) char smem[];
    tail_cycle<SLOTS, false>(d, smem, image, rc, out, vs, vs > 1 ? (int)blockIdx.x : 0);
}

template <int SLOTS>
__global__ __launch_bounds__(1024) void k_tail_pack_op(TailDesc d, const char *__restrict__ image,
                                                       double *__restrict__ T) {
    extern __shared__ __attribute__((aligned(16))) char smem[];
    tail_cycle<SLOTS, true>(d, smem, image, nullptr, T, d.lv[0].n, (int)blockIdx.x);
}

template <int CH, int NV>
__global__ __launch_bounds__(256) void k_tail_apply(int n, const double *__restrict__ T,
                                                    const double *__restrict__ rc, double *__restrict__ out) {
    const int lane = threadIdx.x & 63;
    const int i = (int)blockIdx.x * 4 + (threadIdx.x >> 6);
    if (i >= n) return;
    const double *row = T + (int64_t)i * n;
    double t[CH];
#pragma unroll
    for (int u = 0; u < CH; ++u) {
        const int j = lane + 64 * u;
        t[u] = row[j < n ? j : 0];
    }
    if constexpr (NV == 1) {
        double r[CH];
#pragma unroll
        for (int u = 0; u < CH; ++u) {
            const int j = lane + 64 * u;
            r[u] = rc[j < n ? j : 0];
        }
        double s0 = 0.0, s1 = 0.0;
#pragma unroll
        for (int u = 0; u < CH; u += 2) {
            if (lane + 64 * u < n && t[u] != 0.0) s0 = fma(t[u], r[u], s0);
            if (lane + 64 * (u + 1) < n && t[u + 1] != 0.0) s1 = fma(t[u + 1], r[u + 1], s1);
        }
        const double s = wave_sum(s0 + s1);
        if (lane == 0) out[i] = s;
    } else {
        double s[NV];
#pragma unroll
        for (int c = 0; c < NV; ++c) s[c] = 0.0;
#pragma unroll
        for (int u = 0; u < CH; ++u) {
            const int j = lane + 64 * u;
            const double *rj = rc + (int64_t)(j < n ? j : 0) * NV;
            const bool use = j < n && t[u] != 0.0;
#pragma unroll
            for (int c = 0; c < NV; ++c) {
                const double v = rj[c];
                if (use) s[c] = fma(t[u], v, s[c]);
            }
        }
#pragma unroll
        for (int c = 0; c < NV; ++c) {
            const double v = wave_sum(s[c]);
            if (lane == 0) out[(int64_t)i * NV + c] = v;
        }
    }
}

enum { F_RZ = 0, F_ALPHA = 2, F_CONV = 4, F_RR = 6, F_BB = 7, F_FLAG = 8, F_ITERS = 9, F_TOL2 = 10,
       F_ITNO = 12,
       F_COUNT = 16 };
constexpr int MAX_PARTIALS = 1024;

__global__ __launch_bounds__(TB) void f_init(const double *__restrict__ b, double *__restrict__ x,
                                             double *__restrict__ r, double *__restrict__ Ap,
                                             const double *__restrict__ dinv, cyc_t *__restrict__ x0,
                                             double *__restrict__ part_rr, int64_t n) {
    double srr = 0.0;
    for (int64_t i = (int64_t)xcd_block() * TB + threadIdx.x; i < n; i += (int64_t)gridDim.x * TB) {
        const double ri = b[i];
        x[i] = 0.0;
        r[i] = ri;
        x0[i] = (cyc_t)(OMEGA * dinv[i] * ri);
        Ap[i] = 0.0;
        srr = fma(ri, ri, srr);
    }
    srr = block_sum(srr);
    if (threadIdx.x == 0) part_rr[blockIdx.x] = srr;
}

__global__ __launch_bounds__(TB) void f_direction(const cyc_t *__restrict__ z, double *__restrict__ p,
                                                  const double *__restrict__ part_rz,
                                                  const double *__restrict__ part_zap,
                                                  const double *__restrict__ part_rr, int nparts,
                                                  double *__restrict__ sc, int parity, int64_t n) {
    const int cur = parity & 1, prev = cur ^ 1;
    constexpr int FD_PRE = 4;
    const int64_t i0 = (int64_t)xcd_block() * TB + threadIdx.x, stride = (int64_t)gridDim.x * TB;
    cyc_t zq[FD_PRE];
    double pq[FD_PRE];
#pragma unroll
    for (int u = 0; u < FD_PRE; ++u) {
        const int64_t i = i0 + u * stride, ii = i < n ? i : n - 1;
        zq[u] = z[ii];
        pq[u] = p[ii];
    }
    const int iter = (int)sc[F_ITNO + prev];
    if (blockIdx.x == 0 && threadIdx.x == 0) sc[F_ITNO + cur] = (double)(iter + 1);
    if (iter > 0 && sc[F_CONV + prev] != 0.0) {
        if (blockIdx.x == 0 && threadIdx.x == 0) sc[F_CONV + cur] = 1.0;
        return;
    }
    double rz_new, zap, rr;
    reduce_partials3(part_rz, part_zap, part_rr, nparts, rz_new, zap, rr);
    const double rz_old = iter > 0 ? sc[F_RZ + prev] : 1.0;
    const double beta = (iter > 0 && rz_old != 0.0) ? -sc[F_ALPHA + prev] * zap / rz_old : 0.0;
    const double bb = iter == 0 ? rr : sc[F_BB];
    const bool bad = !(rz_new >= 0.0) || !(rr == rr);
    const bool converged = bb == 0.0 || rr <= sc[F_TOL2] * bb || bad;
    if (blockIdx.x == 0 && threadIdx.x == 0) {
        sc[F_RZ + cur] = rz_new;
        sc[F_RR] = rr;
        if (iter == 0) sc[F_BB] = rr;
        if (bad) sc[F_FLAG] = 1.0;
        sc[F_CONV + cur] = converged ? 1.0 : 0.0;
        if (converged) sc[F_ITERS] = (double)iter;
    }
    if (converged) return;
#pragma unroll
    for (int u = 0; u < FD_PRE; ++u) {
        const int64_t i = i0 + u * stride;
        if (i < n) p[i] = iter > 0 ? fma(beta, pq[u], (double)zq[u]) : (double)zq[u];
    }
    for (int64_t i = i0 + FD_PRE * stride; i < n; i += stride)
        p[i] = iter > 0 ? fma(beta, p[i], (double)z[i]) : (double)z[i];
}

template <int W>
__global__ __launch_bounds__(TB * RowLanes<W>::value) void k_ell_spmv(Ell A, const double *__restrict__ x,
                                                                      double *__restrict__ y) {
    constexpr int LPR = RowLanes<W>::value, NT = TB * LPR;
    const int sub = threadIdx.x & (LPR - 1);
    for (int64_t t = (int64_t)xcd_block() * NT + threadIdx.x; t / LPR < A.n; t += (int64_t)gridDim.x * NT) {
        const int64_t i = t / LPR;
        const double s = ell_row_w<W>(A, A.val, i, sub, [&](int32_t j) { return x[j]; });
        if (sub == 0) y[i] = s;
    }
}

template <int W>
__global__ __launch_bounds__(TB * RowLanes<W>::value) void f_spmv(Ell A, const double *__restrict__ p, double *__restrict__ Ap,
                                             double *__restrict__ part_pap, const double *__restrict__ sc,
                                             int iter) {
    if (sc[F_CONV + (iter & 1)] != 0.0) return;
    double acc = 0.0;
    constexpr int LPR = RowLanes<W>::value, NT = TB * LPR;
    const int sub = threadIdx.x & (LPR - 1);
    for (int64_t t = (int64_t)xcd_block() * NT + threadIdx.x; t / LPR < A.n; t += (int64_t)gridDim.x * NT) {
        const int64_t i = t / LPR;
        const double s = ell_row_w<W>(A, A.val, i, sub, [&](int32_t j) { return p[j]; });
        if (sub != 0) continue;
        Ap[i] = s;
        acc = fma(p[i], s, acc);
    }
    acc = block_sum<NT>(acc);
    if (threadIdx.x == 0) part_pap[blockIdx.x] = acc;
}

template <int W>
__global__ __launch_bounds__(TB * RowLanes<W>::value) void f_dir_spmv(Ell A, const cyc_t *__restrict__ z,
                                                 const double *__restrict__ p_old, double *__restrict__ p_new,
                                                 double *__restrict__ Ap, const double *__restrict__ part_rz,
                                                 const double *__restrict__ part_zap, const double *__restrict__ part_rr,
                                                 int nparts, double *__restrict__ part_pap, double *__restrict__ sc,
                                                 int parity) {
    static_assert(RowLanes<W>::value == 1, "the reduction of the partials assumes TB threads");
    const int cur = parity & 1, prev = cur ^ 1;
    const int64_t i0 = (int64_t)xcd_block() * TB + threadIdx.x, stride = (int64_t)gridDim.x * TB;
    int32_t c0[W > 0 ? W : 1];
    double v0[W > 0 ? W : 1];
    const int64_t ifirst = i0 < A.n ? i0 : A.n - 1;
    if constexpr (W > 0) ell_row_load<W>(A, A.val, ifirst, c0, v0);
    const cyc_t zfirst = z[ifirst];
    const double pfirst = p_old[ifirst];
    const int iter = (int)sc[F_ITNO + prev];
    if (blockIdx.x == 0 && threadIdx.x == 0) sc[F_ITNO + cur] = (double)(iter + 1);
    if (iter > 0 && sc[F_CONV + prev] != 0.0) {
        if (blockIdx.x == 0 && threadIdx.x == 0) sc[F_CONV + cur] = 1.0;
        return;
    }
    double rz_new, zap, rr;
    reduce_partials3(part_rz, part_zap, part_rr, nparts, rz_new, zap, rr);
    const double rz_old = iter > 0 ? sc[F_RZ + prev] : 1.0;
    const double beta = (iter > 0 && rz_old != 0.0) ? -sc[F_ALPHA + prev] * zap / rz_old : 0.0;
    const double bb = iter == 0 ? rr : sc[F_BB];
    const bool bad = !(rz_new >= 0.0) || !(rr == rr);
    const bool converged = bb == 0.0 || rr <= sc[F_TOL2] * bb || bad;
    if (blockIdx.x == 0 && threadIdx.x == 0) {
        sc[F_RZ + cur] = rz_new;
        sc[F_RR] = rr;
        if (iter == 0) sc[F_BB] = rr;
        if (bad) sc[F_FLAG] = 1.0;
        sc[F_CONV + cur] = converged ? 1.0 : 0.0;
        if (converged) sc[F_ITERS] = (double)iter;
    }
    if (converged) return;
    const bool first = iter == 0;
    auto pn = [&](int32_t j) { return first ? (double)z[j] : fma(beta, p_old[j], (double)z[j]); };
    double acc = 0.0;
    for (int64_t i = i0; i < A.n; i += stride) {
        double s, pi;
        if (W > 0 && i == i0) {
            s = ell_row_sum<W>(i, c0, v0, pn);
            pi = first ? (double)zfirst : fma(beta, pfirst, (double)zfirst);
        } else {
            s = ell_row_w<W>(A, A.val, i, 0, pn);
            pi = pn((int32_t)i);
        }
        p_new[i] = pi;
        Ap[i] = s;
        acc = fma(pi, s, acc);
    }
    acc = block_sum<TB>(acc);
    if (threadIdx.x == 0) part_pap[blockIdx.x] = acc;
}

__global__ __launch_bounds__(TB) void f_update(double *__restrict__ x, double *__restrict__ r,
                                               const double *__restrict__ p, const double *__restrict__ Ap,
                                               const double *__restrict__ part_pap, int nparts,
                                               const double *__restrict__ dinv, cyc_t *__restrict__ x0,
                                               double *__restrict__ part_rr, double *__restrict__ sc, int iter,
                                               int64_t n) {
    const int cur = iter & 1;
    constexpr int FU_PRE = 4;
    const int64_t i0 = (int64_t)xcd_block() * TB + threadIdx.x, stride = (int64_t)gridDim.x * TB;
    double xq[FU_PRE], rq[FU_PRE], pq[FU_PRE], aq[FU_PRE], dq[FU_PRE];
#pragma unroll
    for (int u = 0; u < FU_PRE; ++u) {
        const int64_t i = i0 + u * stride, ii = i < n ? i : n - 1;
        xq[u] = x[ii];
        rq[u] = r[ii];
        pq[u] = p[ii];
        aq[u] = Ap[ii];
        dq[u] = dinv[ii];
    }
    if (sc[F_CONV + cur] != 0.0) return;
    const double pap = reduce_partials(part_pap, nparts);
    const double rz = sc[F_RZ + cur];
    const bool bad = !(pap > 0.0) && rz != 0.0;
    const double alpha = (pap > 0.0) ? rz / pap : 0.0;
    if (blockIdx.x == 0 && threadIdx.x == 0) {
        sc[F_ALPHA + cur] = alpha;
        if (bad) sc[F_FLAG] = 1.0;
    }
    double srr = 0.0;
#pragma unroll
    for (int u = 0; u < FU_PRE; ++u) {
        const int64_t i = i0 + u * stride;
        if (i < n) {
            x[i] = fma(alpha, pq[u], xq[u]);
            const double ri = fma(-alpha, aq[u], rq[u]);
            r[i] = ri;
            x0[i] = (cyc_t)(OMEGA * dq[u] * ri);
            srr = fma(ri, ri, srr);
        }
    }
    for (int64_t i = i0 + FU_PRE * stride; i < n; i += stride) {
        x[i] = fma(alpha, p[i], x[i]);
        const double ri = fma(-alpha, Ap[i], r[i]);
        r[i] = ri;
        x0[i] = (cyc_t)(OMEGA * dinv[i] * ri);
        srr = fma(ri, ri, srr);
    }
    srr = block_sum(srr);
    if (threadIdx.x == 0) part_rr[blockIdx.x] = srr;
}

}
```

Baseline: 163.0 circuits/s.

## Fuse last-level smoothing, restriction and dense tail solve into three launches

```diff
diff --git a/include/nodal_hip.h b/include/nodal_hip.h
--- a/include/nodal_hip.h
+++ b/include/nodal_hip.h
@@ -174,7 +174,8 @@
 enum {
     NODAL_HA_ACOL = 0, NODAL_HA_AVAL = 1, NODAL_HA_AVALF = 2, NODAL_HA_ALEN = 3, NODAL_HA_DINV = 4, NODAL_HA_ADCOL = 5,
     NODAL_HA_AGG = 6, NODAL_HA_PCOL = 7, NODAL_HA_PVAL = 8, NODAL_HA_PVALF = 9, NODAL_HA_RCOL = 10, NODAL_HA_RVAL = 11,
-    NODAL_HA_RVALF = 12, NODAL_HA_RLEN = 13, NODAL_HA_WCOL = 14, NODAL_HA_WVAL = 15, NODAL_HA_WLEN = 16
+    NODAL_HA_RVALF = 12, NODAL_HA_RLEN = 13, NODAL_HA_WCOL = 14, NODAL_HA_WVAL = 15, NODAL_HA_WLEN = 16,
+    NODAL_HA_P2COL = 17, NODAL_HA_P2VAL = 18, NODAL_HA_P2LEN = 19, NODAL_HA_D2 = 20
 };
 int nodal_debug_hierarchy_info(nodal_handle h, int32_t *nlev, int64_t *ints , double *reals );
 int nodal_debug_hierarchy_array(nodal_handle h, int32_t level, int32_t which, void *dst, int64_t capacity_bytes,
diff --git a/nodal_amd/_ffi.py b/nodal_amd/_ffi.py
--- a/nodal_amd/_ffi.py
+++ b/nodal_amd/_ffi.py
@@ -87,7 +87,8 @@
                     ("dinv", np.float64), ("adcol", np.int16), ("agg", np.int32), ("pcol", np.int32),
                     ("pval", np.float64), ("pvalf", np.float32), ("rcol", np.int32), ("rval", np.float64),
                     ("rvalf", np.float32), ("rlen", np.int32), ("wcol", np.int32), ("wval", np.float32),
-                    ("wlen", np.int32))
+                    ("wlen", np.int32), ("p2col", np.int32), ("p2val", np.float32), ("p2len", np.int32),
+                    ("d2", np.float32))
 HIERARCHY_INFO = ("n", "ld", "nc", "width", "maxlen", "wfix", "nnz", "rld", "rcap", "wslots", "fold_want", "fold", "d16",
                   "in_tail", "refreshed", "dense_coarsest")
 
diff --git a/nodal_amd/csrc/knobs.h b/nodal_amd/csrc/knobs.h
--- a/nodal_amd/csrc/knobs.h
+++ b/nodal_amd/csrc/knobs.h
@@ -117,6 +117,9 @@
 inline constexpr OffUnlessNon0 SA_GRAPH{"NODAL_SA_GRAPH"};
 inline constexpr Text SA_FOLD_POST{"NODAL_SA_FOLD_POST"};
 inline constexpr OffUnlessNon0 SA_FOLD_CHECK{"NODAL_SA_FOLD_CHECK"};
+inline constexpr OnUnless0 SA_FOLD_VISIT{"NODAL_SA_FOLD_VISIT"};
+inline constexpr Int64 SA_VISIT_CAP{"NODAL_SA_VISIT_CAP", 16777216};
+inline constexpr OffUnlessNon0 SA_VISIT_CHECK{"NODAL_SA_VISIT_CHECK"};
 inline constexpr OnUnless0 SA_TAIL_DENSE{"NODAL_SA_TAIL_DENSE"};
 inline constexpr OffUnlessNon0 SA_TAIL_CHECK{"NODAL_SA_TAIL_CHECK"};
 inline constexpr Int SA_TAIL_NU{"NODAL_SA_TAIL_NU", 3};
diff --git a/nodal_amd/csrc/sagg.hip b/nodal_amd/csrc/sagg.hip
--- a/nodal_amd/csrc/sagg.hip
+++ b/nodal_amd/csrc/sagg.hip
@@ -62,7 +62,8 @@
        ST_MAXR = 6, ST_NC = 7 ,
        ST_FARCOL = 8 ,
        ST_FOLDMISS = 9 ,
-       ST_COUNT = 10 };
+       ST_VISITMISS = 10 ,
+       ST_COUNT = 11 };
 
 struct SLevel {
     int64_t n = 0, ld = 0, nc = 0;
@@ -81,6 +82,8 @@
     DevBuf wcol, wval, wlen;
     int32_t wslots = 0;
     bool fold_want = false, fold = false;
+    DevBuf p2col, p2val, p2len, d2;
+    bool visit_want = false, visit = false;
     Ell A() const {
         Ell e;
         e.n = n; e.ld = ld; e.width = width;
@@ -173,7 +176,7 @@
         for (SLevel *l : pool) {
             DevBuf *b[] = {&l->acol, &l->aval, &l->alen, &l->dinv, &l->agg, &l->pcol, &l->pval, &l->rcol,
                            &l->rval, &l->rlen, &l->vec, &l->part, &l->gflag, &l->avalf, &l->pvalf, &l->rvalf, &l->adcol,
-                           &l->wcol, &l->wval, &l->wlen};
+                           &l->wcol, &l->wval, &l->wlen, &l->p2col, &l->p2val, &l->p2len, &l->d2};
             for (DevBuf *x : b) x->release();
             delete l;
         }
@@ -1228,6 +1231,11 @@
             fprintf(stderr, "[sagg] level %d (%lld rows): first post-smoothing sweep %s\n", k, (long long)L->n,
                     miss ? "NOT folded: a row of A P lacks a column of its P row (no stored diagonal)"
                          : "folded into the prolongation");
+        const bool wide = hs[(size_t)k * ST_COUNT + ST_VISITMISS] != 0;
+        L->visit = L->visit_want && L->fold && !wide;
+        if (trace && L->visit_want)
+            fprintf(stderr, "[sagg] level %d (%lld rows): visit %s\n", k, (long long)L->n,
+                    L->visit ? "in three launches" : "NOT in three launches: W missing, or a row of P2 beyond its slots");
     }
 }
 
@@ -1521,6 +1529,146 @@
     H->tail_dense = true;
     static const bool check = knob::TRACE.now() && knob::SA_TAIL_CHECK.now();
     if (check) NODAL_TRY(tail_self_check(h, H));
+    return NODAL_OK;
+}
+
+constexpr int P2LIST = 1024;
+__global__ __launch_bounds__(64) void p2_rows_wave(Ell A, const double *__restrict__ dinv, const int32_t *__restrict__ wcol,
+                                                   const float *__restrict__ wval, const int32_t *__restrict__ wlen,
+                                                   int32_t *__restrict__ p2col, float *__restrict__ p2val,
+                                                   int32_t *__restrict__ p2len, unsigned long long *__restrict__ stats) {
+    __shared__ int32_t lJ[P2LIST];
+    __shared__ double lV[P2LIST];
+    __shared__ uint32_t mask[TAIL_MAX_N / 32];
+    __shared__ int32_t cols[P2CAP];
+    static_assert(TAIL_MAX_N / 32 <= 64, "one lane per word of the column mask");
+    const int lane = threadIdx.x;
+    bool overflow = false;
+    for (int64_t i = blockIdx.x; i < A.n; i += gridDim.x) {
+        if (lane < TAIL_MAX_N / 32) mask[lane] = 0u;
+        const int32_t total = A.len[i] + 1;
+        const double wd = -OMEGA * dinv[i];
+        int np = 0;
+        bool fits = true;
+        for (int32_t g0 = 0; g0 < total; g0 += 64) {
+            const int32_t src = g0 + lane;
+            const bool has = src < total;
+            const int32_t su = has && src >= 1 ? src - 1 : 0;
+            const int32_t ka = A.col[(int64_t)su * A.ld + i];
+            const double a = A.val[(int64_t)su * A.ld + i];
+            const int32_t k = src == 0 ? (int32_t)i : ka;
+            const double cf = src == 0 ? 1.0 : wd * a;
+            const int32_t lk = wlen[k];
+            const int32_t len = has ? lk : 0;
+            int tot = 0;
+            int o = np + wave_excl_scan(len, &tot);
+            if (np + tot > P2LIST) {
+                fits = false;
+                break;
+            }
+            constexpr int SQ = 8;
+            for (int32_t s0 = 0; s0 < len; s0 += SQ) {
+                int32_t cj[SQ];
+                float cv[SQ];
+#pragma unroll
+                for (int q = 0; q < SQ; ++q) {
+                    const int32_t s = s0 + q < len ? s0 + q : s0;
+                    cj[q] = wcol[(int64_t)s * A.ld + k];
+                    cv[q] = wval[(int64_t)s * A.ld + k];
+                }
+#pragma unroll
+                for (int q = 0; q < SQ; ++q)
+                    if (s0 + q < len) {
+                        lJ[o] = cj[q];
+                        lV[o] = cf * (double)cv[q];
+                        ++o;
+                    }
+            }
+            np += tot;
+        }
+        __syncthreads();
+        if (fits)
+            for (int p = lane; p < np; p += 64) atomicOr(&mask[lJ[p] >> 5], 1u << (lJ[p] & 31));
+        __syncthreads();
+        uint32_t m = lane < TAIL_MAX_N / 32 ? mask[lane] : 0u;
+        int distinct = 0;
+        int at = wave_excl_scan(__popc(m), &distinct);
+        if (!fits || distinct > P2CAP) {
+            overflow = true;
+            if (lane == 0) p2len[i] = 0;
+            __syncthreads();
+            continue;
+        }
+        while (m) {
+            cols[at++] = lane * 32 + (__ffs(m) - 1);
+            m &= m - 1u;
+        }
+        __syncthreads();
+        if (lane < distinct) {
+            const int32_t c = cols[lane];
+            double acc = 0.0;
+#pragma unroll 8
+            for (int p = 0; p < np; ++p) {
+                const int32_t j = lJ[p];
+                const double v = lV[p];
+                if (j == c) acc += v;
+            }
+            p2col[(int64_t)lane * A.ld + i] = c;
+            p2val[(int64_t)lane * A.ld + i] = (float)acc;
+        }
+        if (lane == 0) p2len[i] = distinct;
+        __syncthreads();
+    }
+    if (overflow) stats[ST_VISITMISS] = 1ull;
+}
+
+__global__ __launch_bounds__(TB) void d2_zero(float4 *__restrict__ d, int64_t pieces) {
+    for (int64_t e = (int64_t)blockIdx.x * TB + threadIdx.x; e < pieces; e += (int64_t)gridDim.x * TB)
+        d[e] = make_float4(0.0f, 0.0f, 0.0f, 0.0f);
+}
+
+__global__ __launch_bounds__(TB) void d2_scatter(int64_t n, int64_t ld, const int32_t *__restrict__ p2col,
+                                                 const float *__restrict__ p2val, const int32_t *__restrict__ p2len,
+                                                 float *__restrict__ d2) {
+    for (int64_t e = (int64_t)blockIdx.x * TB + threadIdx.x; e < (int64_t)P2CAP * ld; e += (int64_t)gridDim.x * TB) {
+        const int64_t s = e / ld, i = e - s * ld;
+        if (i >= n || s >= p2len[i]) continue;
+        d2[(int64_t)p2col[e] * ld + i] = p2val[e];
+    }
+}
+
+void apply_nu_knob(SHierarchy *H) {
+    if (const char *e = knob::SA_NU.now()) {
+        for (int k = 0; k < 3 && e[k] >= '1' && e[k] <= '3'; ++k) H->nu[k] = e[k] - '0';
+    }
+}
+
+int build_visit(nodal_ctx *h, SHierarchy *H, bool general) {
+    static const bool on = knob::SA_FOLD_VISIT.now();
+    static const int64_t cap = knob::SA_VISIT_CAP.now();
+    for (int k = 0; k < H->nlev; ++k) H->pool[k]->visit_want = H->pool[k]->visit = false;
+    if (!on || general || H->tail < 2 || !H->tail_dense) return NODAL_OK;
+    const int l = H->tail - 1;
+    SLevel *L = H->pool[l];
+    apply_nu_knob(H);
+    const int64_t nt = H->pool[H->tail]->n;
+    if (H->nu[l < 2 ? l : 2] != 2 || !L->fold_want || nt > TAIL_MAX_N || nt * L->ld * 4 > cap) return NODAL_OK;
+    hipStream_t st = h->stream;
+    NODAL_HIP_TRY(h, L->p2col.reserve((size_t)P2CAP * L->ld * 4 + 64));
+    NODAL_HIP_TRY(h, L->p2val.reserve((size_t)P2CAP * L->ld * 4 + 64));
+    NODAL_HIP_TRY(h, L->p2len.reserve((size_t)L->ld * 4 + 64));
+    NODAL_HIP_TRY(h, L->d2.reserve((size_t)nt * L->ld * 4 + 64));
+    Ell A = L->A();
+    const unsigned gl = (unsigned)(L->n < 8192 ? L->n : 8192);
+    p2_rows_wave<<<gl, 64, 0, st>>>(A, L->dinv.as<double>(), L->wcol.as<int32_t>(), L->wval.as<float>(), L->wlen.as<int32_t>(),
+                                  L->p2col.as<int32_t>(), L->p2val.as<float>(), L->p2len.as<int32_t>(),
+                                  H->stats.as<unsigned long long>() + (size_t)l * ST_COUNT);
+    NODAL_HIP_TRY(h, hipGetLastError());
+    d2_zero<<<grid_for(nt * L->ld / 4), TB, 0, st>>>(L->d2.as<float4>(), nt * L->ld / 4);
+    d2_scatter<<<grid_for((int64_t)P2CAP * L->ld), TB, 0, st>>>(L->n, L->ld, L->p2col.as<int32_t>(), L->p2val.as<float>(),
+                                                                 L->p2len.as<int32_t>(), L->d2.as<float>());
+    NODAL_HIP_TRY(h, hipGetLastError());
+    L->visit_want = true;
     return NODAL_OK;
 }
 
@@ -1586,6 +1734,7 @@
                     "(worst row against its own bound: %.3e)\n", l, (long long)n, (int)L->wslots, (int)L->maxlen, dm, qm);
     return NODAL_OK;
 }
+int visit_self_check(nodal_ctx *h, SHierarchy *H);
 int fold_self_check(nodal_ctx *h, SHierarchy *H) {
     static const bool check = knob::TRACE.now() && knob::SA_FOLD_CHECK.now();
     if (!check) return NODAL_OK;
@@ -1728,6 +1877,7 @@
     if (H->tail >= 0) k_tail_pack<<<1, 1024, 0, st>>>(H->td, H->tail_image.as<char>());
     NODAL_HIP_TRY(h, hipGetLastError());
     NODAL_TRY(form_tail_op(h, H));
+    NODAL_TRY(build_visit(h, H, general));
     NODAL_HIP_TRY(h, hipMemcpyAsync(hs, dstats, (size_t)MAX_LEVELS * ST_COUNT * 8, hipMemcpyDeviceToHost, st));
     NODAL_WAIT_STREAM(h, st);
     const int64_t bar = n0 / 100 < 32 ? (n0 / 100 > 0 ? n0 / 100 : 1) : 32;
@@ -1736,6 +1886,7 @@
         if (hs[(size_t)k * ST_COUNT + ST_BADDIAG] || hs[(size_t)k * ST_COUNT + ST_OVERFLOW]) return NODAL_OK;
     decide_folds(H, hs, false);
     NODAL_TRY(fold_self_check(h, H));
+    NODAL_TRY(visit_self_check(h, H));
     *ok = true;
     return NODAL_OK;
 }
@@ -1919,6 +2070,7 @@
         NODAL_HIP_TRY(h, L->part.reserve(5 * DOT_BLOCKS * 8 + 512));
     }
     NODAL_TRY(build_tail(h, H, hs));
+    NODAL_TRY(build_visit(h, H, general));
 
     if (!check_floating) {
         NODAL_HIP_TRY(h, hipMemcpyAsync(hs, dstats, (size_t)MAX_LEVELS * ST_COUNT * 8, hipMemcpyDeviceToHost, st));
@@ -1947,6 +2099,7 @@
     }
     decide_folds(H, hs, trace);
     NODAL_TRY(fold_self_check(h, H));
+    NODAL_TRY(visit_self_check(h, H));
     H->ready = true;
     *accepted = true;
     H->sym_valid = true;
@@ -1992,6 +2145,24 @@
         ++H->ksamples;
         H->kcount = H->ksamples < 3 ? H->ksamples : 3;
     }
+}
+
+int visit_three(nodal_ctx *h, SHierarchy *H, int l, const cyc_t *b, const cyc_t *x0, cyc_t *out) {
+    hipStream_t st = h->stream;
+    SLevel *L = H->pool[l], *C = H->pool[l + 1];
+    const Ell A = L->A();
+    const double *dinv = L->dinv.as<double>();
+    cyc_t *x1 = L->v<cyc_t>(V_X1), *x2 = L->v<cyc_t>(V_T);
+    double *rc = C->v<double>(V_RC), *c1 = C->v<double>(V_C1);
+    const int nt = (int)C->n;
+    const unsigned g = grid_for(L->n);
+    SAGG_DISPATCH_W(L->wfix, (k_visit_first<W><<<g + (unsigned)nt, TB, 0, st>>>(A, dinv, b, x0, x1, g, L->d2.as<float>(), rc)));
+    SAGG_DISPATCH_W(L->wfix, (k_visit_second<W><<<g + (unsigned)((nt + 3) / 4), TB, 0, st>>>(A, dinv, b, x1, x2, g, nt,
+                                                                                             H->tail_op.as<double>(), rc, c1)));
+    SAGG_DISPATCH_W(L->wfix, (k_visit_last<W><<<grid_for(L->n * VL), TB, 0, st>>>(A, dinv, b, x2, out, L->p2col.as<int32_t>(), L->p2val.as<float>(),
+                                                                L->p2len.as<int32_t>(), c1)));
+    NODAL_HIP_TRY(h, hipGetLastError());
+    return NODAL_OK;
 }
 
 template <typename TBV, typename TOUT>
@@ -2009,7 +2180,10 @@
     const unsigned tb = L->wfix ? TB : TB * LPR_RAGGED;
     const int nu = H->nu[l < 2 ? l : 2];
     const bool fold = L->fold && !(sb && nu == 1);
-    auto hand_up = [&](const auto *c1, const auto *c2, const double *cf) {
+    if constexpr (std::is_same_v<TBV, cyc_t> && std::is_same_v<TOUT, cyc_t>) {
+        if (L->visit && !sb && nu == 2 && l + 1 == H->tail && H->tail_dense) return visit_three(h, H, l, b, x0, out);
+    }
+    auto hand_up =[&](const auto *c1, const auto *c2, const double *cf) {
         using TC = std::remove_cv_t<std::remove_pointer_t<decltype(c1)>>;
         if (!fold)
             k_prolong<TC><<<grid_for(n), TB, 0, st>>>(n, L->ld, L->pcol.as<int32_t>(), L->pvalf.as<float>(), x, c1, c2, cf, xp);
@@ -2117,6 +2291,140 @@
 
 size_t align_up(size_t x) { return (x + 255) & ~(size_t)255; }
 
+int visit_check_level(nodal_ctx *h, SHierarchy *H, int l) {
+    hipStream_t st = h->stream;
+    SLevel *L = H->pool[l], *C = H->pool[l + 1];
+    const int64_t n = L->n, ld = L->ld, nt = C->n;
+    uint64_t seed = 0x9e3779b97f4a7c15ull + 977ull * (uint64_t)l;
+    auto unit = [&]() {
+        uint64_t z = (seed += 0x9e3779b97f4a7c15ull);
+        z = (z ^ (z >> 30)) * 0xbf58476d1ce4e5b9ull;
+        z = (z ^ (z >> 27)) * 0x94d049bb133111ebull;
+        z ^= z >> 31;
+        return (double)(z >> 11) * (1.0 / 4503599627370496.0) - 1.0;
+    };
+    std::vector<double> dinv((size_t)n), T((size_t)nt * nt), c6((size_t)nt), c3((size_t)nt);
+    std::vector<cyc_t> hb((size_t)n), hx0((size_t)n), x1((size_t)n), x2((size_t)n), r((size_t)n), xp((size_t)n),
+        o6((size_t)n), o3((size_t)n);
+    std::vector<int32_t> acol((size_t)L->width * ld), alen((size_t)n), pcol((size_t)PW * ld), wcol((size_t)L->wslots * ld),
+        wlen((size_t)n), p2col((size_t)P2CAP * ld), p2len((size_t)n);
+    std::vector<float> aval((size_t)L->width * ld), pval((size_t)PW * ld), wval((size_t)L->wslots * ld),
+        p2val((size_t)P2CAP * ld);
+    auto down = [&](void *dst, const void *src, size_t bytes) { return hipMemcpy(dst, src, bytes, hipMemcpyDeviceToHost); };
+    hipError_t e = hipStreamSynchronize(st);
+    if (e == hipSuccess) e = down(dinv.data(), L->dinv.p, (size_t)n * 8);
+    for (int64_t i = 0; i < n; ++i) {
+        hb[i] = (cyc_t)unit();
+        hx0[i] = (cyc_t)(OMEGA * dinv[i] * (double)hb[i]);
+    }
+    const size_t vb = align256((size_t)n * sizeof(cyc_t));
+    DevBuf buf;
+    if (e == hipSuccess) e = buf.reserve(4 * vb);
+    char *p = buf.as<char>();
+    cyc_t *b = reinterpret_cast<cyc_t *>(p), *x0 = reinterpret_cast<cyc_t *>(p + vb), *out6 = reinterpret_cast<cyc_t *>(p + 2 * vb),
+          *out3 = reinterpret_cast<cyc_t *>(p + 3 * vb);
+    if (e == hipSuccess) e = hipMemcpyAsync(b, hb.data(), (size_t)n * sizeof(cyc_t), hipMemcpyHostToDevice, st);
+    if (e == hipSuccess) e = hipMemcpyAsync(x0, hx0.data(), (size_t)n * sizeof(cyc_t), hipMemcpyHostToDevice, st);
+    int rc = NODAL_OK;
+    if (e == hipSuccess) {
+        L->visit = false;
+        rc = cycle<cyc_t, cyc_t>(h, H, l, b, x0, out6, nullptr);
+        L->visit = true;
+    }
+    if (e == hipSuccess && rc == NODAL_OK) e = hipStreamSynchronize(st);
+    if (e == hipSuccess) e = down(r.data(), L->v<cyc_t>(V_R), (size_t)n * sizeof(cyc_t));
+    if (e == hipSuccess) e = down(xp.data(), L->v<cyc_t>(V_XP), (size_t)n * sizeof(cyc_t));
+    if (e == hipSuccess) e = down(c6.data(), C->v<double>(V_C1), (size_t)nt * 8);
+    if (e == hipSuccess && rc == NODAL_OK) rc = cycle<cyc_t, cyc_t>(h, H, l, b, x0, out3, nullptr);
+    if (e == hipSuccess && rc == NODAL_OK) e = hipStreamSynchronize(st);
+    if (e == hipSuccess) e = down(x1.data(), L->v<cyc_t>(V_X1), (size_t)n * sizeof(cyc_t));
+    if (e == hipSuccess) e = down(x2.data(), L->v<cyc_t>(V_T), (size_t)n * sizeof(cyc_t));
+    if (e == hipSuccess) e = down(c3.data(), C->v<double>(V_C1), (size_t)nt * 8);
+    if (e == hipSuccess) e = down(o6.data(), out6, (size_t)n * sizeof(cyc_t));
+    if (e == hipSuccess) e = down(o3.data(), out3, (size_t)n * sizeof(cyc_t));
+    if (e == hipSuccess) e = down(acol.data(), L->acol.p, acol.size() * 4);
+    if (e == hipSuccess) e = down(aval.data(), L->avalf.p, aval.size() * 4);
+    if (e == hipSuccess) e = down(alen.data(), L->alen.p, (size_t)n * 4);
+    if (e == hipSuccess) e = down(pcol.data(), L->pcol.p, pcol.size() * 4);
+    if (e == hipSuccess) e = down(pval.data(), L->pvalf.p, pval.size() * 4);
+    if (e == hipSuccess) e = down(wcol.data(), L->wcol.p, wcol.size() * 4);
+    if (e == hipSuccess) e = down(wval.data(), L->wval.p, wval.size() * 4);
+    if (e == hipSuccess) e = down(wlen.data(), L->wlen.p, (size_t)n * 4);
+    if (e == hipSuccess) e = down(p2col.data(), L->p2col.p, p2col.size() * 4);
+    if (e == hipSuccess) e = down(p2val.data(), L->p2val.p, p2val.size() * 4);
+    if (e == hipSuccess) e = down(p2len.data(), L->p2len.p, (size_t)n * 4);
+    if (e == hipSuccess) e = down(T.data(), H->tail_op.p, (size_t)nt * nt * 8);
+    buf.release();
+    if (rc != NODAL_OK) return rc;
+    NODAL_HIP_TRY(h, e);
+    using Vec = std::vector<double>;
+    auto absv = [](const auto &v) { Vec y(v.size()); for (size_t i = 0; i < v.size(); ++i) y[i] = fabs((double)v[i]); return y; };
+    auto add = [](Vec a, const Vec &b2) { for (size_t i = 0; i < a.size(); ++i) a[i] += b2[i]; return a; };
+    auto wd = [&](Vec v) { for (int64_t i = 0; i < n; ++i) v[i] *= OMEGA * dinv[i]; return v; };
+    auto absA = [&](const Vec &v) {
+        Vec y((size_t)n, 0.0);
+        for (int64_t i = 0; i < n; ++i)
+            for (int32_t s = 0; s < alen[i]; ++s) y[i] += fabs((double)aval[(size_t)s * ld + i]) * v[acol[(size_t)s * ld + i]];
+        return y;
+    };
+    auto absG = [&](const Vec &v) { return add(v, wd(absA(v))); };
+    auto absGT = [&](const Vec &v) { return add(v, absA(wd(v))); };
+    auto ell = [&](int slots, const std::vector<int32_t> &col, const std::vector<float> &val, const std::vector<int32_t> *len,
+                   const Vec &v, bool transposed) {
+        Vec y((size_t)(transposed ? nt : n), 0.0);
+        for (int64_t i = 0; i < n; ++i) {
+            const int32_t m = len ? (*len)[i] : slots;
+            for (int32_t s = 0; s < m; ++s) {
+                const int32_t J = col[(size_t)s * ld + i];
+                if (J < 0) continue;
+                const double a = fabs((double)val[(size_t)s * ld + i]);
+                if (transposed) y[J] += a * v[i];
+                else y[i] += a * v[J];
+            }
+        }
+        return y;
+    };
+    auto absT = [&](const Vec &v) {
+        Vec y((size_t)nt, 0.0);
+        for (int64_t i = 0; i < nt; ++i)
+            for (int64_t j = 0; j < nt; ++j) y[i] += fabs(T[(size_t)i * nt + j]) * v[j];
+        return y;
+    };
+    auto Pt = [&](const Vec &v) { return ell(PW, pcol, pval, nullptr, v, true); };
+    auto Wm = [&](const Vec &v) { return ell(L->wslots, wcol, wval, &wlen, v, false); };
+    auto Wt = [&](const Vec &v) { return ell(L->wslots, wcol, wval, &wlen, v, true); };
+    auto P2m = [&](const Vec &v) { return ell(P2CAP, p2col, p2val, &p2len, v, false); };
+    auto P2t = [&](const Vec &v) { return ell(P2CAP, p2col, p2val, &p2len, v, true); };
+    const Vec ax1 = absA(absv(x1));
+    const Vec e_r = add(absv(r), ax1);
+    const Vec e_c6 = absT(Pt(add(absv(r), e_r)));
+    const Vec e_xp = add(add(absv(xp), wd(e_r)), add(Wm(absv(c6)), Wm(e_c6)));
+    const Vec dev6 = add(add(absv(o6), absG(e_xp)), wd(absA(absv(xp))));
+    const Vec e_x2 = add(absv(x2), wd(ax1));
+    const Vec e_c3 = absT(add(P2t(absv(hb)), Wt(absGT(absv(hb)))));
+    const Vec ac3 = absv(c3);
+    const Vec dev3 = add(add(add(absv(o3), absG(e_x2)), wd(absA(absv(x2)))), add(add(P2m(ac3), absG(Wm(ac3))), P2m(e_c3)));
+    double dm = 0.0;
+    int maxp2 = 0;
+    for (int64_t i = 0; i < n; ++i) {
+        const double di = fabs((double)o3[i] - (double)o6[i]) / (dev6[i] + dev3[i]);
+        dm = !(di <= dm) ? di : dm;
+        maxp2 = p2len[i] > maxp2 ? p2len[i] : maxp2;
+    }
+    fprintf(stderr, "[sagg] visit check: level %d, rows %lld, n_t %lld, longest P2 row %d, three launches against the six "
+                    "d = %.3e (against the bound 2^-23: %.3e)\n", l, (long long)n, (long long)nt, maxp2, dm, dm / 0x1p-23);
+    return NODAL_OK;
+}
+int visit_self_check(nodal_ctx *h, SHierarchy *H) {
+    static const bool check = knob::TRACE.now() && knob::SA_VISIT_CHECK.now();
+    if (!check) return NODAL_OK;
+    for (int l = 1; l + 1 < H->nlev; ++l) {
+        const SLevel *L = H->pool[l];
+        if (L->visit && l + 1 == H->tail && H->tail_dense && H->nu[l < 2 ? l : 2] == 2) NODAL_TRY(visit_check_level(h, H, l));
+    }
+    return NODAL_OK;
+}
+
 }
 
 __global__ __launch_bounds__(TB) void k_x0(int64_t n, const double *__restrict__ dinv, const double *__restrict__ r,
@@ -2200,6 +2508,10 @@
         case NODAL_HA_WCOL: buf = &L->wcol; bytes = wslots * 4; break;
         case NODAL_HA_WVAL: buf = &L->wval; bytes = wslots * 4; break;
         case NODAL_HA_WLEN: buf = &L->wlen; bytes = wslots ? L->n * 4 : 0; break;
+        case NODAL_HA_P2COL: buf = &L->p2col; bytes = next && L->visit_want ? (int64_t)P2CAP * L->ld * 4 : 0; break;
+        case NODAL_HA_P2VAL: buf = &L->p2val; bytes = next && L->visit_want ? (int64_t)P2CAP * L->ld * 4 : 0; break;
+        case NODAL_HA_P2LEN: buf = &L->p2len; bytes = next && L->visit_want ? L->n * 4 : 0; break;
+        case NODAL_HA_D2: buf = &L->d2; bytes = next && L->visit_want ? L->nc * L->ld * 4 : 0; break;
         default: return nodal_fail(h, NODAL_E_INVALID, "debug hierarchy: no such array");
         }
     }
@@ -2277,9 +2589,7 @@
     static const int kc = knob::SA_KCYCLE.now();
     H->kcycle = kc != 0;
     H->klevels = knob::SA_KLEVELS.now();
-    if (const char *e = knob::SA_NU.now()) {
-        for (int k = 0; k < 3 && e[k] >= '1' && e[k] <= '3'; ++k) H->nu[k] = e[k] - '0';
-    }
+    apply_nu_knob(H);
 
     const size_t vec = align_up((size_t)n * 8);
     NODAL_HIP_TRY(h, h->solver.reserve(6 * vec + 4 * MAX_PARTIALS * 8 + F_COUNT * 8 + 256));
@@ -2381,6 +2691,11 @@
             for (const void *q : ps) mix((uint64_t)(uintptr_t)q);
             mix((uint64_t)(L->fold ? 1 + L->wslots : 0));
             if (L->fold) { mix((uint64_t)(uintptr_t)L->wcol.p); mix((uint64_t)(uintptr_t)L->wval.p); mix((uint64_t)(uintptr_t)L->wlen.p); }
+            mix((uint64_t)L->visit);
+            if (L->visit) {
+                mix((uint64_t)(uintptr_t)L->p2col.p); mix((uint64_t)(uintptr_t)L->p2val.p);
+                mix((uint64_t)(uintptr_t)L->p2len.p); mix((uint64_t)(uintptr_t)L->d2.p);
+            }
             mix((uint64_t)L->n); mix((uint64_t)L->ld); mix((uint64_t)L->wfix); mix((uint64_t)L->rld);
         }
         if (H->it_exec && H->it_key != key) H->drop_graph();
diff --git a/nodal_amd/csrc/sagg_cycle.h b/nodal_amd/csrc/sagg_cycle.h
--- a/nodal_amd/csrc/sagg_cycle.h
+++ b/nodal_amd/csrc/sagg_cycle.h
@@ -716,35 +716,47 @@
     tail_cycle<SLOTS, true>(d, smem, image, nullptr, T, d.lv[0].n, (int)blockIdx.x);
 }
 
+template <int CH>
+__device__ __forceinline__ void tail_apply_row(int n, const double *__restrict__ T, const double *__restrict__ rc,
+                                               double *__restrict__ out, int i, int lane) {
+    const double *row = T + (int64_t)i * n;
+    double t[CH], r[CH];
+#pragma unroll
+    for (int u = 0; u < CH; ++u) {
+        const int j = lane + 64 * u;
+        t[u] = row[j < n ? j : 0];
+    }
+#pragma unroll
+    for (int u = 0; u < CH; ++u) {
+        const int j = lane + 64 * u;
+        r[u] = rc[j < n ? j : 0];
+    }
+    double s0 = 0.0, s1 = 0.0;
+#pragma unroll
+    for (int u = 0; u < CH; u += 2) {
+        if (lane + 64 * u < n && t[u] != 0.0) s0 = fma(t[u], r[u], s0);
+        if (lane + 64 * (u + 1) < n && t[u + 1] != 0.0) s1 = fma(t[u + 1], r[u + 1], s1);
+    }
+    const double s = wave_sum(s0 + s1);
+    if (lane == 0) out[i] = s;
+}
+
 template <int CH, int NV>
 __global__ __launch_bounds__(256) void k_tail_apply(int n, const double *__restrict__ T,
                                                     const double *__restrict__ rc, double *__restrict__ out) {
     const int lane = threadIdx.x & 63;
     const int i = (int)blockIdx.x * 4 + (threadIdx.x >> 6);
     if (i >= n) return;
-    const double *row = T + (int64_t)i * n;
-    double t[CH];
-#pragma unroll
-    for (int u = 0; u < CH; ++u) {
-        const int j = lane + 64 * u;
-        t[u] = row[j < n ? j : 0];
-    }
     if constexpr (NV == 1) {
-        double r[CH];
+        tail_apply_row<CH>(n, T, rc, out, i, lane);
+    } else {
+        const double *row = T + (int64_t)i * n;
+        double t[CH];
 #pragma unroll
         for (int u = 0; u < CH; ++u) {
             const int j = lane + 64 * u;
-            r[u] = rc[j < n ? j : 0];
-        }
-        double s0 = 0.0, s1 = 0.0;
-#pragma unroll
-        for (int u = 0; u < CH; u += 2) {
-            if (lane + 64 * u < n && t[u] != 0.0) s0 = fma(t[u], r[u], s0);
-            if (lane + 64 * (u + 1) < n && t[u + 1] != 0.0) s1 = fma(t[u + 1], r[u + 1], s1);
-        }
-        const double s = wave_sum(s0 + s1);
-        if (lane == 0) out[i] = s;
-    } else {
+            t[u] = row[j < n ? j : 0];
+        }
         double s[NV];
 #pragma unroll
         for (int c = 0; c < NV; ++c) s[c] = 0.0;
@@ -764,6 +776,152 @@
             const double v = wave_sum(s[c]);
             if (lane == 0) out[(int64_t)i * NV + c] = v;
         }
+    }
+}
+
+static_assert(LPR_RAGGED == 1 && TB == 256, "the visit's launches mix row blocks and dense-row blocks of 256 threads");
+
+__device__ __forceinline__ unsigned xcd_block_sub(unsigned first, unsigned count) {
+    const unsigned b = blockIdx.x - first;
+    return (count & 7u) ? b : (b & 7u) * (count >> 3) + (b >> 3);
+}
+
+template <int W>
+__device__ __forceinline__ void visit_sweep_rows(const Ell &A, const double *__restrict__ dinv, const cyc_t *__restrict__ b,
+                                                 const cyc_t *__restrict__ xin, cyc_t *__restrict__ xout, unsigned vb,
+                                                 unsigned count) {
+    for (int64_t i = (int64_t)vb * TB + threadIdx.x; i < A.n; i += (int64_t)count * TB) {
+        const double s = ell_row_w<W>(A, A.valf, i, 0, [&](int32_t j) { return (double)xin[j]; });
+        xout[i] = (cyc_t)fma(OMEGA * dinv[i], (double)b[i] - s, (double)xin[i]);
+    }
+}
+
+template <int W>
+__global__ __launch_bounds__(TB) void k_visit_first(Ell A, const double *__restrict__ dinv, const cyc_t *__restrict__ b,
+                                                    const cyc_t *__restrict__ x0, cyc_t *__restrict__ x1, unsigned grows,
+                                                    const float *__restrict__ D2, double *__restrict__ rc) {
+    if (blockIdx.x < grows) {
+        visit_sweep_rows<W>(A, dinv, b, x0, x1, xcd_block_sub(0, grows), grows);
+        return;
+    }
+    __shared__ double ws[TB / 64];
+    const int64_t I = (int64_t)(blockIdx.x - grows);
+    const float4 *row = reinterpret_cast<const float4 *>(D2 + I * A.ld);
+    const float4 *bv = reinterpret_cast<const float4 *>(b);
+    const int pieces = (int)(A.ld >> 2);
+    constexpr int U = 10;
+    double s0 = 0.0, s1 = 0.0;
+    for (int p0 = threadIdx.x; p0 < pieces; p0 += TB * U) {
+        float4 d[U], v[U];
+#pragma unroll
+        for (int u = 0; u < U; ++u) {
+            const int p = p0 + TB * u;
+            d[u] = row[p < pieces ? p : p0];
+            v[u] = bv[p < pieces ? p : p0];
+        }
+#pragma unroll
+        for (int u = 0; u < U; ++u) {
+            const int p = p0 + TB * u;
+            if (p >= pieces) continue;
+            const int64_t j = (int64_t)p * 4;
+            if (j + 0 < A.n && d[u].x != 0.0f) s0 = fma((double)d[u].x, (double)v[u].x, s0);
+            if (j + 1 < A.n && d[u].y != 0.0f) s1 = fma((double)d[u].y, (double)v[u].y, s1);
+            if (j + 2 < A.n && d[u].z != 0.0f) s0 = fma((double)d[u].z, (double)v[u].z, s0);
+            if (j + 3 < A.n && d[u].w != 0.0f) s1 = fma((double)d[u].w, (double)v[u].w, s1);
+        }
+    }
+    const double s = wave_sum(s0 + s1);
+    if ((threadIdx.x & 63) == 0) ws[threadIdx.x >> 6] = s;
+    __syncthreads();
+    if (threadIdx.x == 0) {
+        double t = 0.0;
+#pragma unroll
+        for (int w = 0; w < TB / 64; ++w) t += ws[w];
+        rc[I] = t;
+    }
+}
+
+template <int W>
+__global__ __launch_bounds__(TB) void k_visit_second(Ell A, const double *__restrict__ dinv, const cyc_t *__restrict__ b,
+                                                     const cyc_t *__restrict__ x1, cyc_t *__restrict__ x2, unsigned grows,
+                                                     int nt, const double *__restrict__ T, const double *__restrict__ rc,
+                                                     double *__restrict__ c) {
+    if (blockIdx.x < grows) {
+        visit_sweep_rows<W>(A, dinv, b, x1, x2, xcd_block_sub(0, grows), grows);
+        return;
+    }
+    const int i = (int)(blockIdx.x - grows) * 4 + (int)(threadIdx.x >> 6);
+    if (i >= nt) return;
+    tail_apply_row<TAIL_MAX_N / 64>(nt, T, rc, c, i, (int)(threadIdx.x & 63));
+}
+
+constexpr int P2CAP = 64;
+constexpr int VL = 4;
+template <int W>
+__global__ __launch_bounds__(TB) void k_visit_last(Ell A, const double *__restrict__ dinv, const cyc_t *__restrict__ b,
+                                                   const cyc_t *__restrict__ x2, cyc_t *__restrict__ out,
+                                                   const int32_t *__restrict__ p2col, const float *__restrict__ p2val,
+                                                   const int32_t *__restrict__ p2len, const double *__restrict__ c) {
+    constexpr int PQ = P2CAP / VL, AQ = W > 0 ? (W + VL - 1) / VL : 8, ROWS = TB / VL;
+    static_assert(P2CAP % VL == 0 && TB % VL == 0 && 64 % VL == 0, "whole rows per wavefront");
+    const int sub = threadIdx.x & (VL - 1);
+    for (int64_t i = (int64_t)xcd_block() * ROWS + threadIdx.x / VL; i < A.n; i += (int64_t)gridDim.x * ROWS) {
+        const int32_t len = p2len[i];
+        int32_t J[PQ];
+        float w[PQ];
+#pragma unroll
+        for (int j = 0; j < PQ; ++j) {
+            J[j] = p2col[(int64_t)(sub + VL * j) * A.ld + i];
+            w[j] = p2val[(int64_t)(sub + VL * j) * A.ld + i];
+        }
+        double s = 0.0;
+        if constexpr (W > 0) {
+            int32_t ca[AQ];
+            float va[AQ];
+#pragma unroll
+            for (int j = 0; j < AQ; ++j) {
+                const int q = sub + VL * j;
+                const int64_t at = (int64_t)(q < W ? q : 0) * A.ld + i;
+                ca[j] = A.col[at];
+                va[j] = A.valf[at];
+            }
+#pragma unroll
+            for (int j = 0; j < AQ; ++j) {
+                const double xv = (double)x2[ca[j]];
+                if (sub + VL * j < W) s = fma((double)va[j], xv, s);
+            }
+        } else {
+            const int32_t la = A.len[i];
+            for (int32_t s0 = sub; s0 < la; s0 += VL * AQ) {
+                int32_t ca[AQ];
+                float va[AQ];
+#pragma unroll
+                for (int j = 0; j < AQ; ++j) {
+                    const int32_t q = s0 + VL * j;
+                    const int64_t at = (int64_t)(q < la ? q : s0) * A.ld + i;
+                    ca[j] = A.col[at];
+                    va[j] = A.valf[at];
+                }
+#pragma unroll
+                for (int j = 0; j < AQ; ++j) {
+                    const double xv = (double)x2[ca[j]];
+                    if (s0 + VL * j < la) s = fma((double)va[j], xv, s);
+                }
+            }
+        }
+        double acc = 0.0;
+#pragma unroll
+        for (int j = 0; j < PQ; ++j) {
+            const bool ok = sub + VL * j < len;
+            const double cv = c[ok ? J[j] : 0];
+            if (ok) acc = fma((double)w[j], cv, acc);
+        }
+#pragma unroll
+        for (int off = VL >> 1; off > 0; off >>= 1) {
+            s += __shfl_xor(s, off, 64);
+            acc += __shfl_xor(acc, off, 64);
+        }
+        if (sub == 0) out[i] = (cyc_t)(fma(OMEGA * dinv[i], (double)b[i] - s, (double)x2[i]) + acc);
     }
 }
 
```

New measurement: 169.0 circuits/s, median of 6. 1.04x the previous value.
